# NikolasMarkou/blind_image_denoising

Measured on AMD Instinct MI355X. Metric: denoised images/sec (256x256x3) + MAE vs ref, resnet_1x18, higher is better.
Workload: dtype f16x2 split (hi+lo, fp32 accumulate)

## Files before the change

### blind_image_denoising_amd/_native.py

```python
import ctypes as C
import os
import pathlib

_HERE = pathlib.Path(__file__).resolve().parent
LIB_PATH = pathlib.Path(os.environ.get("BFCNN_HIP_LIB", _HERE / "lib" / "libbfcnn_hip.so"))

BF_OK, BF_EINVAL, BF_EUNSUPPORTED, BF_EWORKSPACE, BF_EHIP = 0, -1, -2, -3, -4
BF_ACT_LINEAR, BF_ACT_RELU, BF_ACT_LEAKY_RELU = 0, 1, 2
BF_REG_NONE, BF_REG_L1, BF_REG_L2 = 0, 1, 2
BF_MODE_INFERENCE, BF_MODE_TRAIN = 0, 1
BF_DTYPE_U8, BF_DTYPE_F32 = 0, 1
BF_LOSS_COUNT = 8
(BF_LOSS_TOTAL, BF_LOSS_DENOISER_TOTAL, BF_LOSS_MAE, BF_LOSS_MSE, BF_LOSS_SSIM,
 BF_LOSS_REGULARIZATION, BF_LOSS_MODEL_TOTAL, BF_LOSS_GRAD_NORM) = range(8)
EPI_RELU, EPI_AFFINE, EPI_RES, EPI_MASK, EPI_STATS, EPI_BNBWD = 1, 2, 4, 8, 16, 32


class ResnetDesc(C.Structure):
    _fields_ = [(n, C.c_int32) for n in (
        "struct_size", "in_channels", "filters", "kernel_size", "no_layers", "block_convs",
        "block_kernel", "activation", "base_activation", "use_bn", "head_filters",
        "head_activation", "out_channels", "denormalize", "reg_base", "reg_block", "reg_head")] + \
        [(n, C.c_float) for n in ("v_min", "v_max", "bn_eps", "bn_momentum", "leaky_alpha")]


class LossDesc(C.Structure):
    _fields_ = [("struct_size", C.c_int32)] + [(n, C.c_float) for n in (
        "hinge", "cutoff", "mae_multiplier", "mse_multiplier", "ssim_multiplier",
        "regularization", "depth_weight")]


class TensorInfo(C.Structure):
    _fields_ = [("name", C.c_char * 64), ("offset", C.c_int64), ("rank", C.c_int32),
                ("shape", C.c_int32 * 4), ("kind", C.c_int32), ("regularizer", C.c_int32)]


_P, _I, _I64, _F, _D = C.c_void_p, C.c_int, C.c_int64, C.c_float, C.c_double

SIGNATURES = {
    "bf_abi_version": (_I, []),
    "bf_create": (_I, [C.POINTER(ResnetDesc), C.POINTER(_P)]),
    "bf_destroy": (None, [_P]),
    "bf_last_error": (C.c_char_p, [_P]),
    "bf_param_count": (_I64, [_P]),
    "bf_state_count": (_I64, [_P]),
    "bf_tensor_count": (_I, [_P, _I]),
    "bf_tensor_at": (_I, [_P, _I, _I, C.POINTER(TensorInfo)]),
    "bf_packed_bytes": (_I64, [_P]),
    "bf_workspace_bytes": (_I64, [_P, _I, _I, _I, _I]),
    "bf_pack_inference": (_I, [_P, _P, _P, _P, _P]),
    "bf_forward_u8": (_I, [_P, _P, _P, _P, _I, _I, _I, _P, _I64, _P]),
    "bf_forward_f32": (_I, [_P, _P, _P, _P, _I, _I, _I, _P, _I64, _P]),
    "bf_forward_u8_f32": (_I, [_P, _P, _P, _P, _I, _I, _I, _P, _I64, _P]),
    "bf_train_step": (_I, [_P, _P, _P, _P, _P, _I, _I, _I, C.POINTER(LossDesc), _P, _P, _P, _P, _I64, _P]),
    "bf_adam_step": (_I, [_P, _P, _P, _P, _P, _I64, _F, _F, _F, _F, _F, _F, _P, _P, _P]),
    "bf_adam_step_ex": (_I, [_P, _P, _P, _P, _P, _I64, _F, _F, _F, _F, _F, _F, _F, _P, _I, _P, _F, _P, _P, _P]),
    "bf_avgpool_s2_same": (_I, [_P, _P, _I, _I, _I, _I, _I, _I, _P]),
    "bf_avgpool2_valid": (_I, [_P, _P, _I, _I, _I, _I, _I, _I, _P]),
    "bf_upsample2x": (_I, [_P, _P, _P, _I, _I, _I, _I, _I, _F, _F, _P]),
    "bf_laplacian_split": (_I, [_P, _P, _P, _I, _I, _I, _I, _I, _I, _P]),
    "bf_strided_slice2": (_I, [_P, _P, _I, _I, _I, _I, _P]),
    "bf_noise_augment": (_I, [_P, _P, _P, _I, _I, _I, _I, _I, _F, _F, C.c_uint64, _P]),
    "bf_image_metrics_scratch_bytes": (_I64, [_I, _I, _I, _I, _I]),
    "bf_image_metrics": (_I, [_P, _P, _I, _I, _I, _I, _I, _D, _I, _D, _D, _D, _P, _P, _I64, _P]),
    "bf_noise_estimate_scratch_bytes": (_I64, [_I, _I, _I, _I]),
    "bf_noise_estimate": (_I, [_P, _I, _I, _I, _I, _I, _P, _I64, _P, _P]),
    "bf_op_pack_pointwise": (_I, [_P, _P, _I, _I, _P]),
    "bf_op_pointwise": (_I, [_P, _P, _P, _P, _P, C.c_int64, _I, _I, _I, _F, _P]),
    "bf_op_pointwise_ex": (_I, [_P, _P, _P, _P, _P, _P, C.c_int64, _I, _I, _I, _F, _I, _P]),
    "bf_op_convnext_mlp": (_I, [_P, _P, _P, _P, _P, _P, C.c_int64, _I, _I, _F, _P]),
    "bf_op_mlp_h3_pack_bytes": (C.c_int64, [_I]),
    "bf_op_pack_mlp_h3": (_I, [_P, _P, _P, _I, _P]),
    "bf_op_convnext_mlp_h3": (_I, [_P, _P, _P, _P, _P, C.c_int64, _I, _I, _F, _P]),
    "bf_op_convnext_block1_h3": (_I, [_P, _P, _P, _P, _F, _P, _P, C.c_int64, _I, _I, _F, _P]),
    "bf_op_pack_mlp_h3_chain": (_I, [_P, _P, _P, _I, _P]),
    "bf_op_convnext_chain32_h3": (_I, [_P, _P, _P, _I, _P, _P, _P, _P, _F, _I, _I, _I, _I, _F, _I, _F, _P]),
    "bf_op_convnext_block1_up_h3": (_I, [_P, _P, _P, _P, _P, _F, _P, _P, _I, _I, _I, _I, _I, _F, _I, _F, _P]),
    "bf_op_convnext_block_h3": (_I, [_P, _P, _P, _I, _P, _F, _P, _P, _I, _I, _I, _I, _I, _F, _P]),
    "bf_op_set_variant": (_I, [C.c_char_p, _I]),
    "bf_op_dwconv_ln": (_I, [_P, _P, _P, _P, _I, _I, _I, _I, _I, _F, _I, _F, _P]),
    "bf_op_smooth_split": (_I, [_P, _P, _P, _P, _I, _I, _I, _I, _I, _I, _P]),
    "bf_op_conv2d": (_I, [_P, _P, _P, _P, _P, _I, _I, _I, _I, _I, _I, _I, _I, _I, _F, _P]),
    "bf_op_upcat_conv2d": (_I, [_P, _P, _P, _P, _P, _P, _I, _I, _I, _I, _I, _I, _I, _I, _F, _P]),
    "bf_op_dwconv_mult": (_I, [_P, _P, _P, _P, _I, _I, _I, _I, _I, _I, _I, _F, _P]),
    "bf_op_bneck_h3_pack_bytes": (C.c_int64, []),
    "bf_op_pack_bneck_h3": (_I, [_P, _P, _P, _P, _P]),
    "bf_op_bneck_block_h3": (_I, [_P, _P, _P, _P, _I, _F, _P, _I, _F, _P, _I, _F, _I, _I, _I, _I, _P]),
    "bf_op_dwmult_pointwise": (_I, [_P, _P, _P, _P, _I, _F, _P, _P, _I, _F, _P, _I, _I, _I, _I, _I, _I, _I, _P]),
    "bf_op_maxpool2": (_I, [_P, _P, _I, _I, _I, _I, _P]),
    "bf_op_maxpool2_bwd": (_I, [_P, _P, _P, _I, _I, _I, _I, _P]),
    "bf_op_norm_smooth_split": (_I, [_P, _P, _F, _I, _F, _P, _P, _P, _I, _I, _I, _I, _I, _P]),
    "bf_op_upsample_act_add": (_I, [_P, _P, _P, _I, _I, _I, _I, _I, _F, _P]),
    "bf_op_resize_bilinear": (_I, [_P, _P, _I, _I, _I, _I, _I, _I, _P]),
    "bf_op_attention": (_I, [_P, _P, _P, _P, _I, _I, _I, _P]),
    "bf_op_attention_ld": (_I, [_P, _P, _P, _P, _I, _I, _I, _I, _P]),
    "bf_op_first_conv": (_I, [_P, _I, _P, _P, _I, _I, _I, _I, _I, _I, _I, _I, _I, _F, _F, _I, _F, _P]),
    "bf_op_first_conv_h3": (_I, [_P, _I, _P, _P, _I, _I, _I, _I, _I, _I, _F, _F, _I, _F, _P]),
    "bf_op_first_conv_h3k": (_I, [_P, _I, _P, _P, _I, _I, _I, _I, _I, _I, _I, _F, _F, _I, _F, _P]),
    "bf_op_head_out": (_I, [_P, _P, _P, _I, _I, _I, _I, _I, _I, _I, _I, _I, _F, _F, _P, _P]),
    "bf_op_head_fused": (_I, [_P, _P, _F, _P, _I, _F, _P, _P, _I, _I, _I, _I, _I, _I, _I, _I, _I, _I, _F, _F, _P, _P]),
    "bf_op_head_fused_h3": (_I, [_P, _P, _F, _P, _I, _F, _P, _P, _I, _I, _I, _I, _I, _I, _I, _I, _I, _I, _F, _F, _P, _P]),
    "bf_op_fill32": (_I, [_P, _I, _I64, _P]),
    "bf_op_axpy": (_I, [_P, _P, _F, _I, _I64, _P]),
    "bf_op_conv2d_transpose": (_I, [_P, _P, _P, _I, _I, _I, _I, _I, _I, _I, _I, _F, _P]),
    "bf_op_adam_step": (_I, [_P, _P, _P, _P, _I64, _I64, _F, _F, _F, _F, _F, _F, _F, _P, _I, _P, _F, _P, _P, _P]),
    "bf_op_act_bwd": (_I, [_P, _P, _P, _I64, _I, _F, _I, _P]),
    "bf_op_matmul_wgrad": (_I, [_P, _P, _P, _I64, _I, _I, _P, _I64, _P]),
    "bf_op_dwconv_wgrad": (_I, [_P, _P, _P, _I, _I, _I, _I, _I, _P, _I64, _P]),
    "bf_op_layernorm_bwd": (_I, [_P, _P, _P, _P, _P, _I64, _I, _F, _P, _I64, _P]),
    "bf_op_scale_add": (_I, [_P, _P, _P, _P, _P, _I, _I64, _I, _P]),
    "bf_op_scale_add_bwd": (_I, [_P, _P, _P, _P, _P, _P, _I, _I64, _I, _P, _I64, _P]),
    "bf_op_multiplier_bwd": (_I, [_P, _P, _P, _I, _P]),
    "bf_op_smooth_split_bwd": (_I, [_P, _P, _P, _P, _I, _I, _I, _I, _I, _P]),
    "bf_op_smooth_split_bwd_ex": (_I, [_P, _P, _P, _P, _I, _I, _I, _I, _I, _I, _P]),
    "bf_op_upsample2x_bwd": (_I, [_P, _P, _I, _I, _I, _I, _I, _P]),
    "bf_op_conv2d_wgrad": (_I, [_P, _I, _P, _P, _I, _I, _I, _I, _I, _I, _I, _F, _F, _P, _I64, _P]),
    "bf_op_head_out_bwd": (_I, [_P, _P, _P, _P, _P, _I64, _I, _I, _I, _F, _F, _P, _I64, _P]),
    "bf_op_denoiser_loss_scratch_floats": (_I64, [_I, _I, _I, _I]),
    "bf_op_denoiser_loss": (_I, [_P, _P, _I, _I, _I, _I, C.POINTER(LossDesc), _P, _P, _P, _I64, _P]),
    "bf_op_attention_train": (_I, [_P, _P, _P, _P, _P, _P, _I, _I, _I, _P]),
    "bf_op_attention_bwd": (_I, [_P, _P, _P, _P, _P, _P, _P, _P, _P, _P, _I, _I, _I, _P]),
    "bf_op_resize_bilinear_bwd": (_I, [_P, _P, _I, _I, _I, _I, _I, _I, _P, _P]),
    "bf_op_reg_elementwise": (_I, [_P, _P, _I64, _I, _F, _F, _P, _P]),
    "bf_op_reg_soft_orthonormal": (_I, [_P, _P, _I, _I, _F, _F, _F, _F, _P, _P, _P]),
    "bf_op_reg_soft_orthogonal_ex": (_I, [_P, _P, _I, _I, _F, _F, _F, _F, _P, _P, _I, _P]),
    "bf_op_bn_train_scratch_floats": (_I64, [_I]),
    "bf_op_bn_train_fwd": (_I, [_P, _P, _P, _P, _P, _P, _I64, _I, _F, _F, _I, _F, _P, _I64, _P]),
    "bf_op_bn_train_bwd": (_I, [_P, _P, _P, _P, _P, _P, _I64, _I, _P, _I64, _P]),
    "bf_op_gate_save_floats": (_I64, [_I, _I, _I]),
    "bf_op_gate_scratch_floats": (_I64, [_I, _I]),
    "bf_op_gate_fwd": (_I, [_P, _P, _P, _P, _P, _P, _I, _I64, _I, _I, _P, _I64, _P]),
    "bf_op_gate_bwd": (_I, [_P, _P, _P, _P, _P, _P, _P, _P, _I, _I64, _I, _I, _P, _I64, _P]),
    "bf_op_channel_gate_save_floats": (_I64, [_I, _I, _I, _I]),
    "bf_op_channel_gate_ex": (_I, [_P, _P, _P, _P, _P, _P, _P, _P, _P, _P, _I, _I64, _I, _I, _I, _I, _F, _I, _P, _I64, _P]),
    "bf_op_dense2": (_I, [_P, _P, _P, _P, _P, _P, _I64, _I, _I, _I, _I, _F, _I, _P]),
    "bf_op_selector_mix": (_I, [_P, _P, _P, _P, _I64, _I, _P]),
    "bf_op_avgpool_same": (_I, [_P, _P, _I, _I, _I, _I, _I, _I, _I, _I, _P]),
    "bf_op_concat_channels": (_I, [_P, _P, _P, _P, _I64, _I, _I, _I, _P]),
    "bf_op_channel_mean_broadcast": (_I, [_P, _P, _I, _I64, _I, _I64, _P, _I64, _P]),
    "bf_op_sigmoid_gate": (_I, [_P, _P, _P, _P, _I64, _P]),
    "bf_op_sigmoid_gate_bwd": (_I, [_P, _P, _P, _P, _P, _I64, _P]),
    "bf_op_relu_shift": (_I, [_P, _I, _F, _P, _I, _P]),
    "bf_op_linear_shift": (_I, [_P, _I, _F, _P, _I, _P]),
    "bf_op_center_scale": (_I, [_P, _P, _P, _P, _I64, _F, _P]),
    "bf_op_pass_filter": (_I, [_P, _P, _I64, _F, _I, _I, _P]),
    "bf_op_pass_filter_bwd": (_I, [_P, _P, _P, _I64, _F, _I, _I, _P]),
    "bf_op_center_scale_bwd": (_I, [_P, _P, _P, _P, _P, _P, _I64, _F, _P]),
    "bf_op_center_sq_bwd": (_I, [_P, _P, _P, _P, _P, _I64, _P]),
    "bf_op_concat_input": (_I, [_P, _P, _I, _P, _I, _I, _I, _I, _I, _I, _I, _I, _F, _F, _P]),
    "bf_op_selector_mix_bwd": (_I, [_P, _P, _P, _P, _P, _P, _P, _I64, _I, _P]),
    "bf_op_avgpool_same_bwd": (_I, [_P, _P, _I, _I, _I, _I, _I, _I, _I, _I, _I, _P]),
    "bf_op_dense2_bwd_scratch_floats": (_I64, [_I64, _I, _I]),
    "bf_op_dense2_bwd": (_I, [_P, _P, _P, _P, _P, _P, _P, _I64, _I, _I, _I, _F, _P, _I64, _P]),
    "bf_op_slice_channels": (_I, [_P, _P, _I64, _I, _I, _I, _P]),
    "bf_op_relu_shift_bwd": (_I, [_P, _I, _F, _P, _P, _I, _P]),
    "bf_op_normalize": (_I, [_P, _P, _I64, _F, _F, _I, _P]),
    "bf_op_channel_repeat": (_I, [_P, _P, _I64, _I, _I, _P]),
    "bf_op_channel_group_sum": (_I, [_P, _P, _I64, _I, _I, _P]),
    "bf_op_group_kernel": (_I, [_P, _P, _I, _I, _I, _I, _P]),
    "bf_op_flip_hw": (_I, [_P, _P, _I, _I, _P]),
    "bf_op_transpose2d": (_I, [_P, _P, _I, _I, _P]),
    "bf_comm_unique_id": (_I, [C.c_char_p]),
    "bf_comm_init_rank": (_I, [C.POINTER(_P), _I, _I, C.c_char_p]),
    "bf_comm_destroy": (_I, [_P]),
    "bf_allreduce_grads": (_I, [_P, _P, _I64, _P, _P]),
    "bf_comm_last_error": (C.c_char_p, []),
    "bf_op_channel_multiplier": (_I, [_P, _P, _I, _P]),
    "bf_op_prune_tensors": (_I, [_P, _I64, _P, _I, _I, _F, _F, _F, C.c_uint64, _P, _P, _P]),
    "bf_op_count_below": (_I, [_P, _I64, _P, _I, _F, _P, _P]),
    "bf_op_dihedral_stack_u8": (_I, [_P, _P, _P, _I, _I, _I, _I, _I, _P]),
    "bf_op_dihedral_merge": (_I, [_P, _P, _P, _I, _I, _I, _I, _I, _I, _P]),
    "bf_op_risk_probe_u8": (_I, [_P, _P, _I, _I, _I, _I, _I, _I, C.c_uint64, _P]),
    "bf_op_risk_sums_scratch_bytes": (_I64, [_I, _I, _I, _I, _I]),
    "bf_op_risk_sums": (_I, [_P, _P, _I, _I, _I, _I, _I, _I, C.c_uint64, _P, _I64, _P, _P]),
    "bf_op_neighbor_pairs": (_I, [_P, _I, _P, _F, _P, _P, _I, _I, _I, _I, C.c_uint64, _P]),
    "bf_set_option": (_I, [_P, C.c_char_p, _I]),
    "bf_get_timing": (_I, [_P, C.POINTER(C.c_float), C.POINTER(C.c_int)]),
    "bf_get_block_kernel": (C.c_char_p, [_P, C.POINTER(C.c_int)]),
    "bf_get_train_kernels": (C.c_char_p, [_P]),
    "bf_debug_conv3x3": (_I, [_P, _P, _P, _P, _P, _P, _P, _P, _P, _I, _I, _I, _I, _I, _P]),
    "bf_debug_conv3x3_grid": (_I, [_I, _I, _I]),
    "bf_debug_h3_weight_scale": (_F, [_F]),
    "bf_debug_fused_block": (_I, [_P, _P, _P, _P, _P, _P, _P, _I, _I, _I, _I, _P]),
    "bf_debug_fused_block_h3_scratch_floats": (_I64, [_I, _I, _I]),
    "bf_debug_fused_block_h3": (_I, [_P, _P, _P, _P, _P, _P, _P, _I, _I, _I, _I, _P]),
    "bf_debug_fused_block2_h3_scratch_floats": (_I64, [_I, _I, _I]),
    "bf_debug_fused_block2_h3": (_I, [_P, _P, _P, _P, _P, _P, _I, _I, _I, _I, _I, _P]),
    "bf_debug_set_h3_variant": (_I, [_I]),
    "bf_debug_set_upsample_band": (_I, [_I]),
    "bf_debug_conv3x3_h3_scratch_floats": (_I64, []),
    "bf_debug_conv3x3_h3": (_I, [_P, _P, _P, _P, _P, _P, _P, _I, _I, _I, _I, _I, _P]),
    "bf_debug_wgrad_partial_floats": (_I64, [_I, _I, _I]),
    "bf_debug_wgrad3x3": (_I, [_P, _P, _P, _P, _I, _I, _I, _P]),
    "bf_debug_wgrad3x3_h3": (_I, [_P, _P, _P, _P, _I, _I, _I, _P]),
    "bf_debug_fwd_block_h3t_scratch_floats": (_I64, [_I, _I, _I]),
    "bf_debug_fwd_block_h3t": (_I, [_P, _P, _P, _P, _P, _P, _P, _P, _P, _P, _P, _I, _I, _I, _I, _I, _P]),
    "bf_debug_bwd_block_h3t_scratch_floats": (_I64, [_I, _I, _I]),
    "bf_debug_bwd_block_h3t": (_I, [_P, _P, _P, _P, _P, _P, _P, _P, _P, _P, _P, _P, _I, _I, _I, _I, _I, _P]),
    "bf_debug_conv3x3_h3_pre": (_I, [_P, _P, _P, _P, _P, _P, _P, _P, _I, _I, _I, _I, _I, _P]),
    "bf_debug_bwd3x3_h3_scratch_floats": (_I64, [_I, _I, _I]),
    "bf_debug_bwd3x3_h3_grid": (_I, [_I, _I, _I]),
    "bf_debug_bwd3x3_h3_grid_ex": (_I, [_I, _I, _I, _I]),
    "bf_debug_bwd3x3_h3": (_I, [_P, _P, _P, _P, _P, _P, _P, _P, _P, _P, _P, _I, _I, _I, _I, _I, _I, _P]),
    "bf_debug_forward_plan": (_I, [_P, _I, _I, _I, _I, C.c_char_p, _I]),
    "bf_debug_mfma_probe": (_I, [_P, _P, _P, _P]),
}

BF_STATUS_BYTES = 2048
BF_STATUS_F16_RANGE = 1

_lib = None


class StreamArg(C.c_void_p):
    _bf_device = None


def _device_guard(fn):
    def call(*args):
        for a in args:
            dev = getattr(a, "_bf_device", None)
            if dev is not None:
                import torch
                if torch.cuda.current_device() != dev:
                    with torch.cuda.device(dev):
                        return fn(*args)
                break
        return fn(*args)
    call.raw = fn
    call.__name__ = getattr(fn, "__name__", "bf_call")
    return call


class _Library:

    def __init__(self, handle):
        self._handle = handle

    def __getattr__(self, name):
        return getattr(self._handle, name)


def lib():
    global _lib
    if _lib is None:
        if not LIB_PATH.exists():
            raise ImportError(
                f"{LIB_PATH} is missing: the gfx950 HIP library has not been built "
                f"(run blind_image_denoising_amd/csrc/build.sh). There is no CPU fallback.")
        handle = C.CDLL(str(LIB_PATH), mode=getattr(os, "RTLD_NOW", 2))
        wrapped = _Library(handle)
        for name, (res, args) in SIGNATURES.items():
            fn = getattr(handle, name)
            fn.restype = res
            fn.argtypes = args
            setattr(wrapped, name, _device_guard(fn))
        if handle.bf_abi_version() != 1:
            raise ImportError("libbfcnn_hip.so ABI version mismatch")
        _lib = wrapped
    return _lib


def last_error(handle=None) -> str:
    msg = lib().bf_last_error(handle)
    return msg.decode("utf-8", "replace") if msg else ""


def check(rc: int, handle=None, what: str = ""):
    if rc == BF_OK:
        return
    msg = f"{what}: {last_error(handle)}" if what else last_error(handle)
    if rc == BF_EINVAL:
        raise ValueError(msg)
    if rc == BF_EUNSUPPORTED:
        raise NotImplementedError(msg)
    if rc == BF_EWORKSPACE:
        raise MemoryError(msg)
    raise RuntimeError(f"HIP error ({rc}) {msg}")


def call(fn_name: str, *args):
    check(getattr(lib(), fn_name)(*args), None, fn_name)


def ptr(t):
    if t is None:
        return None
    if not t.is_contiguous():
        raise ValueError("tensor must be contiguous")
    return C.c_void_p(t.data_ptr())


def stream_ptr(t=None):
    import torch
    if t is not None and t.is_cuda:
        dev = t.device.index if t.device.index is not None else torch.cuda.current_device()
    else:
        dev = torch.cuda.current_device()
    s = StreamArg(torch.cuda.current_stream(dev).cuda_stream)
    s._bf_device = dev
    return s
```

### blind_image_denoising_amd/csrc/base_rows.hip

```cpp
#include "bf_common.h"
#include "h3_core.h"
#include "h3_weights.h"
#include <cstdlib>

constexpr int BR_NT = 256, BR_CW = 256, BR_RING = 4, BR_ROWPX = BR_CW + 4;

__global__ __launch_bounds__(BR_NT) void base_conv_rows_kernel(BaseConvArgs a, int nchunks, int rows_per_band, int nbands, int abl)
{
    __shared__ __attribute__((aligned(16))) h4 ring[BR_RING][2][BR_ROWPX];
    __shared__ float red[BR_NT];
    const int tid = threadIdx.x, lane = tid & 63, wave = tid >> 6, n = lane & 15, q = lane >> 4;
    if (a.status && blockIdx.x == 0 && tid == 0) *a.status = 0;
    const float* __restrict__ w = a.w;

    auto wval = [&](const int tap, const int c, const int m) -> float {
        if (c < 3) return w[(tap * 3 + c) * 16 + m] / 255.0f;
        return -0.5f * (w[(tap * 3 + 0) * 16 + m] + w[(tap * 3 + 1) * 16 + m] + w[(tap * 3 + 2) * 16 + m]);
    };
    const float s = bf_h3_block_weight_scale<BR_NT>([&](const int i) { return wval(i / 64, (i >> 4) & 3, i & 15); }, 9 * 4 * 16, red);
    const float inv_s = 1.0f / s;
    h8 wa[3];
#pragma unroll
    for (int dy = 0; dy < 3; ++dy) {
#pragma unroll
        for (int j = 0; j < 8; ++j) {
            const int slot = 8 * (q & 1) + j, dx = slot >> 2, c = slot & 3;
            float v = 0.f;
            if (dx < 3) v = wval(dy * 3 + dx, c, n) * s;
            _Float16 hi, lo;
            bf_h3_split(v, hi, lo);
            wa[dy][j] = (q >> 1) ? lo : hi;
        }
    }

    int bx = blockIdx.x;
    const int ch = bx % nchunks; bx /= nchunks;
    const int band = bx % nbands;
    const int b = bx / nbands;
    const int x0 = ch * BR_CW;
    const int y0 = band * rows_per_band, y1 = min(y0 + rows_per_band, a.H);
    const uint8_t* __restrict__ src = reinterpret_cast<const uint8_t*>(a.in) + (int64_t)b * a.Hs * a.Ws * 3;

    auto fetch = [&](const int yy, const int j) -> h4 {
        const int x = x0 - 1 + j;
        h4 r = {(_Float16)0.f, (_Float16)0.f, (_Float16)0.f, (_Float16)0.f};
        if (yy >= 0 && yy < a.H && x >= 0 && x < a.W) {
            r[3] = (_Float16)1.f;
            if (!(abl & 2) && yy < a.Hs && x < a.Ws) {
                const uint8_t* p = src + ((int64_t)yy * a.Ws + x) * 3;
                r[0] = (_Float16)(float)p[0];
                r[1] = (_Float16)(float)p[1];
                r[2] = (_Float16)(float)p[2];
            }
        }
        return r;
    };
    auto store_px = [&](const int slot, const int j, const h4 v) {
        ring[slot][0][j] = v;
        if (j > 0) ring[slot][1][j - 1] = v;
    };
    auto put = [&](const int yy) {
        const int slot = ((yy % BR_RING) + BR_RING) % BR_RING;
        store_px(slot, tid, fetch(yy, tid));
        if (tid < 4) store_px(slot, BR_CW + tid, fetch(yy, BR_CW + tid));
    };
    put(y0 - 1);
    put(y0);
    put(y0 + 1);
    __syncthreads();

    const int64_t hw = (int64_t)a.H * a.W;
    char* outb = reinterpret_cast<char*>(a.out) + (int64_t)b * hw * 64 + (int64_t)((q >> 1) + 2 * (q & 1)) * hw * 16;
    int frag_off[4];
#pragma unroll
    for (int g = 0; g < 4; ++g) {
        const int p = 64 * wave + 16 * g + n + 2 * (q & 1);
        frag_off[g] = ((p & 1) * BR_ROWPX + (p & ~1)) * 8;
    }
    const char* ring_b = reinterpret_cast<const char*>(&ring[0][0][0]);
    constexpr int SLOT_BYTES = 2 * BR_ROWPX * 8;
    for (int y = y0; y < y1; ++y) {
        const h4 nx = fetch(y + 2, tid);
        h4 nx2 = {(_Float16)0.f, (_Float16)0.f, (_Float16)0.f, (_Float16)0.f};
        if (tid < 4) nx2 = fetch(y + 2, BR_CW + tid);
        int so[3];
#pragma unroll
        for (int dy = 0; dy < 3; ++dy) so[dy] = ((((y + dy - 1) % BR_RING) + BR_RING) % BR_RING) * SLOT_BYTES;
        char* orow = outb + (int64_t)y * a.W * 16;
#pragma unroll
        for (int g = 0; g < 4; ++g) {
            const int xc = 64 * wave + 16 * g + n;
            f32x4 acc = {0.f, 0.f, 0.f, 0.f};
#pragma unroll
            for (int dy = 0; dy < 3; ++dy)
                acc = MFMA_H(wa[dy], *reinterpret_cast<const h8*>(ring_b + so[dy] + frag_off[g]), acc);
            acc = bf_acc_ready(acc) * inv_s;
            if (a.act_relu) {
#pragma unroll
                for (int c = 0; c < 4; ++c) acc[c] = fmaxf(acc[c], 0.f);
            }
            const int x = x0 + xc;
            const h8 rec = h3_split_record(acc);
            if ((abl & 1) ? acc[0] == 12345.678f : x < a.W) *reinterpret_cast<h8*>(orow + (int64_t)x * 16) = rec;
        }
        const int slot = (((y + 2) % BR_RING) + BR_RING) % BR_RING;
        store_px(slot, tid, nx);
        if (tid < 4) store_px(slot, BR_CW + tid, nx2);
        __syncthreads();
    }
}

bool bf_base_conv_rows_supports(const BaseConvArgs& a)
{
    return a.in_is_u8 && a.cin == 3 && a.k == 3 && a.out_split == 1 && a.v_min == 0.f && a.v_max == 255.f && a.H >= 1 && a.W >= 1;
}

hipError_t bf_launch_base_conv_rows(const BaseConvArgs& a, hipStream_t s)
{
    if (!bf_base_conv_rows_supports(a)) return hipErrorInvalidValue;
    const int nchunks = (a.W + BR_CW - 1) / BR_CW;
    int rows = 32;
    int ablate = 0;
#ifdef BF_ABLATE
    if (const char* e = getenv("BF_BASE_ROWS_ABL")) ablate = atoi(e);
    if (const char* e = getenv("BF_BASE_ROWS_BAND")) rows = atoi(e) > 0 ? atoi(e) : rows;
    else
#endif
    while (rows > 8 && (int64_t)a.B * nchunks * ((a.H + rows - 1) / rows) < 1024) rows /= 2;
    const int nbands = (a.H + rows - 1) / rows;
    const int64_t grid = (int64_t)a.B * nchunks * nbands;
    if (grid > 0x7fffffff) return hipErrorInvalidValue;
    hipLaunchKernelGGL(base_conv_rows_kernel, dim3((unsigned)grid), dim3(BR_NT), 0, s, a, nchunks, rows, nbands, ablate);
    return hipGetLastError();
}
```

### blind_image_denoising_amd/csrc/bf_common.h

```cpp
#pragma once
#include <hip/hip_runtime.h>
#include <stdint.h>
#include <stddef.h>
#include "../../include/bfcnn_hip.h"
#include "../../include/bfcnn_hip_debug.h"

typedef float f32x4 __attribute__((ext_vector_type(4)));

__device__ __forceinline__ f32x4 bf_acc_ready(f32x4 acc)
{
    asm volatile("s_nop 7" : "+v"(acc));
    return acc;
}


#include <mutex>
#include <unordered_set>
inline hipError_t bf_set_max_lds(const void* kernel, int bytes)
{
    static std::mutex mu;
    static std::unordered_set<uint64_t> done;
    int dev = 0;
    hipError_t e = hipGetDevice(&dev);
    if (e != hipSuccess) return e;
    const uint64_t key = (uint64_t)(uintptr_t)kernel * 131u + (uint64_t)(dev + 1);
    std::lock_guard<std::mutex> lock(mu);
    if (done.count(key)) return hipSuccess;
    e = hipFuncSetAttribute(kernel, hipFuncAttributeMaxDynamicSharedMemorySize, bytes);
    if (e == hipSuccess) done.insert(key);
    return e;
}

typedef _Float16 bf_h8 __attribute__((ext_vector_type(8)));
typedef _Float16 bf_h2 __attribute__((ext_vector_type(2)));
typedef short bf_s2 __attribute__((ext_vector_type(2)));
typedef unsigned bf_u2 __attribute__((ext_vector_type(2)));
#define BF_H3C_SCALE (1.0f / 4096.0f)
__device__ __forceinline__ bf_u2 bf_h3c_encode8(const bf_h8 v)
{
    const bf_h2 lim = {(_Float16)(448.0f / 4096.0f), (_Float16)(448.0f / 4096.0f)};
    bf_h2 p[4] = {{v[0], v[1]}, {v[2], v[3]}, {v[4], v[5]}, {v[6], v[7]}};
#pragma unroll
    for (int i = 0; i < 4; ++i) p[i] = __builtin_elementwise_min(__builtin_elementwise_max(p[i], -lim), lim);
    bf_s2 r0 = {0, 0}, r1 = {0, 0};
    r0 = __builtin_amdgcn_cvt_scalef32_pk_fp8_f16(r0, p[0], BF_H3C_SCALE, false);
    r0 = __builtin_amdgcn_cvt_scalef32_pk_fp8_f16(r0, p[1], BF_H3C_SCALE, true);
    r1 = __builtin_amdgcn_cvt_scalef32_pk_fp8_f16(r1, p[2], BF_H3C_SCALE, false);
    r1 = __builtin_amdgcn_cvt_scalef32_pk_fp8_f16(r1, p[3], BF_H3C_SCALE, true);
    bf_u2 out;
    out[0] = ((unsigned)(unsigned short)r0[0]) | ((unsigned)(unsigned short)r0[1] << 16);
    out[1] = ((unsigned)(unsigned short)r1[0]) | ((unsigned)(unsigned short)r1[1] << 16);
    return out;
}
__device__ __forceinline__ bf_h8 bf_h3c_decode8(const bf_u2 b)
{
    const bf_h2 a0 = __builtin_amdgcn_cvt_scalef32_pk_f16_fp8(b[0], BF_H3C_SCALE, false);
    const bf_h2 a1 = __builtin_amdgcn_cvt_scalef32_pk_f16_fp8(b[0], BF_H3C_SCALE, true);
    const bf_h2 a2 = __builtin_amdgcn_cvt_scalef32_pk_f16_fp8(b[1], BF_H3C_SCALE, false);
    const bf_h2 a3 = __builtin_amdgcn_cvt_scalef32_pk_f16_fp8(b[1], BF_H3C_SCALE, true);
    return (bf_h8){a0[0], a0[1], a1[0], a1[1], a2[0], a2[1], a3[0], a3[1]};
}

__device__ __forceinline__ float bf_gelu(const float v)
{
    const float a = fabsf(v) * 0.70710678f;
    float q = fmaf(4.22452448e-05f, a, -4.19236813e-04f);
    q = fmaf(q, a, 1.40204388e-03f);
    q = fmaf(q, a, 9.21467334e-04f);
    q = fmaf(q, a, -2.83861113e-02f);
    q = fmaf(q, a, 1.48544322e-01f);
    q = fmaf(q, a, 9.18402423e-01f);
    q = fmaf(q, a, 1.62790967f);
    const float h = __builtin_amdgcn_exp2f(fmaf(-a, q, -1.f));
    return v * (v >= 0.f ? 1.f - h : h);
}

#define BF_C 16
#define BF_WPACK_FLOATS (36 * 64)

enum { EPI_RELU = 1, EPI_AFFINE = 2, EPI_RES = 4, EPI_MASK = 8, EPI_STATS = 16, EPI_BNBWD = 32 };

struct ConvArgs {
    const float* in;
    float* out;
    const float* wpack;
    const float* scale;
    const float* shift;
    const float* res;
    const float* mask;
    float* stats;
    const float* bnc;
    int B, H, W;
    int reverse;
    const float* pre_c; const float* pre_scale; const float* pre_shift; float* pre_out;
};

struct FusedBlockArgs {
    const float* in;
    float* out;
    const float* w1pack;
    const float* w2pack;
    const float* scale;
    const float* shift;
    int B, H, W;
    int tiles_x, tiles_y, ntiles;
    int act1_relu;
    const float* zeros;
};

#define BF_H3R_WPACK_FLOATS (13 * 64 * 4)
#define BF_H3_BLOCK_FLOATS (64 + 2 * BF_H3R_WPACK_FLOATS)
struct FusedH3Args {
    const void* in;
    void* out;
    const void* w1r;
    const void* w2r;
    const float* aux;
    int B, H, W;
    int tiles_x, tiles_y, ntiles;
    int rows_per_tile;
    int reverse_tiles;
    int variant;
    int act1_relu;
    const void* zeros;
    void* dump;
    unsigned long long* dbg;
    const float* head_wh;
    void* head_out;
    int head_u8, Ho, Wo, denormalize;
    float v_min, v_max;
    int* status;
    int compact = 0;
};
struct H3Request {
    int B, H, W;
    int variant;
    bool head;
    bool compact;
};
enum class H3Kernel { Tiles32, Tiles16, FullRow };
struct H3Choice {
    H3Kernel kernel;
    bool bottom_up;
};
H3Choice   bf_select_fused_block_h3(const H3Request& r);
hipError_t bf_launch_fused_block_h3_as(const FusedH3Args& a, H3Kernel k, hipStream_t s);
hipError_t bf_launch_fused_block_h3(const FusedH3Args& a, hipStream_t s);
bool       bf_fused_block_h3_use_pairs(const H3Request& r);
const char* bf_fused_block_h3_kernel_name(H3Kernel k);
const char* bf_fused_block_kernel_name();
void       bf_set_h3_variant(int v);
hipError_t bf_launch_fused_block_h3v(const FusedH3Args& a, hipStream_t s);
bool       bf_fused_block_h3v_supports(int H, int W);
struct FusedH3WArgs {
    const void* in;
    void* out;
    const void* w1r[2];
    const void* w2r[2];
    const float* aux[2];
    int B, H, W;
    int nstrips, tiles_y, ntiles, rows_per_tile;
    int reverse_tiles;
    int act1_relu;
    const void* zeros;
    unsigned long long* dbg;
    const float* head_wh;
    void* head_out;
    int head_u8, Ho, Wo, denormalize;
    float v_min, v_max;
    int* status;
};
hipError_t bf_launch_fused_block2_h3w(const FusedH3WArgs& a, hipStream_t s);
bool       bf_fused_block2_h3w_supports(int H, int W);
hipError_t bf_launch_pack_h3(const float* params, const float* state, int64_t p_blocks, int64_t p_stride, float* dst,
                             int64_t d_stride, int layers, int use_bn, float eps, const float* ext_scale,
                             const float* ext_shift, hipStream_t s);
#define BF_H3_TRAIN_PACK_FLOATS (BF_H3R_WPACK_FLOATS + 64)
#define BF_TRAIN_PACK_STRIDE BF_H3_TRAIN_PACK_FLOATS
hipError_t bf_launch_conv3x3_h3(const ConvArgs& a, int epi, hipStream_t s);
hipError_t bf_launch_wgrad3x3_h3(const float* x, const float* dy, float* partial, float* dw, int B, int H, int W, hipStream_t s);

struct BwdH3Args {
    const float* x;
    const float* g;
    const float* c;
    const float* coef;
    const float* wpack;
    float* out;
    const float* res;
    const float* bnc;
    float* wpartial;
    float* stats;
    int B, H, W, reverse;
    int reserved[4];
    int tiles_x, tiles_y, ntiles;
};
struct FwdBlockH3Args {
    const float* x;
    const float* pre_c;
    const float* pre_scale; const float* pre_shift;
    float* a_out;
    float* t_out;
    float* c_out;
    const float* wpack0;
    const float* wpack1;
    float* stats;
    int B, H, W, reverse, act_relu;
    int tiles_y, ntiles, rows_per_tile;
    const float* fin_partial;
    int fin_nblk;
    double fin_count;
    const float* fin_gamma;
    float *fin_mm, *fin_mv;
    float fin_eps, fin_momentum;
    float* fin_scale;
    float* fin_meaninv;
};
bool       bf_fwd_block_h3t_supports(int H, int W);
int        bf_fwd_block_h3t_grid(int B, int H, int W);
hipError_t bf_launch_fwd_block_h3t(const FwdBlockH3Args& a, hipStream_t s);
struct BwdBlockH3Args {
    const float* a;
    const float* g;
    const float* c;
    const float* coef;
    const float* wfwd0;
    const float* wdg1;
    const float* wdg0;
    const float* bnc;
    float* out;
    float* wpartial1;
    float* wpartial0;
    float* stats;
    int B, H, W, reverse, act_relu;
    int nstrips, tiles_y, ntiles, rows_per_tile;
    unsigned long long* dbg;
    const float* fin_partial;
    int fin_nblk;
    double fin_count;
    const float* fin_gamma;
    const float* fin_meaninv;
    float* fin_dgamma;
};
bool       bf_bwd_block_h3t_supports(int H, int W);
int        bf_bwd_block_h3t_grid(int B, int H, int W);
int64_t    bf_bwd_block_h3t_strip_rows(int B, int H, int W);
hipError_t bf_launch_bwd_block_h3t(const BwdBlockH3Args& a, hipStream_t s);
int        bf_bwd3x3_h3_grid(int B, int H, int W);
hipError_t bf_launch_bwd3x3_h3(const BwdH3Args& a, int epi, float* dw, hipStream_t s);
hipError_t bf_launch_reduce_wgrad_slots(const float* slots, int64_t slot_floats, int nblk, float* out, int64_t p_stride, int layers,
                                        int nconv, int unit, hipStream_t s);
hipError_t bf_launch_pack_h3_train(const float* params, int64_t p_blocks, int64_t p_stride, float* dst, int layers, int nconv,
                                   int unit, hipStream_t s);
hipError_t bf_launch_h3_from_f32(const float* x, void* y, int B, int H, int W, hipStream_t s);
hipError_t bf_launch_h3_to_f32(const void* y, float* x, int B, int H, int W, hipStream_t s);

hipError_t bf_launch_conv3x3_c16(const ConvArgs& a, int epi, hipStream_t s);
int        bf_conv3x3_c16_grid(int B, int H, int W);
hipError_t bf_launch_fused_block(const FusedBlockArgs& a, hipStream_t s);
void       bf_set_fused_tile(int variant);
hipError_t bf_launch_pack_conv(const float* w_hwio, float* wpack, int transpose_flip, hipStream_t s);
hipError_t bf_launch_wgrad3x3_c16(const float* x, const float* dy, float* partial, float* dw,
                                  int B, int H, int W, hipStream_t s);
int        bf_wgrad_grid(int B, int H, int W);

struct BaseConvArgs {
    const void* in; float* out; const float* w;
    int B, Hs, Ws, H, W, cin, k, in_is_u8, act_relu;
    float v_min, v_max;
    int out_split;
    int* status;
};
hipError_t bf_launch_base_conv(const BaseConvArgs& a, hipStream_t s);
bool       bf_base_conv_rows_supports(const BaseConvArgs& a);
hipError_t bf_launch_base_conv_rows(const BaseConvArgs& a, hipStream_t s);
void       bf_set_base_conv_rows(int on);
hipError_t bf_launch_base_wgrad(const float* in_f32, const float* dy, float* partial, float* dw,
                                int B, int H, int W, int cin, int k, float v_min, float v_max, hipStream_t s);
int        bf_base_wgrad_grid(int B, int H, int W);

struct HeadArgs {
    const float* feat;
    const float* w0;
    const float* w1;
    const float* wh;
    void* out;
    int B, H, W, Ho, Wo, hf, cout, act, out_is_u8, denormalize;
    float v_min, v_max, leaky_alpha;
    int feat_split;
    int* status;
};
#define BF_STATUS_BYTES 2048

hipError_t bf_launch_head(const HeadArgs& a, hipStream_t s);

struct HeadTrainArgs {
    const float* feat; const float* wh;
    const float* gt; float* pred;
    float* dfeat;
    float* partial;
    const float* dextra;
    int B, H, W, cout, denormalize;
    float v_min, v_max, hinge, cutoff, dscale;
    float dfeat_scale;
};
hipError_t bf_launch_head_train(const HeadTrainArgs& a, int grid, hipStream_t s);
hipError_t bf_launch_loss_extra(const float* pred, const float* gt, int B, int H, int W, int C, const float* head_partial,
                                int blocks_per_image, float hinge, float cutoff, float mse_multiplier, float ssim_multiplier,
                                float depth_weight, float max_val, float* maps, float* ssim_partial, float* coef, float* scal,
                                float* dextra, hipStream_t s);
hipError_t bf_launch_loss_extra_finalize(const float* scal, int B, int H, int W, int C, float mse_multiplier, float ssim_multiplier,
                                         float depth_weight, float* losses, hipStream_t s);
int        bf_head_train_grid(int B, int H, int W);

hipError_t bf_launch_bn_finalize(const float* partial, int nblk, double count, const float* gamma,
                                 float* moving_mean, float* moving_var, float eps, float momentum,
                                 float* scale, float* shift, float* mean_inv , double* stage1 ,
                                 hipStream_t s);
hipError_t bf_launch_affine_add(const float* x, const float* c, const float* scale, const float* shift,
                                float* y, int64_t npix, hipStream_t s);
hipError_t bf_launch_affine_act(const float* c, const float* scale, const float* shift, float* y, int relu, int64_t npix,
                                hipStream_t s);
hipError_t bf_launch_bn_bwd_reduce(const float* dy, const float* c, float* partial, int64_t npix, int grid, hipStream_t s);
hipError_t bf_launch_bn_bwd_finalize(const float* partial, int nblk, double count, const float* gamma,
                                     const float* mean_inv, float* coef , float* dgamma,
                                     double* stage1 , hipStream_t s);
hipError_t bf_launch_bn_bwd_apply(const float* dy, const float* c, const float* coef, float* dc, int64_t npix, hipStream_t s);
hipError_t bf_launch_reduce_partials(const float* partial, int nblk, int width, float* out, float scale, hipStream_t s);
hipError_t bf_launch_zero(float* p, int64_t n, hipStream_t s);
```

### blind_image_denoising_amd/csrc/edge_layers.hip

```cpp
#include "bf_common.h"
#include "block_reduce.h"

typedef _Float16 h8 __attribute__((ext_vector_type(8)));

constexpr int BC_T = 16;

template <int CIN, int K, bool U8>
__global__ __launch_bounds__(256) void base_conv_kernel(BaseConvArgs a)
{
    constexpr int R = K / 2, IT = BC_T + 2 * R;
    __shared__ float tile[IT * IT * CIN];
    const float* __restrict__ wg = a.w;
    const int tiles_x = (a.W + BC_T - 1) / BC_T, tiles_y = (a.H + BC_T - 1) / BC_T;
    int t = blockIdx.x;
    const int tx = t % tiles_x; t /= tiles_x;
    const int ty = t % tiles_y;
    const int b = t / tiles_y;
    const int y0 = ty * BC_T, x0 = tx * BC_T;
    if (a.status && blockIdx.x == 0 && threadIdx.x == 0) *a.status = 0;
    const float range = a.v_max - a.v_min;
    {
        constexpr int NE = (IT * IT * CIN + 255) / 256;
        float raw[NE];
        bool inimg[NE];
#pragma unroll
        for (int i = 0; i < NE; ++i) {
            const int n = threadIdx.x + i * 256;
            const int ci = n % CIN, px = (n / CIN) % IT, row = n / (CIN * IT);
            const int gy = y0 - R + row, gx = x0 - R + px;
            inimg[i] = n < IT * IT * CIN && gy >= 0 && gy < a.H && gx >= 0 && gx < a.W;
            raw[i] = 0.f;
            if (inimg[i] && gy < a.Hs && gx < a.Ws) {
                const int64_t si = (((int64_t)b * a.Hs + gy) * a.Ws + gx) * CIN + ci;
                raw[i] = U8 ? (float)reinterpret_cast<const uint8_t*>(a.in)[si] : reinterpret_cast<const float*>(a.in)[si];
            }
        }
#pragma unroll
        for (int i = 0; i < NE; ++i) {
            const int n = threadIdx.x + i * 256;
            const float v = inimg[i] ? (fminf(fmaxf(raw[i], a.v_min), a.v_max) - a.v_min) / range - 0.5f : 0.f;
            if (n < IT * IT * CIN) tile[n] = v;
        }
    }
    __syncthreads();
    const int ly = threadIdx.x >> 4, lx = threadIdx.x & 15;
    const int y = y0 + ly, x = x0 + lx;
    float acc[16];
#pragma unroll
    for (int c = 0; c < 16; ++c) acc[c] = 0.f;
#pragma unroll
    for (int ky = 0; ky < K; ++ky)
#pragma unroll
        for (int kx = 0; kx < K; ++kx)
#pragma unroll
            for (int ci = 0; ci < CIN; ++ci) {
                const float v = tile[((ly + ky) * IT + lx + kx) * CIN + ci];
                const float* wr = wg + ((ky * K + kx) * CIN + ci) * 16;
#pragma unroll
                for (int c = 0; c < 16; ++c) acc[c] = fmaf(v, wr[c], acc[c]);
            }
    if (y < a.H && x < a.W) {
        if (a.act_relu) {
#pragma unroll
            for (int c = 0; c < 16; ++c) acc[c] = fmaxf(acc[c], 0.f);
        }
        if (a.out_split) {
            const int64_t hw = (int64_t)a.H * a.W;
            char* base = reinterpret_cast<char*>(a.out) + (int64_t)b * hw * 64 + ((int64_t)y * a.W + x) * 16;
            h8 hi[2], lo[2];
#pragma unroll
            for (int c = 0; c < 16; ++c) {
                const _Float16 h = (_Float16)acc[c];
                hi[c >> 3][c & 7] = h;
                lo[c >> 3][c & 7] = (_Float16)(acc[c] - (float)h);
            }
            *reinterpret_cast<h8*>(base) = hi[0];
            *reinterpret_cast<h8*>(base + hw * 16) = hi[1];
            if (a.out_split == 2) {
                char* lob = reinterpret_cast<char*>(a.out) + (int64_t)b * hw * 64 + hw * 32 + ((int64_t)y * a.W + x) * 8;
                *reinterpret_cast<bf_u2*>(lob) = bf_h3c_encode8(lo[0]);
                *reinterpret_cast<bf_u2*>(lob + hw * 8) = bf_h3c_encode8(lo[1]);
                return;
            }
            *reinterpret_cast<h8*>(base + hw * 32) = lo[0];
            *reinterpret_cast<h8*>(base + hw * 48) = lo[1];
            return;
        }
        float4* o = reinterpret_cast<float4*>(a.out + (((int64_t)b * a.H + y) * a.W + x) * 16);
        o[0] = make_float4(acc[0], acc[1], acc[2], acc[3]);
        o[1] = make_float4(acc[4], acc[5], acc[6], acc[7]);
        o[2] = make_float4(acc[8], acc[9], acc[10], acc[11]);
        o[3] = make_float4(acc[12], acc[13], acc[14], acc[15]);
    }
}

template <int CIN, int K>
static hipError_t launch_base(const BaseConvArgs& a, hipStream_t s)
{
    const int grid = a.B * ((a.H + BC_T - 1) / BC_T) * ((a.W + BC_T - 1) / BC_T);
    if (a.in_is_u8) hipLaunchKernelGGL((base_conv_kernel<CIN, K, true>), dim3(grid), dim3(256), 0, s, a);
    else            hipLaunchKernelGGL((base_conv_kernel<CIN, K, false>), dim3(grid), dim3(256), 0, s, a);
    return hipGetLastError();
}

static int g_base_rows = 1;
void bf_set_base_conv_rows(int on) { g_base_rows = on == 2 ? 2 : (on ? 1 : 0); }
static bool base_rows_preferred(const BaseConvArgs& a)
{
    const int64_t nchunks = (a.W + 255) / 256;
    return (int64_t)a.B * a.H * nchunks >= 8192 && (int64_t)a.W * 5 >= nchunks * 256 * 3;
}

hipError_t bf_launch_base_conv(const BaseConvArgs& a, hipStream_t s)
{
    if (g_base_rows && bf_base_conv_rows_supports(a) && (g_base_rows == 2 || base_rows_preferred(a))) return bf_launch_base_conv_rows(a, s);
#define BF_BASE(C, KK) if (a.cin == C && a.k == KK) return launch_base<C, KK>(a, s);
    BF_BASE(3, 3) BF_BASE(3, 5) BF_BASE(3, 7) BF_BASE(3, 1)
    BF_BASE(1, 3) BF_BASE(1, 5) BF_BASE(1, 7) BF_BASE(1, 1)
#undef BF_BASE
    return hipErrorInvalidValue;
}

constexpr int BW_TH = 16, BW_TW = 32;

template <int CIN, int K>
__global__ __launch_bounds__(512) void base_wgrad_kernel(const float* __restrict__ in, const float* __restrict__ dy,
                                                         float* __restrict__ partial, int B, int H, int W,
                                                         float v_min, float v_max, int tiles_x, int tiles_y, int ntiles)
{
    constexpr int R = K / 2, IH = BW_TH + 2 * R, IW = BW_TW + 2 * R;
    constexpr int NCOMB = K * K * CIN, PERC = (NCOMB + 31) / 32, NOUT = NCOMB * 16;
    static_assert(BW_TH == 16, "one row slice per 32 threads");
    __shared__ float tx_[IH * IW * CIN];
    __shared__ __attribute__((aligned(16))) float td[BW_TH * BW_TW * 16];
    const int tid = threadIdx.x, slice = tid >> 5, j0 = tid & 31;
    const float range = v_max - v_min;
    f32x4 acc[PERC][4];
    int xoff[PERC];
#pragma unroll
    for (int i = 0; i < PERC; ++i) {
#pragma unroll
        for (int q = 0; q < 4; ++q) acc[i][q] = (f32x4){0.f, 0.f, 0.f, 0.f};
        int jj = j0 + 32 * i;
        if (jj >= NCOMB) jj = 0;
        const int ci = jj % CIN, tap = jj / CIN;
        xoff[i] = ((tap / K) * IW + (tap % K)) * CIN + ci;
    }
    for (int t = blockIdx.x; t < ntiles; t += gridDim.x) {
        int tt = t;
        const int txi = tt % tiles_x; tt /= tiles_x;
        const int tyi = tt % tiles_y;
        const int b = tt / tiles_y;
        const int y0 = tyi * BW_TH, x0 = txi * BW_TW;
        for (int n = tid; n < IH * IW * CIN; n += 512) {
            const int ci = n % CIN, px = (n / CIN) % IW, row = n / (CIN * IW);
            const int gy = y0 - R + row, gx = x0 - R + px;
            float v = 0.f;
            if (gy >= 0 && gy < H && gx >= 0 && gx < W) {
                const float raw = in[(((int64_t)b * H + gy) * W + gx) * CIN + ci];
                v = (fminf(fmaxf(raw, v_min), v_max) - v_min) / range - 0.5f;
            }
            tx_[n] = v;
        }
        for (int n = tid; n < BW_TH * BW_TW * 4; n += 512) {
            const int row = n / (BW_TW * 4), rem = n - row * (BW_TW * 4);
            const int gy = y0 + row, gx = x0 + (rem >> 2);
            float4 v = make_float4(0.f, 0.f, 0.f, 0.f);
            if (gy < H && gx < W)
                v = *reinterpret_cast<const float4*>(dy + (((int64_t)b * H + gy) * W + gx) * 16 + (rem & 3) * 4);
            *reinterpret_cast<float4*>(td + n * 4) = v;
        }
        __syncthreads();
        for (int c = 0; c < BW_TW; ++c) {
            const int pb = (slice * IW + c) * CIN, db = (slice * BW_TW + c) * 16;
            f32x4 d[4];
#pragma unroll
            for (int q = 0; q < 4; ++q) d[q] = *reinterpret_cast<const f32x4*>(td + db + 4 * q);
#pragma unroll
            for (int i = 0; i < PERC; ++i) {
                const float xv = tx_[pb + xoff[i]];
#pragma unroll
                for (int q = 0; q < 4; ++q) acc[i][q] += d[q] * xv;
            }
        }
        __syncthreads();
    }
    float* red = td;
#pragma unroll
    for (int i = 0; i < PERC; ++i) {
        __syncthreads();
#pragma unroll
        for (int q = 0; q < 4; ++q) *reinterpret_cast<f32x4*>(red + (slice * 32 + j0) * 16 + 4 * q) = acc[i][q];
        __syncthreads();
        const int jj = (tid >> 4) + 32 * i, co = tid & 15;
        if (jj < NCOMB) {
            float a = 0.f;
#pragma unroll
            for (int sl = 0; sl < 16; ++sl) a += red[(sl * 32 + (tid >> 4)) * 16 + co];
            partial[(size_t)blockIdx.x * NOUT + jj * 16 + co] = a;
        }
    }
}

int bf_base_wgrad_grid(int B, int H, int W)
{
    const int ntiles = B * ((H + BW_TH - 1) / BW_TH) * ((W + BW_TW - 1) / BW_TW);
    return ntiles < 512 ? ntiles : 512;
}

template <int CIN, int K>
static hipError_t launch_base_wgrad(const float* in, const float* dy, float* partial, float* dw, int B, int H, int W,
                                    float v_min, float v_max, hipStream_t s)
{
    const int tiles_x = (W + BW_TW - 1) / BW_TW, tiles_y = (H + BW_TH - 1) / BW_TH;
    const int ntiles = B * tiles_x * tiles_y, grid = bf_base_wgrad_grid(B, H, W);
    hipLaunchKernelGGL((base_wgrad_kernel<CIN, K>), dim3(grid), dim3(512), 0, s, in, dy, partial, B, H, W, v_min, v_max,
                       tiles_x, tiles_y, ntiles);
    hipError_t e = hipGetLastError();
    if (e != hipSuccess) return e;
    return bf_launch_reduce_partials(partial, grid, K * K * CIN * 16, dw, 1.0f, s);
}

hipError_t bf_launch_base_wgrad(const float* in, const float* dy, float* partial, float* dw, int B, int H, int W,
                                int cin, int k, float v_min, float v_max, hipStream_t s)
{
#define BF_BW(C, KK) if (cin == C && k == KK) return launch_base_wgrad<C, KK>(in, dy, partial, dw, B, H, W, v_min, v_max, s);
    BF_BW(3, 3) BF_BW(3, 5) BF_BW(3, 7) BF_BW(3, 1)
    BF_BW(1, 3) BF_BW(1, 5) BF_BW(1, 7) BF_BW(1, 1)
#undef BF_BW
    return hipErrorInvalidValue;
}

__device__ __forceinline__ float bf_act(float x, int act, float alpha)
{
    if (act == BF_ACT_RELU) return fmaxf(x, 0.f);
    if (act == BF_ACT_LEAKY_RELU) return x > 0.f ? x : alpha * x;
    return x;
}

template <bool U8>
__global__ __launch_bounds__(256) void head_kernel(HeadArgs a)
{
    __shared__ float w0s[16 * 64];
    __shared__ float w1s[64 * 4];
    __shared__ float whs[64];
    const bool fused = a.wh != nullptr;
    if (fused) {
        for (int i = threadIdx.x; i < 64; i += 256) whs[i] = a.wh[i];
    } else {
        for (int i = threadIdx.x; i < 16 * a.hf; i += 256) w0s[i] = a.w0[i];
        for (int i = threadIdx.x; i < a.hf * a.cout; i += 256) w1s[i] = a.w1[i];
    }
    __syncthreads();
    const int64_t npix = (int64_t)a.B * a.Ho * a.Wo;
    for (int64_t pix = (int64_t)blockIdx.x * 256 + threadIdx.x; pix < npix; pix += (int64_t)gridDim.x * 256) {
        const int x = (int)(pix % a.Wo);
        const int64_t t = pix / a.Wo;
        const int y = (int)(t % a.Ho);
        const int b = (int)(t / a.Ho);
        float f[16];
        if (a.feat_split) {
            const int64_t hw = (int64_t)a.H * a.W;
            const char* base = reinterpret_cast<const char*>(a.feat) + (int64_t)b * hw * 64 + ((int64_t)y * a.W + x) * 16;
            const h8 hi0 = *reinterpret_cast<const h8*>(base), hi1 = *reinterpret_cast<const h8*>(base + hw * 16);
            h8 lo0, lo1;
            if (a.feat_split == 2) {
                const char* lob = reinterpret_cast<const char*>(a.feat) + (int64_t)b * hw * 64 + hw * 32 + ((int64_t)y * a.W + x) * 8;
                lo0 = bf_h3c_decode8(*reinterpret_cast<const bf_u2*>(lob));
                lo1 = bf_h3c_decode8(*reinterpret_cast<const bf_u2*>(lob + hw * 8));
            } else {
                lo0 = *reinterpret_cast<const h8*>(base + hw * 32);
                lo1 = *reinterpret_cast<const h8*>(base + hw * 48);
            }
            bool finite = true;
#pragma unroll
            for (int c = 0; c < 8; ++c) {
                f[c] = (float)hi0[c] + (float)lo0[c];
                f[8 + c] = (float)hi1[c] + (float)lo1[c];
                finite = finite && fabsf(f[c]) <= 3.0e38f && fabsf(f[8 + c]) <= 3.0e38f;
            }
            if (!finite && a.status) atomicOr(a.status, BF_STATUS_F16_RANGE);
        } else {
            const float4* fp = reinterpret_cast<const float4*>(a.feat + (((int64_t)b * a.H + y) * a.W + x) * 16);
#pragma unroll
            for (int i = 0; i < 4; ++i) {
                const float4 v = fp[i];
                f[4 * i] = v.x; f[4 * i + 1] = v.y; f[4 * i + 2] = v.z; f[4 * i + 3] = v.w;
            }
        }
        float h1[4] = {0.f, 0.f, 0.f, 0.f};
        if (fused) {
#pragma unroll
            for (int c = 0; c < 16; ++c)
#pragma unroll
                for (int o = 0; o < 4; ++o) h1[o] = fmaf(f[c], whs[c * 4 + o], h1[o]);
        } else {
            for (int j = 0; j < a.hf; ++j) {
                float h = 0.f;
#pragma unroll
                for (int c = 0; c < 16; ++c) h = fmaf(f[c], w0s[c * a.hf + j], h);
                h = bf_act(h, a.act, a.leaky_alpha);
                for (int o = 0; o < a.cout; ++o) h1[o] = fmaf(h, w1s[j * a.cout + o], h1[o]);
            }
        }
        for (int o = 0; o < a.cout; ++o) {
            float v = tanhf(2.0f * h1[o]) * 0.51f;
            if (a.denormalize) v = (fminf(fmaxf(v, -0.5f), 0.5f) + 0.5f) * (a.v_max - a.v_min) + a.v_min;
            if (U8) {
                const float r = fminf(fmaxf(rintf(v), 0.f), 255.f);
                reinterpret_cast<uint8_t*>(a.out)[pix * a.cout + o] = (uint8_t)r;
            } else {
                reinterpret_cast<float*>(a.out)[pix * a.cout + o] = v;
            }
        }
    }
}

hipError_t bf_launch_head(const HeadArgs& a, hipStream_t s)
{
    const int64_t npix = (int64_t)a.B * a.Ho * a.Wo;
    int64_t g = (npix + 255) / 256;
    const int grid = (int)(g < 8192 ? g : 8192);
    if (a.out_is_u8) hipLaunchKernelGGL(head_kernel<true>, dim3(grid), dim3(256), 0, s, a);
    else             hipLaunchKernelGGL(head_kernel<false>, dim3(grid), dim3(256), 0, s, a);
    return hipGetLastError();
}

constexpr int HT_BLOCKS_PER_IMAGE_MAX = 64;

__global__ __launch_bounds__(256) void head_train_kernel(HeadTrainArgs a, int blocks_per_image)
{
    __shared__ float whs[64];
    __shared__ float red[4][80];
    if (threadIdx.x < 64) whs[threadIdx.x] = a.wh[threadIdx.x];
    __syncthreads();
    const int b = blockIdx.x / blocks_per_image, sub = blockIdx.x % blocks_per_image;
    const int hw = a.H * a.W;
    float M[64];
#pragma unroll
    for (int i = 0; i < 64; ++i) M[i] = 0.f;
    float s_abs = 0.f, s_hinge = 0.f, s_sq = 0.f, s_sqh = 0.f;
    for (int pi = sub * 256 + threadIdx.x; pi < hw; pi += blocks_per_image * 256) {
        const int64_t pix = (int64_t)b * hw + pi;
        const float4* fp = reinterpret_cast<const float4*>(a.feat + pix * 16);
        float f[16];
#pragma unroll
        for (int i = 0; i < 4; ++i) {
            const float4 v = fp[i];
            f[4 * i] = v.x; f[4 * i + 1] = v.y; f[4 * i + 2] = v.z; f[4 * i + 3] = v.w;
        }
        float dh1[4] = {0.f, 0.f, 0.f, 0.f};
#pragma unroll
        for (int o = 0; o < 4; ++o) {
            if (o < a.cout) {
                float h = 0.f;
#pragma unroll
                for (int c = 0; c < 16; ++c) h = fmaf(f[c], whs[c * 4 + o], h);
                const float th = tanhf(2.0f * h);
                const float pv = th * 0.51f;
                float pred = pv, dpred_dp = 1.0f;
                if (a.denormalize) {
                    pred = (fminf(fmaxf(pv, -0.5f), 0.5f) + 0.5f) * (a.v_max - a.v_min) + a.v_min;
                    dpred_dp = (pv >= -0.5f && pv <= 0.5f) ? (a.v_max - a.v_min) : 0.f;
                }
                if (a.pred) a.pred[pix * a.cout + o] = pred;
                const float e = a.gt[pix * a.cout + o] - pred;
                const float ae = fabsf(e);
                s_abs += fminf(ae, 255.0f);
                s_hinge += ae > a.hinge ? fminf(ae, a.cutoff) : 0.f;
                const float ep = e > 0.f ? fminf(e, 255.0f) : 0.f;
                s_sq += ep * ep;
                const float eh = e > a.hinge ? fminf(e, a.cutoff * a.cutoff) : 0.f;
                s_sqh += eh * eh;
                float dpred = 0.f;
                if (ae > a.hinge && ae < a.cutoff) dpred = (e > 0.f ? -1.f : (e < 0.f ? 1.f : 0.f)) * a.dscale;
                if (a.dextra) dpred += a.dextra[pix * a.cout + o];
                dh1[o] = dpred * dpred_dp * (0.51f * 2.0f) * (1.0f - th * th);
            }
        }
        float df[16];
#pragma unroll
        for (int c = 0; c < 16; ++c) {
            float d = 0.f;
#pragma unroll
            for (int o = 0; o < 4; ++o) {
                d = fmaf(dh1[o], whs[c * 4 + o], d);
                M[c * 4 + o] = fmaf(f[c], dh1[o], M[c * 4 + o]);
            }
            df[c] = d * a.dfeat_scale;
        }
        float4* dp = reinterpret_cast<float4*>(a.dfeat + pix * 16);
#pragma unroll
        for (int i = 0; i < 4; ++i) dp[i] = make_float4(df[4 * i], df[4 * i + 1], df[4 * i + 2], df[4 * i + 3]);
    }
#pragma unroll
    for (int i = 0; i < 64; ++i) bf_tile_stage(red, i, M[i]);
    const float sv[4] = {s_abs, s_hinge, s_sq, s_sqh};
#pragma unroll
    for (int i = 0; i < 4; ++i) bf_tile_stage(red, 64 + i, sv[i]);
    __syncthreads();
    if (threadIdx.x < 80) {
        const int i = threadIdx.x;
        a.partial[(size_t)blockIdx.x * 80 + i] = i < 68 ? (red[0][i] + red[1][i]) + (red[2][i] + red[3][i]) : 0.f;
    }
}

int bf_head_train_grid(int B, int H, int W)
{
    int bpi = (H * W + 1023) / 1024;
    if (bpi > HT_BLOCKS_PER_IMAGE_MAX) bpi = HT_BLOCKS_PER_IMAGE_MAX;
    if (bpi < 1) bpi = 1;
    return B * bpi;
}

hipError_t bf_launch_head_train(const HeadTrainArgs& a, int grid, hipStream_t s)
{
    hipLaunchKernelGGL(head_train_kernel, dim3(grid), dim3(256), 0, s, a, grid / a.B);
    return hipGetLastError();
}
```

### blind_image_denoising_amd/csrc/engine.h

```cpp
#pragma once
#include "bf_common.h"
#include <string>
#include <utility>
#include <vector>

constexpr int BF_TIMING_RING = 256;

struct TimingRing {
    enum Kind { None, Forward, TrainBlock };
    std::vector<hipEvent_t> ev;
    int64_t n = 0;
    int launches_in_pair = 0;
    Kind kind = None;

    void restart() { n = 0; kind = None; }
    hipError_t begin(hipStream_t s) { return hipEventRecord(ev[2 * (n % BF_TIMING_RING)], s); }
    hipError_t end(hipStream_t s, int launches, Kind k)
    {
        int64_t slot = n % BF_TIMING_RING;
        if (k != kind) {
            std::swap(ev[0], ev[2 * slot]);
            n = 0; slot = 0; kind = k;
        }
        launches_in_pair = launches;
        ++n;
        return hipEventRecord(ev[2 * slot + 1], s);
    }
};

struct bf_engine {
    bf_resnet_desc d;
    std::string err;
    std::vector<bf_tensor_info> tensors, states;
    int64_t n_params = 0, n_state = 0;
    int64_t p_base = 0, p_blocks = 0, p_block_stride = 0, p_head0 = 0, p_head1 = 0;
    int64_t n_base = 0;
    int64_t k_base = 0, k_blocks = 0, k_block_stride = 0, k_w0 = 0, k_w1 = 0, k_wh = 0, k_zero = 0, k_h3 = 0, k_total = 0;
    int fused_blocks = 1;
    int fused_head = 0;
    int h3_zigzag = 1;
    int h3_variant = -1;
    int h3_compact = 0;
    int h3_pair = 1;
    int h3_pair_head = 0;
    int block_launches = 0;
    const char* block_kernel = "";
    std::string train_kernels;
    int arith = 1;
    int train_arith = 1;
    int train_zigzag = 1;
    int train_fused_fwd = 1;
    int train_fwd_block = 1;
    int train_bwd_block = 1;
    int train_fold_finalize = 1;
    int train_fused_bwd = 1;
    int timing = 0;
    TimingRing timed;
};

int fail(bf_handle h, int code, const char* fmt, ...);
int hip_fail(bf_handle h, hipError_t e, const char* what);

#define BF_HIP(call, what) do { hipError_t e__ = (call); if (e__ != hipSuccess) return hip_fail(h, e__, what); } while (0)

static inline int64_t align_up(int64_t v, int64_t a) { return (v + a - 1) / a * a; }

static inline int pow2_target(int n)
{
    int p = 1;
    while (p < n) p <<= 1;
    return p;
}

hipError_t bf_launch_pack_all_convs(const float* params, int64_t p_blocks, int64_t p_stride, float* dst, int64_t d_stride, int layers,
                                    int with_dgrad, int nconv, int unit, hipStream_t s);
int64_t bf_train_workspace_floats(bf_handle h, int B, int H, int W);
```

### blind_image_denoising_amd/csrc/engine.hip

```cpp
#include "engine.h"
#include <cstdarg>
#include <cstdio>
#include <cstring>

static thread_local std::string g_create_error;

int fail(bf_handle h, int code, const char* fmt, ...)
{
    char buf[512];
    va_list ap;
    va_start(ap, fmt);
    vsnprintf(buf, sizeof(buf), fmt, ap);
    va_end(ap);
    if (h) h->err = buf; else g_create_error = buf;
    return code;
}

int hip_fail(bf_handle h, hipError_t e, const char* what)
{
    return fail(h, BF_EHIP, "%s: %s", what, hipGetErrorString(e));
}

extern "C" int bf_abi_version(void) { return BFCNN_ABI_VERSION; }

extern "C" const char* bf_last_error(bf_handle h) { return h ? h->err.c_str() : g_create_error.c_str(); }

static void add_tensor(std::vector<bf_tensor_info>& v, const char* name, int64_t& off, int rank, int s0, int s1, int s2,
                       int s3, int kind, int reg)
{
    bf_tensor_info t;
    memset(&t, 0, sizeof(t));
    snprintf(t.name, sizeof(t.name), "%s", name);
    t.offset = off;
    t.rank = rank;
    t.shape[0] = s0; t.shape[1] = s1; t.shape[2] = s2; t.shape[3] = s3;
    t.kind = kind;
    t.regularizer = reg;
    int64_t n = 1;
    for (int i = 0; i < rank; ++i) n *= t.shape[i];
    off += n;
    v.push_back(t);
}

extern "C" int bf_create(const bf_resnet_desc* d, bf_handle* out)
{
    if (out) *out = nullptr;
    if (!d || !out) return fail(nullptr, BF_EINVAL, "bf_create: desc/out must not be NULL");
    if (d->struct_size != (int32_t)sizeof(bf_resnet_desc))
        return fail(nullptr, BF_EINVAL, "bf_create: struct_size %d != %d (ABI mismatch)", d->struct_size, (int)sizeof(bf_resnet_desc));
    if (d->no_layers < 0) return fail(nullptr, BF_EINVAL, "no_layers must be >= 0");
    if (d->block_convs <= 0) return fail(nullptr, BF_EINVAL, "len(block_kernels) must be >= 0 ");
    if (d->block_convs > 3) return fail(nullptr, BF_EINVAL, "len(block_kernels) must be <= 3");
    if (d->in_channels != 1 && d->in_channels != 3)
        return fail(nullptr, BF_EUNSUPPORTED, "in_channels %d: only 1 and 3 are built", d->in_channels);
    if (d->filters != BF_C) return fail(nullptr, BF_EUNSUPPORTED, "filters %d: the MFMA path is built for 16", d->filters);
    if (d->kernel_size != 1 && d->kernel_size != 3 && d->kernel_size != 5 && d->kernel_size != 7)
        return fail(nullptr, BF_EUNSUPPORTED, "base kernel_size %d: only 1,3,5,7", d->kernel_size);
    if (d->block_kernel != 3)
        return fail(nullptr, BF_EUNSUPPORTED, "block_kernels must be 3x3 (got %d convs of %d)", d->block_convs, d->block_kernel);
    if (d->activation != BF_ACT_RELU && d->activation != BF_ACT_LINEAR)
        return fail(nullptr, BF_EUNSUPPORTED, "block activation must be relu or linear");
    if (d->base_activation != BF_ACT_LINEAR)
        return fail(nullptr, BF_EUNSUPPORTED, "base_activation must be linear");
    if (d->head_filters < 1 || d->head_filters > 64) return fail(nullptr, BF_EUNSUPPORTED, "head filters must be in 1..64");
    if (d->out_channels < 1 || d->out_channels > 4) return fail(nullptr, BF_EUNSUPPORTED, "output_channels must be in 1..4");
    if (!(d->v_max > d->v_min)) return fail(nullptr, BF_EINVAL, "value_range must have max > min");

    bf_engine* h = new bf_engine();
    h->d = *d;
    const int k = d->kernel_size, cin = d->in_channels, hf = d->head_filters, co = d->out_channels;
    int64_t off = 0;
    h->p_base = off;
    add_tensor(h->tensors, "base/kernel", off, 4, k, k, cin, BF_C, BF_KIND_CONV, d->reg_base);
    h->n_base = off;
    h->p_blocks = off;
    const int nb = d->block_convs;
    h->p_block_stride = nb * 2304 + (d->use_bn ? (nb - 1) * 16 : 0);
    char name[64];
    for (int i = 0; i < d->no_layers; ++i) {
        for (int j = 0; j < nb; ++j) {
            snprintf(name, sizeof(name), "block%d/conv%d/kernel", i, j);
            add_tensor(h->tensors, name, off, 4, 3, 3, BF_C, BF_C, BF_KIND_CONV, d->reg_block);
            if (j >= 1 && d->use_bn) {
                snprintf(name, sizeof(name), "block%d/bn%d/gamma", i, j);
                add_tensor(h->tensors, name, off, 1, BF_C, 0, 0, 0, BF_KIND_GAMMA, BF_REG_NONE);
            }
        }
    }
    h->p_head0 = off;
    add_tensor(h->tensors, "head/conv0/kernel", off, 4, 1, 1, BF_C, hf, BF_KIND_CONV, d->reg_head);
    h->p_head1 = off;
    add_tensor(h->tensors, "head/conv1/kernel", off, 4, 1, 1, hf, co, BF_KIND_CONV, d->reg_head);
    h->n_params = off;
    int64_t soff = 0;
    if (d->use_bn) {
        for (int i = 0; i < d->no_layers; ++i)
            for (int j = 1; j < nb; ++j) {
                snprintf(name, sizeof(name), "block%d/bn%d/moving_mean", i, j);
                add_tensor(h->states, name, soff, 1, BF_C, 0, 0, 0, BF_KIND_MOVING_MEAN, BF_REG_NONE);
                snprintf(name, sizeof(name), "block%d/bn%d/moving_variance", i, j);
                add_tensor(h->states, name, soff, 1, BF_C, 0, 0, 0, BF_KIND_MOVING_VAR, BF_REG_NONE);
            }
    }
    h->n_state = soff;
    int64_t ko = 0;
    h->k_base = ko; ko += align_up(h->n_base, 64);
    h->k_blocks = ko; h->k_block_stride = nb == 2 ? 2 * BF_WPACK_FLOATS + 32 : nb * (BF_WPACK_FLOATS + 32);
    ko += h->k_block_stride * d->no_layers;
    h->k_w0 = ko; ko += align_up(16 * hf, 64);
    h->k_w1 = ko; ko += align_up(hf * co, 64);
    h->k_wh = ko; ko += 64;
    h->k_zero = ko; ko += 64;
    h->k_h3 = ko; ko += (int64_t)BF_H3_BLOCK_FLOATS * d->no_layers;
    h->k_total = ko;
    *out = h;
    return BF_OK;
}

extern "C" void bf_destroy(bf_handle h)
{
    if (!h) return;
    for (hipEvent_t e : h->timed.ev) (void)hipEventDestroy(e);
    delete h;
}
extern "C" int64_t bf_param_count(bf_handle h) { return h ? h->n_params : -1; }
extern "C" int64_t bf_state_count(bf_handle h) { return h ? h->n_state : -1; }
extern "C" int bf_tensor_count(bf_handle h, int state) { return h ? (int)(state ? h->states.size() : h->tensors.size()) : -1; }

extern "C" int bf_tensor_at(bf_handle h, int state, int index, bf_tensor_info* out)
{
    if (!h || !out) return BF_EINVAL;
    const auto& v = state ? h->states : h->tensors;
    if (index < 0 || index >= (int)v.size()) return fail(h, BF_EINVAL, "tensor index %d out of range", index);
    *out = v[index];
    return BF_OK;
}

extern "C" int bf_set_option(bf_handle h, const char* key, int value)
{
    if (!h || !key) return BF_EINVAL;
    if (!strcmp(key, "fused_blocks")) { h->fused_blocks = value ? 1 : 0; return BF_OK; }
    if (!strcmp(key, "fused_tile")) { bf_set_fused_tile(value); return BF_OK; }
    if (!strcmp(key, "h3_variant")) { h->h3_variant = value; return BF_OK; }
    if (!strcmp(key, "h3_zigzag")) { h->h3_zigzag = value ? 1 : 0; return BF_OK; }
    if (!strcmp(key, "h3_compact")) { h->h3_compact = value ? 1 : 0; return BF_OK; }
    if (!strcmp(key, "h3_pair")) { h->h3_pair = value == 2 ? 2 : (value ? 1 : 0); return BF_OK; }
    if (!strcmp(key, "base_rows")) { bf_set_base_conv_rows(value); return BF_OK; }
    if (!strcmp(key, "h3_pair_head")) { h->h3_pair_head = value ? 1 : 0; return BF_OK; }
    if (!strcmp(key, "fused_head")) { h->fused_head = value ? 1 : 0; return BF_OK; }
    if (!strcmp(key, "train_zigzag")) { h->train_zigzag = value ? 1 : 0; return BF_OK; }
    if (!strcmp(key, "train_fused_fwd")) { h->train_fused_fwd = value ? 1 : 0; return BF_OK; }
    if (!strcmp(key, "train_fused_bwd")) { h->train_fused_bwd = value ? 1 : 0; return BF_OK; }
    if (!strcmp(key, "train_bwd_block")) { h->train_bwd_block = value < 0 ? 1 : (value > 2 ? 2 : value); return BF_OK; }
    if (!strcmp(key, "train_fwd_block")) { h->train_fwd_block = value < 0 ? 1 : (value > 2 ? 2 : value); return BF_OK; }
    if (!strcmp(key, "train_fused_bwd2") || !strcmp(key, "train_bwd_dbuf")) return BF_OK;
    if (!strcmp(key, "train_fold_finalize")) { h->train_fold_finalize = value ? 1 : 0; return BF_OK; }
    if (!strcmp(key, "train_arith")) { h->train_arith = value < 0 ? 1 : (value ? 1 : 0); return BF_OK; }
    if (!strcmp(key, "arith")) { h->arith = value < 0 ? 1 : (value ? 1 : 0); return BF_OK; }
    if (!strcmp(key, "timing")) {
        h->timing = value ? 1 : 0;
        h->timed.restart();
        if (h->timing && h->timed.ev.empty()) {
            h->timed.ev.resize(2 * BF_TIMING_RING, nullptr);
            for (hipEvent_t& e : h->timed.ev)
                if (hipEventCreate(&e) != hipSuccess) return fail(h, BF_EHIP, "hipEventCreate failed");
        }
        return BF_OK;
    }
    return fail(h, BF_EINVAL, "unknown option [%s]", key);
}

extern "C" int bf_get_timing(bf_handle h, float* ms, int* launches)
{
    if (!h || !ms || !launches) return BF_EINVAL;
    const TimingRing& t = h->timed;
    if (!h->timing || t.ev.empty()) return fail(h, BF_EINVAL, "timing option is off");
    const int64_t n = t.n < BF_TIMING_RING ? t.n : BF_TIMING_RING;
    if (n == 0) return fail(h, BF_EINVAL, "no forward has run since the timing option was set");
    double total = 0.0;
    for (int64_t i = 0; i < n; ++i) {
        float one = 0.f;
        hipError_t e = hipEventElapsedTime(&one, t.ev[2 * i], t.ev[2 * i + 1]);
        if (e != hipSuccess) return hip_fail(h, e, "hipEventElapsedTime");
        total += one;
    }
    *ms = (float)total;
    *launches = (int)(t.launches_in_pair * n);
    return BF_OK;
}

extern "C" const char* bf_get_block_kernel(bf_handle h, int* launches_per_forward)
{
    if (!h) return "";
    if (launches_per_forward) *launches_per_forward = h->block_launches;
    return h->block_kernel;
}

extern "C" const char* bf_get_train_kernels(bf_handle h) { return h ? h->train_kernels.c_str() : ""; }

extern "C" int64_t bf_packed_bytes(bf_handle h) { return h ? h->k_total * 4 : -1; }

extern "C" int64_t bf_workspace_bytes(bf_handle h, int mode, int B, int H, int W)
{
    if (!h || B <= 0 || H <= 0 || W <= 0) return -1;
    if (mode == BF_MODE_INFERENCE) {
        const int Hp = pow2_target(H), Wp = pow2_target(W);
        return (int64_t)B * Hp * Wp * 16 * 4 * 3 + BF_STATUS_BYTES;
    }
    return bf_train_workspace_floats(h, B, H, W) * 4;
}
```

### blind_image_denoising_amd/csrc/engine_infer.hip

```cpp
#include "engine.h"
#include <cstdio>
#include <cstring>

__global__ void pack_all_convs_kernel(const float* __restrict__ params, int64_t p_blocks, int64_t p_stride, float* __restrict__ dst,
                                      int64_t d_stride, int with_dgrad, int nconv, int unit)
{
    const int per = (with_dgrad ? 2 : 1) * nconv;
    const int layer = blockIdx.x / per, which = blockIdx.x % per;
    const int cj = which % nconv;
    const float* w = params + p_blocks + layer * p_stride + (cj == 0 ? 0 : 2304 + (int64_t)(cj - 1) * unit);
    float* o = dst + layer * d_stride + which * (with_dgrad ? (int64_t)BF_TRAIN_PACK_STRIDE : (int64_t)BF_WPACK_FLOATS);
    const int tf = which / nconv;
    for (int idx = threadIdx.x; idx < BF_WPACK_FLOATS; idx += blockDim.x) {
        const int i = idx >> 6, l = idx & 63;
        const int tap = i >> 2, kk = i & 3;
        const int cin = 4 * (l >> 4) + kk, cout = l & 15;
        o[idx] = tf ? w[((8 - tap) * 16 + cout) * 16 + cin] : w[(tap * 16 + cin) * 16 + cout];
    }
}

hipError_t bf_launch_pack_all_convs(const float* params, int64_t p_blocks, int64_t p_stride, float* dst, int64_t d_stride, int layers,
                                    int with_dgrad, int nconv, int unit, hipStream_t s)
{
    hipLaunchKernelGGL(pack_all_convs_kernel, dim3(layers * (with_dgrad ? 2 : 1) * nconv), dim3(256), 0, s, params, p_blocks, p_stride, dst,
                       d_stride, with_dgrad, nconv, unit);
    return hipGetLastError();
}

__global__ void fold_bn_kernel(const float* __restrict__ params, const float* __restrict__ state, int64_t p_blocks, int64_t p_stride,
                               float* __restrict__ packed, int64_t k_blocks, int64_t k_stride, int layers, int use_bn, float eps)
{
    const int i = blockIdx.x * blockDim.x + threadIdx.x;
    if (i >= layers * 16) return;
    const int layer = i / 16, c = i % 16;
    float sc = 1.f, sh = 0.f;
    if (use_bn) {
        const float g = params[p_blocks + layer * p_stride + 4608 + c];
        const float mean = state[layer * 32 + c], var = state[layer * 32 + 16 + c];
        sc = g / sqrtf(var + eps);
        sh = -sc * mean;
    }
    float* o = packed + k_blocks + layer * k_stride + 2 * BF_WPACK_FLOATS;
    o[c] = sc;
    o[16 + c] = sh;
}

__global__ void pack_edges_kernel(const float* __restrict__ params, float* __restrict__ packed, int64_t p_base, int64_t n_base,
                                  int64_t p_head0, int64_t p_head1, int hf, int co, int64_t k_base, int64_t k_w0, int64_t k_w1,
                                  int64_t k_wh)
{
    for (int i = threadIdx.x; i < n_base; i += blockDim.x) packed[k_base + i] = params[p_base + i];
    for (int i = threadIdx.x; i < 16 * hf; i += blockDim.x) packed[k_w0 + i] = params[p_head0 + i];
    for (int i = threadIdx.x; i < hf * co; i += blockDim.x) packed[k_w1 + i] = params[p_head1 + i];
    if (threadIdx.x < 64) {
        const int c = threadIdx.x >> 2, o = threadIdx.x & 3;
        float s = 0.f;
        if (o < co)
            for (int j = 0; j < hf; ++j) s = fmaf(params[p_head0 + c * hf + j], params[p_head1 + j * co + o], s);
        packed[k_wh + threadIdx.x] = s;
        packed[k_wh + 64 + threadIdx.x] = 0.f;
    }
}

__global__ void pack_generic_blocks_kernel(const float* __restrict__ params, const float* __restrict__ state, int64_t p_blocks,
                                           int64_t p_stride, float* __restrict__ dst, int64_t d_stride, int nb, int use_bn, float eps)
{
    const int layer = blockIdx.x / nb, j = blockIdx.x % nb;
    const int64_t conv_off = (int64_t)j * 2304 + (use_bn && j >= 2 ? (j - 1) * 16 : 0);
    const float* w = params + p_blocks + layer * p_stride + conv_off;
    float* o = dst + layer * d_stride + (int64_t)j * BF_WPACK_FLOATS;
    for (int idx = threadIdx.x; idx < BF_WPACK_FLOATS; idx += blockDim.x) {
        const int i = idx >> 6, l = idx & 63;
        const int tap = i >> 2, kk = i & 3;
        const int cin = 4 * (l >> 4) + kk, cout = l & 15;
        o[idx] = w[(tap * 16 + cin) * 16 + cout];
    }
    if (threadIdx.x < 16) {
        const int c = threadIdx.x;
        float sc = 1.f, sh = 0.f;
        if (use_bn && j >= 1) {
            const float g = w[2304 + c];
            const float* st = state + ((int64_t)layer * (nb - 1) + (j - 1)) * 32;
            sc = g / sqrtf(st[16 + c] + eps);
            sh = -sc * st[c];
        }
        float* aff = dst + layer * d_stride + (int64_t)nb * BF_WPACK_FLOATS + j * 32;
        aff[c] = sc;
        aff[16 + c] = sh;
    }
}

extern "C" int bf_pack_inference(bf_handle h, const float* params, const float* state, void* packed, void* stream)
{
    if (!h) return BF_EINVAL;
    if (!params || !packed || (h->n_state > 0 && !state)) return fail(h, BF_EINVAL, "bf_pack_inference: NULL buffer");
    if ((uintptr_t)packed % 16) return fail(h, BF_EWORKSPACE, "packed buffer must be 16-byte aligned");
    hipStream_t s = (hipStream_t)stream;
    float* pk = (float*)packed;
    const bf_resnet_desc& d = h->d;
    if (d.no_layers > 0 && d.block_convs != 2) {
        hipLaunchKernelGGL(pack_generic_blocks_kernel, dim3(d.no_layers * d.block_convs), dim3(256), 0, s, params, state, h->p_blocks,
                           h->p_block_stride, pk + h->k_blocks, h->k_block_stride, d.block_convs, d.use_bn, d.bn_eps);
        BF_HIP(hipGetLastError(), "pack_generic_blocks");
    } else if (d.no_layers > 0) {
        BF_HIP(bf_launch_pack_all_convs(params, h->p_blocks, h->p_block_stride, pk + h->k_blocks, h->k_block_stride, d.no_layers, 0, 2,
                                        2320, s), "pack_all_convs");
        hipLaunchKernelGGL(fold_bn_kernel, dim3((d.no_layers * 16 + 255) / 256), dim3(256), 0, s, params, state, h->p_blocks,
                           h->p_block_stride, pk, h->k_blocks, h->k_block_stride, d.no_layers, d.use_bn, d.bn_eps);
        BF_HIP(hipGetLastError(), "fold_bn");
        BF_HIP(bf_launch_pack_h3(params, state, h->p_blocks, h->p_block_stride, pk + h->k_h3, BF_H3_BLOCK_FLOATS, d.no_layers,
                                 d.use_bn, d.bn_eps, nullptr, nullptr, s), "pack_h3");
    }
    hipLaunchKernelGGL(pack_edges_kernel, dim3(1), dim3(256), 0, s, params, pk, h->p_base, h->n_base, h->p_head0, h->p_head1,
                       d.head_filters, d.out_channels, h->k_base, h->k_w0, h->k_w1, h->k_wh);
    BF_HIP(hipGetLastError(), "pack_edges");
    return BF_OK;
}

enum class StepKind {
    Pair,
    H3Single,
    Fp32Fused,
    GeneralConvs,
    Unfused,
};
constexpr int STEP_KINDS = 5;

struct ForwardStep {
    int first, blocks;
    int launches;
    StepKind kind;
    H3Kernel h3;
    bool reverse;
    bool head;
    const char* kernel_name() const
    {
        switch (kind) {
        case StepKind::Pair: return "fused_block2_h3w_kernel";
        case StepKind::H3Single: return bf_fused_block_h3_kernel_name(h3);
        case StepKind::Fp32Fused: return bf_fused_block_kernel_name();
        default: return "conv3x3_c16_kernel";
        }
    }
};

struct ForwardPlan {
    int N = 0, block_convs = 2;
    bool h3 = false;
    bool compact = false;
    bool pair_ok = false;
    bool head_in_block = false;
    bool head_in_pair = false;
    int split = 0;
    bool zigzag = false;
    StepKind single_kind = StepKind::H3Single;
    H3Choice single = {H3Kernel::Tiles32, false}, last_single = {H3Kernel::Tiles32, false};
    int launches = 0;
    const char* dominant = "";

    bool head_kernel() const { return !head_in_block && !head_in_pair; }
    ForwardStep next(int i, int launch) const
    {
        ForwardStep st;
        st.first = i; st.blocks = 1; st.launches = 1; st.kind = single_kind; st.h3 = single.kernel; st.reverse = false; st.head = false;
        const bool zz = zigzag && (launch & 1);
        if (pair_ok && i + 1 < N && !(head_in_block && i + 1 == N - 1) && !(i == 0 && (N & 1))) {
            st.blocks = 2; st.kind = StepKind::Pair; st.reverse = zz; st.head = head_in_pair && i + 2 == N;
        } else if (single_kind == StepKind::H3Single) {
            st.head = head_in_block && i == N - 1;
            const H3Choice& c = st.head ? last_single : single;
            st.h3 = c.kernel; st.reverse = zz || c.bottom_up;
        } else if (single_kind == StepKind::GeneralConvs) {
            st.launches = block_convs;
        } else if (single_kind == StepKind::Unfused) {
            st.launches = 2;
        }
        return st;
    }
};

static ForwardPlan make_forward_plan(bf_handle h, int B, int H, int W)
{
    const bf_resnet_desc& d = h->d;
    ForwardPlan p;
    p.N = d.no_layers; p.block_convs = d.block_convs; p.zigzag = h->h3_zigzag != 0;
    p.h3 = h->fused_blocks && h->arith == 1 && d.no_layers > 0 && d.block_convs == 2;
    p.single_kind = d.block_convs != 2 ? StepKind::GeneralConvs
                    : p.h3             ? StepKind::H3Single
                    : h->fused_blocks  ? StepKind::Fp32Fused : StepKind::Unfused;
    if (p.h3) {
        const bool head_fits = d.head_activation == BF_ACT_LINEAR && d.out_channels == 3;
        p.head_in_block = h->fused_head && head_fits;
        const H3Request plain = {B, H, W, h->h3_variant, false, false};
        p.single = bf_select_fused_block_h3(plain);
        p.compact = h->h3_compact && !p.head_in_block && p.single.kernel == H3Kernel::FullRow;
        if (p.compact) p.single = bf_select_fused_block_h3({B, H, W, h->h3_variant, false, true});
        if (p.head_in_block) p.last_single = bf_select_fused_block_h3({B, H, W, 1, true, false});
        p.pair_ok = h->h3_pair && !p.compact && (h->h3_pair == 2 || bf_fused_block_h3_use_pairs(plain)) &&
                    bf_fused_block2_h3w_supports(H, W);
        p.head_in_pair = p.pair_ok && !p.head_in_block && h->h3_pair_head && d.no_layers >= 2 && head_fits;
        p.split = p.compact ? 2 : 1;
    }
    const char* name[STEP_KINDS + 1] = {nullptr, nullptr, nullptr, nullptr, nullptr, nullptr};
    int count[STEP_KINDS + 1] = {0, 0, 0, 0, 0, 0};
    for (int i = 0; i < p.N;) {
        const ForwardStep st = p.next(i, p.launches);
        const char* nm = st.kernel_name();
        for (int k = 0; k < STEP_KINDS + 1; ++k) {
            if (name[k] == nullptr) name[k] = nm;
            if (!strcmp(name[k], nm)) { count[k] += st.blocks > 1 ? st.blocks : st.launches; break; }
        }
        p.launches += st.launches;
        i += st.blocks;
    }
    for (int k = 0, best = 0; k < STEP_KINDS + 1 && name[k]; ++k)
        if (count[k] > best) { best = count[k]; p.dominant = name[k]; }
    return p;
}

static int print_forward_plan(const ForwardPlan& p, char* out, int out_bytes)
{
    int n = snprintf(out, out_bytes, "%s", p.split == 2 ? "compact" : (p.split == 1 ? "split" : "f32"));
    for (int i = 0, launch = 0; i < p.N && n < out_bytes;) {
        const ForwardStep st = p.next(i, launch);
        for (int j = 0; j < st.launches && n < out_bytes; ++j) {
            n += snprintf(out + n, out_bytes - n, " %s:%d", st.kernel_name(), st.first);
            if (n < out_bytes && st.blocks == 2) n += snprintf(out + n, out_bytes - n, "+%d", st.first + 1);
            if (n < out_bytes && st.launches > 1) n += snprintf(out + n, out_bytes - n, ".%d", j);
            if (n < out_bytes && st.kind == StepKind::H3Single && st.h3 == H3Kernel::Tiles16) n += snprintf(out + n, out_bytes - n, ",t16");
            if (n < out_bytes && st.reverse) n += snprintf(out + n, out_bytes - n, ",rev");
            if (n < out_bytes && st.head) n += snprintf(out + n, out_bytes - n, ",head");
        }
        launch += st.launches;
        i += st.blocks;
    }
    if (n < out_bytes && p.head_kernel()) n += snprintf(out + n, out_bytes - n, " head");
    return n < out_bytes ? n : -1;
}

extern "C" int bf_debug_forward_plan(bf_handle h, int B, int H, int W, int pad_pow2, char* out, int out_bytes)
{
    if (!h || !out || out_bytes <= 0) return BF_EINVAL;
    if (B <= 0 || H <= 0 || W <= 0) return fail(h, BF_EINVAL, "batch/height/width must be positive (got %d,%d,%d)", B, H, W);
    const ForwardPlan p = pad_pow2 ? make_forward_plan(h, B, pow2_target(H), pow2_target(W)) : make_forward_plan(h, B, H, W);
    if (print_forward_plan(p, out, out_bytes) < 0) {
        out[0] = 0;
        return fail(h, BF_EINVAL, "bf_debug_forward_plan: the plan does not fit %d bytes", out_bytes);
    }
    return p.launches;
}

struct ForwardRun {
    bf_handle h;
    hipStream_t s;
    const float* pk;
    int B, H, W, Hs, Ws;
    float* buf[3];
    int cur;
    int* status;
    void* out;
    int out_is_u8;
};

static int run_pair(ForwardRun& r, const ForwardStep& st)
{
    bf_handle h = r.h;
    const bf_resnet_desc& d = h->d;
    FusedH3WArgs fa;
    memset(&fa, 0, sizeof(fa));
    fa.in = r.buf[r.cur]; fa.out = r.buf[r.cur ^ 1];
    for (int b = 0; b < 2; ++b) {
        const float* aux = r.pk + h->k_h3 + (int64_t)(st.first + b) * BF_H3_BLOCK_FLOATS;
        fa.aux[b] = aux; fa.w1r[b] = aux + 64; fa.w2r[b] = aux + 64 + BF_H3R_WPACK_FLOATS;
    }
    fa.B = r.B; fa.H = r.H; fa.W = r.W;
    fa.reverse_tiles = st.reverse;
    fa.act1_relu = d.activation == BF_ACT_RELU; fa.zeros = r.pk + h->k_zero; fa.dbg = nullptr;
    if (st.head) {
        fa.head_wh = r.pk + h->k_wh; fa.head_out = r.out; fa.head_u8 = r.out_is_u8; fa.Ho = r.Hs; fa.Wo = r.Ws;
        fa.denormalize = d.denormalize; fa.v_min = d.v_min; fa.v_max = d.v_max; fa.status = r.status;
    }
    BF_HIP(bf_launch_fused_block2_h3w(fa, r.s), "fused_block2_h3w");
    r.cur ^= 1;
    return BF_OK;
}

static int run_h3_single(ForwardRun& r, const ForwardStep& st, bool compact)
{
    bf_handle h = r.h;
    const bf_resnet_desc& d = h->d;
    FusedH3Args fa;
    fa.in = r.buf[r.cur]; fa.out = r.buf[r.cur ^ 1];
    fa.aux = r.pk + h->k_h3 + (int64_t)st.first * BF_H3_BLOCK_FLOATS;
    fa.w1r = fa.aux + 64; fa.w2r = fa.aux + 64 + BF_H3R_WPACK_FLOATS;
    fa.B = r.B; fa.H = r.H; fa.W = r.W; fa.tiles_x = fa.tiles_y = fa.ntiles = 0; fa.rows_per_tile = 0; fa.variant = h->h3_variant;
    fa.reverse_tiles = st.reverse;
    fa.act1_relu = d.activation == BF_ACT_RELU; fa.zeros = r.pk + h->k_zero; fa.dump = (char*)r.status + 1024; fa.dbg = nullptr;
    fa.head_wh = nullptr; fa.head_out = nullptr; fa.head_u8 = 0; fa.Ho = fa.Wo = 0; fa.denormalize = 0;
    fa.v_min = fa.v_max = 0.f; fa.status = nullptr; fa.compact = compact;
    if (st.head) {
        fa.variant = 1;
        fa.head_wh = r.pk + h->k_wh; fa.head_out = r.out; fa.head_u8 = r.out_is_u8; fa.Ho = r.Hs; fa.Wo = r.Ws;
        fa.denormalize = d.denormalize; fa.v_min = d.v_min; fa.v_max = d.v_max; fa.status = r.status;
    }
    BF_HIP(bf_launch_fused_block_h3_as(fa, st.h3, r.s), "fused_block_h3");
    r.cur ^= 1;
    return BF_OK;
}

static int run_fp32_fused(ForwardRun& r, const ForwardStep& st)
{
    bf_handle h = r.h;
    const bf_resnet_desc& d = h->d;
    const float* blk = r.pk + h->k_blocks + st.first * h->k_block_stride;
    FusedBlockArgs fa;
    fa.in = r.buf[r.cur]; fa.out = r.buf[r.cur ^ 1];
    fa.w1pack = blk; fa.w2pack = blk + BF_WPACK_FLOATS;
    fa.scale = blk + 2 * BF_WPACK_FLOATS; fa.shift = fa.scale + 16;
    fa.B = r.B; fa.H = r.H; fa.W = r.W; fa.tiles_x = fa.tiles_y = fa.ntiles = 0;
    fa.act1_relu = d.activation == BF_ACT_RELU; fa.zeros = r.pk + h->k_zero;
    BF_HIP(bf_launch_fused_block(fa, r.s), "fused_block");
    r.cur ^= 1;
    return BF_OK;
}

static int run_general_convs(ForwardRun& r, const ForwardStep& st)
{
    bf_handle h = r.h;
    const bf_resnet_desc& d = h->d;
    const float* blk = r.pk + h->k_blocks + st.first * h->k_block_stride;
    const int cur = r.cur;
    const int nbk = d.block_convs;
    const float* aff = blk + (int64_t)nbk * BF_WPACK_FLOATS;
    int src = cur;
    for (int j = 0; j < nbk; ++j) {
        const bool last = j == nbk - 1;
        int dst = (src + 1) % 3;
        if (dst == cur) dst = (dst + 1) % 3;
        ConvArgs ca;
        memset(&ca, 0, sizeof(ca));
        ca.in = r.buf[src]; ca.out = r.buf[dst]; ca.wpack = blk + (int64_t)j * BF_WPACK_FLOATS; ca.B = r.B; ca.H = r.H; ca.W = r.W;
        ca.scale = aff + j * 32; ca.shift = ca.scale + 16; ca.res = r.buf[cur];
        const bool relu = !last && d.activation == BF_ACT_RELU;
        int epi = (j >= 1 ? EPI_AFFINE : 0) | (relu ? EPI_RELU : 0) | (last ? EPI_RES : 0);
        BF_HIP(bf_launch_conv3x3_c16(ca, epi, r.s), "block conv");
        src = dst;
    }
    r.cur = src;
    return BF_OK;
}

static int run_unfused(ForwardRun& r, const ForwardStep& st)
{
    bf_handle h = r.h;
    const bf_resnet_desc& d = h->d;
    const float* blk = r.pk + h->k_blocks + st.first * h->k_block_stride;
    const int cur = r.cur;
    const int t = (cur + 1) % 3, y = (cur + 2) % 3;
    ConvArgs ca;
    memset(&ca, 0, sizeof(ca));
    ca.in = r.buf[cur]; ca.out = r.buf[t]; ca.wpack = blk; ca.B = r.B; ca.H = r.H; ca.W = r.W;
    BF_HIP(bf_launch_conv3x3_c16(ca, d.activation == BF_ACT_RELU ? EPI_RELU : 0, r.s), "conv1");
    ca.in = r.buf[t]; ca.out = r.buf[y]; ca.wpack = blk + BF_WPACK_FLOATS;
    ca.scale = blk + 2 * BF_WPACK_FLOATS; ca.shift = ca.scale + 16; ca.res = r.buf[cur];
    BF_HIP(bf_launch_conv3x3_c16(ca, EPI_AFFINE | EPI_RES, r.s), "conv2");
    r.cur = y;
    return BF_OK;
}

static int run_step(ForwardRun& r, const ForwardStep& st, const ForwardPlan& p)
{
    switch (st.kind) {
    case StepKind::Pair: return run_pair(r, st);
    case StepKind::H3Single: return run_h3_single(r, st, p.compact);
    case StepKind::Fp32Fused: return run_fp32_fused(r, st);
    case StepKind::GeneralConvs: return run_general_convs(r, st);
    default: return run_unfused(r, st);
    }
}

static int run_forward(bf_handle h, const float* pk, const void* in, int in_is_u8, void* out, int out_is_u8, int B, int Hs,
                          int Ws, int H, int W, void* ws, int64_t ws_bytes, hipStream_t s)
{
    const bf_resnet_desc& d = h->d;
    const int64_t act_bytes = (int64_t)B * H * W * 16 * 4;
    if (!ws || (uintptr_t)ws % 16) return fail(h, BF_EWORKSPACE, "workspace must be a 16-byte aligned device buffer");
    if (ws_bytes < act_bytes * 3 + BF_STATUS_BYTES)
        return fail(h, BF_EWORKSPACE, "workspace too small: %lld < %lld bytes", (long long)ws_bytes,
                    (long long)(act_bytes * 3 + BF_STATUS_BYTES));
    const ForwardPlan p = make_forward_plan(h, B, H, W);
    ForwardRun r;
    r.h = h; r.s = s; r.pk = pk; r.B = B; r.H = H; r.W = W; r.Hs = Hs; r.Ws = Ws;
    r.buf[0] = (float*)ws; r.buf[1] = (float*)((char*)ws + act_bytes); r.buf[2] = (float*)((char*)ws + 2 * act_bytes);
    r.cur = 0;
    r.status = (int*)((char*)ws + (ws_bytes - BF_STATUS_BYTES) / 4 * 4);
    r.out = out; r.out_is_u8 = out_is_u8;

    BaseConvArgs ba;
    ba.in = in; ba.out = r.buf[0]; ba.w = pk + h->k_base;
    ba.B = B; ba.Hs = Hs; ba.Ws = Ws; ba.H = H; ba.W = W; ba.cin = d.in_channels; ba.k = d.kernel_size;
    ba.in_is_u8 = in_is_u8; ba.act_relu = d.base_activation == BF_ACT_RELU;
    ba.v_min = d.v_min; ba.v_max = d.v_max;
    ba.out_split = p.split;
    ba.status = r.status;
    BF_HIP(bf_launch_base_conv(ba, s), "base_conv");

    if (h->timing) BF_HIP(h->timed.begin(s), "hipEventRecord");
    for (int i = 0, launch = 0; i < p.N;) {
        const ForwardStep st = p.next(i, launch);
        const int rc = run_step(r, st, p);
        if (rc != BF_OK) return rc;
        launch += st.launches;
        i += st.blocks;
    }
    if (h->timing) BF_HIP(h->timed.end(s, p.launches, TimingRing::Forward), "hipEventRecord");
    h->block_launches = p.launches;
    h->block_kernel = p.dominant;
    if (!p.head_kernel()) return BF_OK;
    HeadArgs ha;
    ha.feat = r.buf[r.cur];
    ha.w0 = pk + h->k_w0; ha.w1 = pk + h->k_w1;
    ha.wh = d.head_activation == BF_ACT_LINEAR ? pk + h->k_wh : nullptr;
    ha.out = out;
    ha.B = B; ha.H = H; ha.W = W; ha.Ho = Hs; ha.Wo = Ws; ha.hf = d.head_filters; ha.cout = d.out_channels;
    ha.act = d.head_activation; ha.out_is_u8 = out_is_u8; ha.denormalize = d.denormalize;
    ha.v_min = d.v_min; ha.v_max = d.v_max; ha.leaky_alpha = d.leaky_alpha;
    ha.feat_split = p.split;
    ha.status = r.status;
    BF_HIP(bf_launch_head(ha, s), "head");
    return BF_OK;
}

static int check_dims(bf_handle h, const void* packed, const void* in, const void* out, int B, int H, int W)
{
    if (!packed || !in || !out) return fail(h, BF_EINVAL, "NULL tensor pointer");
    if (B <= 0 || H <= 0 || W <= 0) return fail(h, BF_EINVAL, "batch/height/width must be positive (got %d,%d,%d)", B, H, W);
    if ((int64_t)B * H * W * 16 >= ((int64_t)1 << 40)) return fail(h, BF_EINVAL, "tensor too large");
    return BF_OK;
}

extern "C" int bf_forward_u8(bf_handle h, const void* packed, const uint8_t* in, uint8_t* out, int B, int H, int W, void* ws,
                             int64_t ws_bytes, void* stream)
{
    if (!h) return BF_EINVAL;
    int rc = check_dims(h, packed, in, out, B, H, W);
    if (rc) return rc;
    return run_forward(h, (const float*)packed, in, 1, out, 1, B, H, W, pow2_target(H), pow2_target(W), ws, ws_bytes,
                          (hipStream_t)stream);
}

extern "C" int bf_forward_u8_f32(bf_handle h, const void* packed, const uint8_t* in, float* out, int B, int H, int W, void* ws,
                                 int64_t ws_bytes, void* stream)
{
    if (!h) return BF_EINVAL;
    int rc = check_dims(h, packed, in, out, B, H, W);
    if (rc) return rc;
    return run_forward(h, (const float*)packed, in, 1, out, 0, B, H, W, pow2_target(H), pow2_target(W), ws, ws_bytes,
                          (hipStream_t)stream);
}

extern "C" int bf_forward_f32(bf_handle h, const void* packed, const float* in, float* out, int B, int H, int W, void* ws,
                              int64_t ws_bytes, void* stream)
{
    if (!h) return BF_EINVAL;
    int rc = check_dims(h, packed, in, out, B, H, W);
    if (rc) return rc;
    return run_forward(h, (const float*)packed, in, 0, out, 0, B, H, W, H, W, ws, ws_bytes, (hipStream_t)stream);
}
```

### blind_image_denoising_amd/csrc/fused_h3w.hip

```cpp
#include "h3v_core.h"
#include "h3_bands.h"

#ifndef H3W_PRIO_SET
#define H3W_PRIO_SET 0
#endif
#if H3W_PRIO_SET == 1
#define H3W_PRIO_A1 0
#define H3W_PRIO_B1 1
#define H3W_PRIO_A2 2
#define H3W_PRIO_B2 3
#elif H3W_PRIO_SET == 2
#define H3W_PRIO_A1 3
#define H3W_PRIO_B1 2
#define H3W_PRIO_A2 1
#define H3W_PRIO_B2 0
#elif H3W_PRIO_SET == 3
#define H3W_PRIO_A1 0
#define H3W_PRIO_B1 2
#define H3W_PRIO_A2 0
#define H3W_PRIO_B2 2
#elif H3W_PRIO_SET == 4
#define H3W_PRIO_A1 2
#define H3W_PRIO_B1 0
#define H3W_PRIO_A2 2
#define H3W_PRIO_B2 0
#endif
#ifndef H3W_PRIO_A1
#define H3W_PRIO_A1 1
#endif
#ifndef H3W_PRIO_B1
#define H3W_PRIO_B1 1
#endif
#ifndef H3W_PRIO_A2
#define H3W_PRIO_A2 1
#endif
#ifndef H3W_PRIO_B2
#define H3W_PRIO_B2 1
#endif

struct H3WGeom {
    static constexpr int NG = 9, GW = 16 * NG;
    static constexpr int G = 3;
    static constexpr int NR = 3, NW = 12, NT = 768;
    static constexpr int SW = 128;
    static constexpr int PITCH = (GW + 2) * 16;
    static constexpr int NRX0 = 5, NRM = 2, NRX1 = 3, NRO = 2;
    static constexpr int PD = 3;
    static constexpr int UNROLL = 6;
    static constexpr int X0_PLANE = (NRX0 * PITCH + 255) / 256 * 256, M_PLANE = (NRM * PITCH + 255) / 256 * 256;
    static constexpr int X1_PLANE = (NRX1 * PITCH + 255) / 256 * 256;
    static constexpr int OUT_PLANE = GW * 16, OUT_SLOT = 4 * OUT_PLANE;
    static constexpr int X0_OFF = 0, M1_OFF = X0_OFF + 4 * X0_PLANE, X1_OFF = M1_OFF + 4 * M_PLANE, M2_OFF = X1_OFF + 4 * X1_PLANE;
    static constexpr int OUT_OFF = M2_OFF + 4 * M_PLANE, LDS_BYTES = OUT_OFF + NRO * OUT_SLOT;
    static constexpr int LEAD = 12;
    static constexpr int NSTAMP = 4;
    static_assert(UNROLL % NRM == 0 && UNROLL % NRO == 0 && UNROLL % NRX1 == 0 && UNROLL % 3 == 0, "static slots");
    static_assert(NRX0 == PD + 2, "x0 ring: rows s-1 (residual), s (conv1a), s+1 (landed), s+2, s+3 (in flight)");
    static_assert(LDS_BYTES <= 160 * 1024, "LDS");
    static_assert(3 * X0_PLANE + NRX0 * PITCH < 65536, "fragment offsets fit the 16-bit ds offset");
};

struct H3WTile : BandUnit {
    int X0, X1;
    int G0;
    int D0, D1;
};

__device__ __forceinline__ H3WTile h3w_tile(const FusedH3WArgs& a, const int t)
{
    H3WTile r{bf_band_unit<false>(a, t)};
    r.X0 = r.sx * H3WGeom::SW;
    r.X1 = min(a.W, r.X0 + H3WGeom::SW);
    r.G0 = min(max(r.X0 - 8, 0), max(a.W - H3WGeom::GW, 0));
    r.D0 = max(0, (r.X0 - 4) & ~7);
    r.D1 = min(a.W, (r.X1 + 4 + 7) & ~7);
    return r;
}

template <int INP>
struct H3WRoleA {
    using Gm = H3WGeom;
    const char* tin;
    char* tmid;
    h8 w[13];
    f32x4 acc[Gm::G][3];
    int rp, rs;
    int wr;
    float inv_s, relu_floor;
    float lane_scale[Gm::G];
    bool skip_last = false;

    __device__ __forceinline__ void init(const void* wimg, const FusedH3WArgs& a, const float* aux, const int lane, const int gc0)
    {
        const int q = lane >> 4;
#pragma unroll
        for (int i = 0; i < 13; ++i) w[i] = reinterpret_cast<const h8*>(wimg)[bf_band_wimage(a, i) * 64 + lane];
        inv_s = aux[0];
        relu_floor = a.act1_relu ? 0.f : -__builtin_inff();
        rp = (q & 1) * INP + (gc0 + (q >> 1)) * 16;
        rs = ((q & 1) + 2 * (q >> 1)) * INP + (gc0 + 2) * 16;
        wr = (q >> 1) * Gm::M_PLANE + (gc0 + 1) * 16 + (q & 1) * 8;
#pragma unroll
        for (int g = 0; g < Gm::G; ++g)
#pragma unroll
            for (int k = 0; k < 3; ++k) acc[g][k] = (f32x4){0.f, 0.f, 0.f, 0.f};
    }
    __device__ __forceinline__ void set_tile(const H3WTile& t, const int W, const int gc0)
    {
#pragma unroll
        for (int g = 0; g < Gm::G; ++g) lane_scale[g] = (t.G0 + gc0 + 16 * g < W) ? inv_s : 0.f;
    }

    __device__ __forceinline__ H3VFrag load(const int islot_bytes, const int g) const
    {
        H3VFrag f;
        const char* p = tin + rp + islot_bytes;
        f.ph = *reinterpret_cast<const h8*>(p + g * 256);
        f.pl = *reinterpret_cast<const h8*>(p + g * 256 + 2 * INP);
        f.s = *reinterpret_cast<const h8*>(tin + rs + islot_bytes + g * 256);
        return f;
    }

    __device__ __forceinline__ H3VEpi<true> epilogue(const int g, const int mslot, const f32x4 v, const bool rowok) const
    {
        H3VEpi<true> e;
        e.v = v;
        e.sc = rowok ? lane_scale[g] : 0.f;
        e.floor_ = relu_floor;
        e.p = tmid + wr + mslot * Gm::PITCH + g * 256;
        e.lo_off = 2 * Gm::M_PLANE;
        return e;
    }

    template <int J, class Epi>
    __device__ __forceinline__ void mfmas(const int g, const int a1, const int a2, const H3VFrag& cur, f32x4& c0, Epi* epi)
    {
        if constexpr (J < 15) {
            constexpr int k = J / 3, which = J % 3;
            if (!(H3V_ABLATE & 8) && !(skip_last && g == Gm::G - 1)) {
                if constexpr (which == 0) acc[g][a2] = h3v_mfma(cur, w, 2, k, acc[g][a2]);
                else if constexpr (which == 1) acc[g][a1] = h3v_mfma(cur, w, 1, k, acc[g][a1]);
                else c0 = h3v_mfma(cur, w, 0, k, c0);
            } else if (J == 0) {
                acc[g][a2][0] += (float)cur.ph[0] + (float)cur.pl[1] + (float)cur.s[2];
            }
            __builtin_amdgcn_sched_barrier(0);
            if constexpr (J >= 2) {
                if (epi) epi->template pair<J - 2>();
            }
            mfmas<J + 1>(g, a1, a2, cur, c0, epi);
        }
    }

    template <int PH, class Hook>
    __device__ __forceinline__ void step(const int islot_bytes, const bool rowok, Hook& hook)
    {
        constexpr int a0 = PH % 3, a1 = (PH + 2) % 3, a2 = (PH + 1) % 3;
        constexpr int mslot = PH % Gm::NRM;
        H3VFrag cur = load(islot_bytes, 0);
#pragma unroll
        for (int g = 0; g < Gm::G; ++g) {
            H3VFrag nx;
            if (g + 1 < Gm::G) nx = load(islot_bytes, g + 1);
            __builtin_amdgcn_sched_barrier(0);
            f32x4 c0 = {0.f, 0.f, 0.f, 0.f};
            if (g > 0) {
                H3VEpi<true> e = epilogue(g - 1, mslot, acc[g - 1][a2], rowok);
                mfmas<0>(g, a1, a2, cur, c0, &e);
            } else {
                mfmas<0>(g, a1, a2, cur, c0, (H3VEpi<true>*)nullptr);
                hook.after_first_group();
                __builtin_amdgcn_sched_barrier(0);
            }
            acc[g][a0] = c0;
            if (g + 1 < Gm::G) cur = nx;
        }
        H3VEpi<true> e = epilogue(Gm::G - 1, mslot, bf_acc_ready(acc[Gm::G - 1][a2]), rowok);
        e.all();
    }
};

template <int RESP, int OUTP>
struct H3WRoleB {
    using Gm = H3WGeom;
    const char* tmid;
    const char* tres;
    char* tout;
    h8 w[13];
    f32x4 acc[Gm::G][3];
    int rp, rs;
    int rr;
    int wo;
    float inv_s2;
    f32x4 shs;
    float lane_scale[Gm::G];
    bool skip_last = false;

    __device__ __forceinline__ void init(const void* wimg, const FusedH3WArgs& a, const float* aux, const int lane, const int gc0,
                                         const bool out_is_ring)
    {
        const int q = lane >> 4;
#pragma unroll
        for (int i = 0; i < 13; ++i) w[i] = reinterpret_cast<const h8*>(wimg)[bf_band_wimage(a, i) * 64 + lane];
        inv_s2 = aux[48];
        shs = *reinterpret_cast<const f32x4*>(aux + 32 + q * 4) * (1.0f / inv_s2);
        rp = (q & 1) * Gm::M_PLANE + (gc0 + (q >> 1)) * 16;
        rs = ((q & 1) + 2 * (q >> 1)) * Gm::M_PLANE + (gc0 + 2) * 16;
        rr = ((q & 1) + 2 * (q >> 1)) * RESP + (gc0 + 1) * 16;
        wo = (q >> 1) * OUTP + (gc0 + (out_is_ring ? 1 : 0)) * 16 + (q & 1) * 8;
#pragma unroll
        for (int g = 0; g < Gm::G; ++g)
#pragma unroll
            for (int k = 0; k < 3; ++k) acc[g][k] = (f32x4){0.f, 0.f, 0.f, 0.f};
    }
    __device__ __forceinline__ void set_tile(const H3WTile& t, const int W, const int gc0)
    {
#pragma unroll
        for (int g = 0; g < Gm::G; ++g) lane_scale[g] = (t.G0 + gc0 + 16 * g < W) ? inv_s2 : 0.f;
    }

    __device__ __forceinline__ H3VFrag load(const int mslot, const int g) const
    {
        H3VFrag f;
        const int o = mslot * Gm::PITCH + g * 256;
        f.ph = *reinterpret_cast<const h8*>(tmid + rp + o);
        f.pl = *reinterpret_cast<const h8*>(tmid + rp + o + 2 * Gm::M_PLANE);
        f.s = *reinterpret_cast<const h8*>(tmid + rs + o);
        return f;
    }
    __device__ __forceinline__ h8 load_res(const int xslot_bytes, const int g) const
    {
        return *reinterpret_cast<const h8*>(tres + rr + xslot_bytes + g * 256);
    }

    __device__ __forceinline__ H3VEpi<false> epilogue(const int g, const int oslot_bytes, const f32x4 accv, const bool rowok) const
    {
        H3VEpi<false> e;
        e.v = accv;
        e.sc = rowok ? lane_scale[g] : 0.f;
        e.floor_ = 0.f;
        e.p = tout + wo + oslot_bytes + g * 256;
        e.lo_off = 2 * OUTP;
        return e;
    }

    template <int J, class Epi>
    __device__ __forceinline__ void mfmas(const int g, const int a1, const int a2, const H3VFrag& cur, const h8 xr, f32x4& c0, Epi* epi)
    {
        if constexpr (J < 16) {
            if (!(H3V_ABLATE & 4) && !(skip_last && g == Gm::G - 1)) {
                if constexpr (J == 0) {
                    c0 = MFMA_H(w[12], xr, shs);
                } else {
                    constexpr int k = (J - 1) / 3, which = (J - 1) % 3;
                    if constexpr (which == 0) acc[g][a2] = h3v_mfma(cur, w, 2, k, acc[g][a2]);
                    else if constexpr (which == 1) acc[g][a1] = h3v_mfma(cur, w, 1, k, acc[g][a1]);
                    else c0 = h3v_mfma(cur, w, 0, k, c0);
                }
            } else if (J == 0) {
                acc[g][a2][0] += (float)cur.ph[0] + (float)cur.pl[1] + (float)cur.s[2] + (float)xr[3];
            }
            __builtin_amdgcn_sched_barrier(0);
            if constexpr (J >= 2) {
                if (epi) epi->template pair<J - 2>();
            }
            mfmas<J + 1>(g, a1, a2, cur, xr, c0, epi);
        }
    }

    template <int PH, class Hook>
    __device__ __forceinline__ void step(const int xslot_bytes, const int oslot_bytes, const bool rowok, Hook& hook)
    {
        constexpr int mslot = (PH + 1) % Gm::NRM;
        constexpr int a0 = PH % 3, a1 = (PH + 2) % 3, a2 = (PH + 1) % 3;
        H3VFrag cur = load(mslot, 0);
        h8 xr = load_res(xslot_bytes, 0);
#pragma unroll
        for (int g = 0; g < Gm::G; ++g) {
            H3VFrag nx;
            h8 xn;
            if (g + 1 < Gm::G) {
                nx = load(mslot, g + 1);
                xn = load_res(xslot_bytes, g + 1);
            }
            __builtin_amdgcn_sched_barrier(0);
            f32x4 c0;
            if (g > 0) {
                H3VEpi<false> e = epilogue(g - 1, oslot_bytes, acc[g - 1][a2], rowok);
                mfmas<0>(g, a1, a2, cur, xr, c0, &e);
            } else {
                mfmas<0>(g, a1, a2, cur, xr, c0, (H3VEpi<false>*)nullptr);
                hook.after_first_group();
                __builtin_amdgcn_sched_barrier(0);
            }
            acc[g][a0] = c0;
            if (g + 1 < Gm::G) {
                cur = nx;
                xr = xn;
            }
        }
        H3VEpi<false> e = epilogue(Gm::G - 1, oslot_bytes, bf_acc_ready(acc[Gm::G - 1][a2]), rowok);
        e.all();
    }
};

#ifndef H3W_MEM_ROLES
#define H3W_MEM_ROLES 0
#endif
constexpr int h3w_mem_kind(const int role)
{
    constexpr int loader[4] = {2, 0, 1, 3}, storer[4] = {0, 1, 0, 0};
    return role == loader[H3W_MEM_ROLES] ? 1 : (role == storer[H3W_MEM_ROLES] ? 2 : 0);
}

template <int KIND>
struct H3WMem {
    __device__ __forceinline__ H3WMem(const FusedH3WArgs&, char*, const char*, int, unsigned) {}
    __device__ __forceinline__ void set_tile(const H3WTile&, int) {}
    __device__ __forceinline__ void prologue(const H3WTile&) {}
    __device__ __forceinline__ void begin(const H3WTile&, int, int) {}
    __device__ __forceinline__ void after_first_group() {}
    __device__ __forceinline__ void end() {}
    __device__ __forceinline__ void finish() {}
};

template <>
struct H3WMem<1> {
    using Gm = H3WGeom;
    const FusedH3WArgs& a;
    char* tin;
    int piece;
    unsigned plane_g;
    unsigned col_off;
    bool active;
    int dslot;

    __device__ __forceinline__ H3WMem(const FusedH3WArgs& a_, char* tx0, const char*, const int rw, const unsigned pg)
        : a(a_), tin(tx0), piece(rw), plane_g(pg), col_off(0), active(false), dslot(0) {}
    __device__ __forceinline__ void set_tile(const H3WTile& t, const int lane)
    {
        const int c = t.G0 + 64 * piece + lane;
        active = (c >= t.D0) & (c < t.D1) & (64 * piece + lane < Gm::GW);
        col_off = (unsigned)c * 16u;
    }
    __device__ __forceinline__ void dma_row(const H3WTile& t, const int r, const int slot) const
    {
        if (H3V_ABLATE & 1) return;
        const int y = t.y(r - 4);
        const bool ok = (y >= 0) & (y < a.H) & (r < t.nrows + 8);
#pragma unroll
        for (int plane = 0; plane < 4; ++plane) {
            const char* src = ok ? reinterpret_cast<const char*>(a.in) + t.img + (size_t)plane * plane_g + (size_t)y * a.W * 16 + col_off
                                 : reinterpret_cast<const char*>(a.zeros);
            char* dst = tin + plane * Gm::X0_PLANE + slot * Gm::PITCH + (1 + 64 * piece) * 16;
            if (active)
                __builtin_amdgcn_global_load_lds((const __attribute__((address_space(1))) void*)src,
                                                 (__attribute__((address_space(3))) void*)dst, 16, 0, 0);
        }
    }
    static constexpr int INFLIGHT = 2 * 4;
    __device__ __forceinline__ void wait_landed() const { __builtin_amdgcn_s_waitcnt(h3_vmcnt((H3V_ABLATE & 1) ? 0 : INFLIGHT)); }
    __device__ __forceinline__ void prologue(const H3WTile& t)
    {
#pragma unroll
        for (int r = 0; r < Gm::PD; ++r) dma_row(t, r, r);
        wait_landed();
        dslot = Gm::PD;
    }
    __device__ __forceinline__ void begin(const H3WTile& t, const int s, int)
    {
        dma_row(t, s + Gm::PD, dslot);
        dslot = h3v_wrap(dslot + 1, Gm::NRX0);
    }
    __device__ __forceinline__ void after_first_group() {}
    __device__ __forceinline__ void end() { wait_landed(); }
    __device__ __forceinline__ void finish() { __builtin_amdgcn_s_waitcnt(h3_vmcnt(0)); }
};

template <>
struct H3WMem<2> {
    using Gm = H3WGeom;
    const FusedH3WArgs& a;
    const char* tout;
    int first, np;
    unsigned plane_g;
    int st_off[3];
    unsigned g_off[3];
    bool okc[3];
    h8 rec[3];
    bool have;
    char* grow;

    __device__ __forceinline__ H3WMem(const FusedH3WArgs& a_, char*, const char* tout_, const int rw, const unsigned pg)
        : a(a_), tout(tout_), first(3 * rw), np(rw < 2 ? 3 : 2), plane_g(pg), have(false), grow(nullptr) {}
    __device__ __forceinline__ void set_tile(const H3WTile& t, const int lane)
    {
#pragma unroll
        for (int i = 0; i < 3; ++i) {
            const int p = first + i, plane = p >> 1, c = t.X0 + 64 * (p & 1) + lane;
            okc[i] = (i < np) & (c < t.X1);
            st_off[i] = plane * Gm::OUT_PLANE + (c - t.G0) * 16;
            g_off[i] = (unsigned)plane * plane_g + (unsigned)c * 16u;
        }
    }
    __device__ __forceinline__ void prologue(const H3WTile&) {}
    __device__ __forceinline__ void begin(const H3WTile& t, const int s, const int PH)
    {
        const int k = s - Gm::LEAD, oslot = (PH + 1) % Gm::NRO;
        have = (k >= 0) & (k < t.nrows) & !(H3V_ABLATE & 2);
        if (!have) return;
        grow = reinterpret_cast<char*>(a.out) + t.img + (size_t)t.y(k) * a.W * 16;
#pragma unroll
        for (int i = 0; i < 3; ++i)
            if (i < np) rec[i] = *reinterpret_cast<const h8*>(tout + oslot * Gm::OUT_SLOT + st_off[i]);
    }
    __device__ __forceinline__ void after_first_group()
    {
        if (!have) return;
#pragma unroll
        for (int i = 0; i < 3; ++i)
            if (okc[i]) *reinterpret_cast<h8*>(grow + g_off[i]) = rec[i];
    }
    __device__ __forceinline__ void end() {}
    __device__ __forceinline__ void finish() {}
};

template <>
struct H3WMem<3> {
    using Gm = H3WGeom;
    const FusedH3WArgs& a;
    const char* tout;
    int half;
    int st_off;
    int col;
    bool okc;

    __device__ __forceinline__ H3WMem(const FusedH3WArgs& a_, char*, const char* tout_, const int rw, const unsigned)
        : a(a_), tout(tout_), half(rw), st_off(0), col(0), okc(false) {}
    __device__ __forceinline__ void set_tile(const H3WTile& t, const int lane)
    {
        col = t.X0 + 64 * half + lane;
        okc = (half < 2) & (col < t.X1) & (col < a.Wo);
        st_off = (col - t.G0) * 16;
    }
    __device__ __forceinline__ void prologue(const H3WTile&) {}
    __device__ __forceinline__ void begin(const H3WTile& t, const int s, const int PH)
    {
        const int k = s - Gm::LEAD, oslot = (PH + 1) % Gm::NRO;
        bool have = (half < 2) & (k >= 0) & (k < t.nrows) & !(H3V_ABLATE & 2);
        if (have) have = t.y(k) < a.Ho;
        if (!have) return;
        char* orow = reinterpret_cast<char*>(a.head_out) + ((size_t)t.b * a.Ho + (size_t)t.y(k)) * a.Wo * 3 * (a.head_u8 ? 1 : 4);
        const char* src = tout + oslot * Gm::OUT_SLOT + st_off;
        float h0 = 0.f, h1 = 0.f, h2 = 0.f;
#pragma unroll
        for (int hf = 0; hf < 2; ++hf) {
            const h8 hi = *reinterpret_cast<const h8*>(src + hf * Gm::OUT_PLANE), lo = *reinterpret_cast<const h8*>(src + (2 + hf) * Gm::OUT_PLANE);
#pragma unroll
            for (int c = 0; c < 8; ++c) {
                const float v = (float)hi[c] + (float)lo[c];
                const f32x4 w = *reinterpret_cast<const f32x4*>(a.head_wh + (hf * 8 + c) * 4);
                h0 = fmaf(v, w.x, h0);
                h1 = fmaf(v, w.y, h1);
                h2 = fmaf(v, w.z, h2);
            }
        }
        const bool finite = fabsf(h0) <= 3.0e38f && fabsf(h1) <= 3.0e38f && fabsf(h2) <= 3.0e38f;
        if (!finite && a.status) atomicOr(a.status, BF_STATUS_F16_RANGE);
        float r[3] = {h0, h1, h2};
#pragma unroll
        for (int o = 0; o < 3; ++o) {
            float v = (1.0f - 2.0f / (__expf(4.0f * r[o]) + 1.0f)) * 0.51f;
            if (a.denormalize) v = (fminf(fmaxf(v, -0.5f), 0.5f) + 0.5f) * (a.v_max - a.v_min) + a.v_min;
            r[o] = v;
        }
        if (!okc) return;
        if (a.head_u8) {
            unsigned char* p = reinterpret_cast<unsigned char*>(orow) + (size_t)col * 3;
#pragma unroll
            for (int o = 0; o < 3; ++o) p[o] = (unsigned char)fminf(fmaxf(rintf(r[o]), 0.f), 255.f);
        } else {
            float* p = reinterpret_cast<float*>(orow) + (size_t)col * 3;
#pragma unroll
            for (int o = 0; o < 3; ++o) p[o] = r[o];
        }
        __builtin_amdgcn_sched_barrier(0);
    }
    __device__ __forceinline__ void after_first_group() {}
    __device__ __forceinline__ void end() {}
    __device__ __forceinline__ void finish() {}
};

template <bool HEAD>
__global__ __launch_bounds__(H3WGeom::NT, 3) void fused_block2_h3w_kernel(FusedH3WArgs a)
{
    using Gm = H3WGeom;
    extern __shared__ __attribute__((aligned(16))) char h3w_lds[];
    char* tx0 = h3w_lds + Gm::X0_OFF;
    char* tm1 = h3w_lds + Gm::M1_OFF;
    char* tx1 = h3w_lds + Gm::X1_OFF;
    char* tm2 = h3w_lds + Gm::M2_OFF;
    char* tout = h3w_lds + Gm::OUT_OFF;
    const int tid = threadIdx.x, lane = tid & 63;
    const int wave = __builtin_amdgcn_readfirstlane(tid >> 6);
    const int n = lane & 15;
    const int role = wave / Gm::NR, rw = wave - role * Gm::NR;
    const unsigned plane_g = (unsigned)a.H * (unsigned)a.W * 16u;
    const int gc0 = 16 * Gm::G * rw + n;

    for (int i = tid * 16; i < Gm::LDS_BYTES; i += Gm::NT * 16) *reinterpret_cast<f32x4*>(h3w_lds + i) = (f32x4){0.f, 0.f, 0.f, 0.f};
    __syncthreads();

#if H3V_ABLATE & 32
    unsigned long long stamp_sum[Gm::NSTAMP] = {0, 0, 0, 0}, stamp_prev, real0;
    asm volatile("s_memrealtime %0\n\ts_memtime %1\n\ts_waitcnt lgkmcnt(0)" : "=s"(real0), "=s"(stamp_prev)::"memory");
#endif

#define H3W_ROW_IN_IMAGE(k) ((t.y(k) >= 0) & (t.y(k) < a.H))
#define H3W_BAND(R, M, ACTIVE, STEP)                                                                          \
    for (int ti = blockIdx.x; ti < a.ntiles; ti += gridDim.x) {                                               \
        const H3WTile t = h3w_tile(a, ti);                                                                    \
        R.set_tile(t, a.W, gc0);                                                                              \
        M.set_tile(t, lane);                                                                                  \
        M.prologue(t);                                                                                        \
        h3v_barrier();                                                               \
        const int nsteps = t.nrows + Gm::LEAD;                                                                \
        int slot5 = 0;                                                                           \
        for (int s0 = 0; s0 < nsteps; s0 += Gm::UNROLL) {                                                     \
            H3W_ONE(0, M, ACTIVE, STEP); H3W_ONE(1, M, ACTIVE, STEP); H3W_ONE(2, M, ACTIVE, STEP);            \
            H3W_ONE(3, M, ACTIVE, STEP); H3W_ONE(4, M, ACTIVE, STEP); H3W_ONE(5, M, ACTIVE, STEP);            \
        }                                                                                                     \
        M.finish();                                                                                           \
        h3v_barrier();                                                                                        \
    }
#define H3W_ONE(PH, M, ACTIVE, STEP)                                                                          \
    do {                                                                                                      \
        const int s = s0 + PH;                                                                                \
        M.begin(t, s, PH);                                                                                    \
        if (ACTIVE(s)) { STEP(PH); }                                                                          \
        else M.after_first_group();                                                                           \
        slot5 = h3v_wrap(slot5 + 1, Gm::NRX0);                                                                \
        H3V_STAMP(0);                                                                                         \
        M.end();                                                                                              \
        H3V_STAMP(1);                                                                                         \
        h3v_barrier();                                                                                        \
        H3V_STAMP(2);                                                                                         \
    } while (0)

    if (role == 0) {
        __builtin_amdgcn_s_setprio(H3W_PRIO_A1);
        H3WRoleA<Gm::X0_PLANE> R;
        R.tin = tx0; R.tmid = tm1;
        R.init(a.w1r[0], a, a.aux[0], lane, gc0);
        R.skip_last = (H3V_ABLATE & 256) && rw == Gm::NR - 1;
        H3WMem<(HEAD && h3w_mem_kind(0) == 2) ? 3 : h3w_mem_kind(0)> M(a, tx0, tout, rw, plane_g);
        __builtin_amdgcn_s_waitcnt(h3_vmcnt(0));
#define H3W_ACTIVE(s) ((s) < t.nrows + 8)
#define H3W_STEP(PH) R.template step<PH>(slot5 * Gm::PITCH, (s >= 2) & H3W_ROW_IN_IMAGE(s - 5), M)
        H3W_BAND(R, M, H3W_ACTIVE, H3W_STEP)
#undef H3W_ACTIVE
#undef H3W_STEP
    } else if (role == 1) {
        __builtin_amdgcn_s_setprio(H3W_PRIO_B1);
        H3WRoleB<Gm::X0_PLANE, Gm::X1_PLANE> R;
        R.tmid = tm1; R.tres = tx0; R.tout = tx1;
        R.init(a.w2r[0], a, a.aux[0], lane, gc0, true);
        R.skip_last = (H3V_ABLATE & 256) && rw == Gm::NR - 1;
        H3WMem<(HEAD && h3w_mem_kind(1) == 2) ? 3 : h3w_mem_kind(1)> M(a, tx0, tout, rw, plane_g);
        __builtin_amdgcn_s_waitcnt(h3_vmcnt(0));
#define H3W_ACTIVE(s) (((s) >= 3) & ((s) < t.nrows + 9))
#define H3W_STEP(PH) R.template step<PH>(h3v_wrap(slot5 + Gm::NRX0 - 1, Gm::NRX0) * Gm::PITCH, (PH % Gm::NRX1) * Gm::PITCH, H3W_ROW_IN_IMAGE(s - 7), M)
        H3W_BAND(R, M, H3W_ACTIVE, H3W_STEP)
#undef H3W_ACTIVE
#undef H3W_STEP
    } else if (role == 2) {
        __builtin_amdgcn_s_setprio(H3W_PRIO_A2);
        H3WRoleA<Gm::X1_PLANE> R;
        R.tin = tx1; R.tmid = tm2;
        R.init(a.w1r[1], a, a.aux[1], lane, gc0);
        R.skip_last = (H3V_ABLATE & 256) && rw == Gm::NR - 1;
        H3WMem<(HEAD && h3w_mem_kind(2) == 2) ? 3 : h3w_mem_kind(2)> M(a, tx0, tout, rw, plane_g);
        __builtin_amdgcn_s_waitcnt(h3_vmcnt(0));
#define H3W_ACTIVE(s) (((s) >= 6) & ((s) < t.nrows + 10))
#define H3W_STEP(PH) R.template step<PH>(((PH + 2) % Gm::NRX1) * Gm::PITCH, H3W_ROW_IN_IMAGE(s - 9), M)
        H3W_BAND(R, M, H3W_ACTIVE, H3W_STEP)
#undef H3W_ACTIVE
#undef H3W_STEP
    } else {
        __builtin_amdgcn_s_setprio(H3W_PRIO_B2);
        H3WRoleB<Gm::X1_PLANE, Gm::OUT_PLANE> R;
        R.tmid = tm2; R.tres = tx1; R.tout = tout;
        R.init(a.w2r[1], a, a.aux[1], lane, gc0, false);
        R.skip_last = (H3V_ABLATE & 256) && rw == Gm::NR - 1;
        H3WMem<(HEAD && h3w_mem_kind(3) == 2) ? 3 : h3w_mem_kind(3)> M(a, tx0, tout, rw, plane_g);
        __builtin_amdgcn_s_waitcnt(h3_vmcnt(0));
#define H3W_ACTIVE(s) (((s) >= 9) & ((s) < t.nrows + 11))
#define H3W_STEP(PH) R.template step<PH>(((PH + 1) % Gm::NRX1) * Gm::PITCH, (PH % Gm::NRO) * Gm::OUT_SLOT, true, M)
        H3W_BAND(R, M, H3W_ACTIVE, H3W_STEP)
#undef H3W_ACTIVE
#undef H3W_STEP
    }
#undef H3W_BAND
#undef H3W_ONE
#undef H3W_ROW_IN_IMAGE
#if H3V_ABLATE & 32
    {
        unsigned long long real1;
        asm volatile("s_memrealtime %0\n\ts_waitcnt lgkmcnt(0)" : "=s"(real1)::"memory");
        stamp_sum[3] = real1 - real0;
    }
    if (a.dbg && lane == 0) {
        for (int k = 0; k < Gm::NSTAMP; ++k) a.dbg[((size_t)blockIdx.x * Gm::NW + wave) * 8 + k] = stamp_sum[k];
    }
#endif
}

bool bf_fused_block2_h3w_supports(int H, int W) { return W >= 1 && H >= 1; }

hipError_t bf_launch_fused_block2_h3w(const FusedH3WArgs& args, hipStream_t s)
{
    using Gm = H3WGeom;
    FusedH3WArgs a = args;
    if (!a.zeros || !a.in || (!a.out && !a.head_wh) || !bf_fused_block2_h3w_supports(a.H, a.W)) return hipErrorInvalidValue;
    if ((int64_t)a.H * a.W * 64 >= ((int64_t)1 << 32)) return hipErrorInvalidValue;
    const BandPlan p = bf_band_plan(a.B, a.H, (a.W + Gm::SW - 1) / Gm::SW, Gm::LEAD + 2);
    a.nstrips = p.nstrips;
    a.rows_per_tile = p.rows_per_tile;
    a.tiles_y = p.tiles_y;
    a.ntiles = p.ntiles;
    if (a.head_wh && (!a.head_out || a.Ho < 1 || a.Wo < 1 || a.Ho > a.H || a.Wo > a.W)) return hipErrorInvalidValue;
    void (*kernel)(FusedH3WArgs) = a.head_wh ? fused_block2_h3w_kernel<true> : fused_block2_h3w_kernel<false>;
    const hipError_t e = bf_set_max_lds(reinterpret_cast<const void*>(kernel), Gm::LDS_BYTES);
    if (e != hipSuccess) return e;
    hipLaunchKernelGGL(kernel, dim3(p.grid), dim3(Gm::NT), Gm::LDS_BYTES, s, a);
    return hipGetLastError();
}
```

### blind_image_denoising_amd/model.py

```python
import copy
import ctypes as C
import json
import math
import os
from collections import namedtuple
from typing import Dict, List, Optional, Sequence, Union

import numpy as np
import torch

from . import _native as N
from .constants import *
from .custom_logger import logger
from .utilities import input_shape_fixer, load_config

BuilderResults = namedtuple(
    "BuilderResults", ["backbone", "normalizer", "denormalizer", "denoiser", "hydra", "options"])

_ACT = {"linear": N.BF_ACT_LINEAR, "relu": N.BF_ACT_RELU}
_LEAKY = {"leakyrelu": 0.3, "leaky_relu": 0.3, "leakyrelu_01": 0.1, "leaky_relu_01": 0.1,
          "leaky_relu_001": 0.01, "leakyrelu_001": 0.01}
_REG = {None: N.BF_REG_NONE, "l1": N.BF_REG_L1, "l2": N.BF_REG_L2}


def _act_code(name: Optional[str]):
    name = (name or "linear").lower().strip()
    if name in _ACT:
        return _ACT[name], 0.0
    if name in _LEAKY:
        return N.BF_ACT_LEAKY_RELU, _LEAKY[name]
    raise NotImplementedError(f"activation [{name}] is outside the hot path")


def _reg_code(reg):
    if isinstance(reg, str):
        reg = reg.lower().strip()
    if reg not in _REG:
        raise NotImplementedError(
            f"regularizer [{reg}]: only the keras strings 'l1' / 'l2' are on the hot path")
    return _REG[reg]


def describe_resnet(config: Dict, strict_snapshot: bool = False) -> N.ResnetDesc:
    config_backbone = copy.deepcopy(config[BACKBONE_STR])
    config_denoiser = copy.deepcopy(config[DENOISER_STR])
    model_type = config_backbone[TYPE_STR].strip().lower()
    if model_type == "convnext":
        raise NotImplementedError(
            f"backbone [{model_type}] is outside the MI355X hot path (resnet, unet and unet_laplacian only)")
    if model_type in ("unet", "unet_laplacian"):
        raise ValueError(f"{model_type} models are described by blind_image_denoising_amd."
                         f"{'unet_backbone' if model_type == 'unet' else 'unet_laplacian'}")
    if model_type == "efficientnet":
        raise NotImplementedError("efficientnet not implemented yet")
    if model_type != "resnet":
        raise ValueError("don't know how to build model [{0}]".format(model_type))

    value_range = config_backbone.get("value_range", (0, 255))
    input_shape = input_shape_fixer(config_backbone.get(INPUT_SHAPE_STR, (None, None, 1)))
    block_kernels = list(config_backbone.get("block_kernels", [3, 3]))
    block_filters = list(config_backbone.get("block_filters", [32, 32]))
    kernel_regularizer = config_backbone.get("kernel_regularizer", "l1")
    block_regularizer = config_backbone.get("block_regularizer") or [kernel_regularizer] * len(block_kernels)
    activation = config_backbone.get("activation", "relu")
    block_activation = config_backbone.get("block_activation") or [activation] * len(block_kernels)
    block_depthwise = config_backbone.get("block_depthwise") or [-1] * len(block_kernels)
    block_groups = config_backbone.get("block_groups") or [1] * len(block_kernels)

    if len(block_kernels) <= 0:
        raise ValueError("len(block_kernels) must be >= 0 ")
    if len(block_kernels) > 3:
        raise ValueError("len(block_kernels) must be <= 3")
    if len(block_filters) <= 0:
        raise ValueError("len(block_filters) must be >= 0 ")
    if len(block_kernels) != len(block_filters):
        raise ValueError("len(block_filters) must == len(block_kernels)")
    if len(block_kernels) != len(block_groups):
        raise ValueError("len(block_filters) must == len(block_groups)")
    if len(block_regularizer) != len(block_groups):
        raise ValueError("len(block_regularizer) must == len(block_groups)")
    if len(block_activation) != len(block_groups):
        raise ValueError("len(block_activation) must == len(block_groups)")
    if len(block_depthwise) != len(block_kernels):
        raise ValueError("len(block_depthwise) must == len(block_kernels)")

    unsupported = [k for k in ("add_gelu", "add_gates", "add_final_bn", "add_initial_bn",
                               "add_concat_input", "add_gradient_dropout", "add_channelwise_scaling",
                               "add_learnable_multiplier", "add_mean_sigma_normalization")
                   if config_backbone.get(k, False)]
    if config_backbone.get("selector_params") is not None:
        unsupported.append("selector_params")
    if config_backbone.get("dropout_rate", -1) != -1:
        unsupported.append("dropout_rate")
    if any(d != -1 for d in block_depthwise):
        unsupported.append("block_depthwise")
    if any(g != 1 for g in block_groups):
        unsupported.append("block_groups")
    if config_backbone.get(USE_BIAS, False) or config_denoiser.get(USE_BIAS, False):
        unsupported.append("use_bias")
    if config_denoiser.get("use_bn", False) or config_denoiser.get("use_ln", False):
        unsupported.append("denoiser use_bn/use_ln")
    if unsupported:
        raise NotImplementedError(f"resnet options outside the hot path: {unsupported}")
    if len(set(block_kernels)) != 1 or len(set(block_filters)) != 1 or \
            block_filters[0] != config_backbone["filters"]:
        raise NotImplementedError("block_kernels / block_filters must be uniform and equal to `filters`")
    if len(set(block_regularizer)) != 1:
        raise NotImplementedError("block_regularizer must be uniform")

    d = N.ResnetDesc()
    d.struct_size = C.sizeof(N.ResnetDesc)
    d.in_channels = int(input_shape[-1])
    d.filters = int(config_backbone["filters"])
    d.kernel_size = int(config_backbone["kernel_size"])
    d.no_layers = int(config_backbone["no_layers"])
    d.block_convs = len(block_kernels)
    d.block_kernel = int(block_kernels[0])
    d.activation, alpha0 = _act_code(block_activation[0])
    d.base_activation, _ = _act_code(config_backbone.get("base_activation", "linear"))
    d.use_bn = 1 if config_backbone.get("use_bn", True) else 0
    d.head_filters = int(config_denoiser.get("filters", 32))
    d.head_activation, alpha1 = _act_code(config_denoiser.get("activation", "linear"))
    d.out_channels = int(config_denoiser.get("output_channels", 3))
    d.denormalize = 0 if strict_snapshot else 1
    d.reg_base = _reg_code(kernel_regularizer)
    d.reg_block = _reg_code(block_regularizer[0])
    d.reg_head = _reg_code(config_denoiser.get(KERNEL_REGULARIZER, "l2"))
    d.v_min, d.v_max = float(value_range[0]), float(value_range[1])
    d.bn_eps, d.bn_momentum = DEFAULT_BN_EPSILON, DEFAULT_BN_MOMENTUM
    d.leaky_alpha = alpha1 or alpha0
    return d


def glorot_normal(shape: Sequence[int], rng: np.random.Generator) -> np.ndarray:
    kh, kw, ci, co = shape
    std = math.sqrt(2.0 / (kh * kw * ci + kh * kw * co)) / 0.87962566103423978
    w = rng.standard_normal(shape)
    bad = np.abs(w) > 2.0
    while bad.any():
        w[bad] = rng.standard_normal(int(bad.sum()))
        bad = np.abs(w) > 2.0
    return (w * std).astype(np.float32)


class Variable:

    def __init__(self, name, tensor, kind, regularizer, offset):
        self.name, self.tensor, self.kind, self.regularizer, self.offset = name, tensor, kind, regularizer, offset

    @property
    def shape(self):
        return tuple(self.tensor.shape)

    def numpy(self):
        return self.tensor.detach().cpu().numpy()

    def __repr__(self):
        return f"<Variable {self.name} {self.shape}>"


class HydraModel:

    name = "hydra"

    def __init__(self, config: Dict, device: Optional[Union[str, torch.device]] = None,
                 strict_snapshot: bool = False, seed: Optional[int] = None):
        self.config = copy.deepcopy(config)
        self.desc = describe_resnet(config, strict_snapshot)
        self._lib = N.lib()
        handle = C.c_void_p()
        N.check(self._lib.bf_create(C.byref(self.desc), C.byref(handle)), None, "model_builder")
        self._h = handle
        if device is None:
            device = torch.device("cuda", torch.cuda.current_device()) if torch.cuda.is_available() \
                else torch.device("cpu")
        self.device = torch.device(device)
        self.n_params = int(self._lib.bf_param_count(self._h))
        self.n_state = int(self._lib.bf_state_count(self._h))
        self._infos, self._state_infos = self._tensor_infos(0), self._tensor_infos(1)
        params, state = self._initial_values(seed)
        self.params = torch.from_numpy(params).to(self.device)
        self.state = torch.from_numpy(state).to(self.device)
        self._packed = None
        self._packed_dirty = True
        self.version = 0
        self._workspace = None
        self.outputs = [None]
        self.inputs = [None]

    def __del__(self):
        try:
            if getattr(self, "_h", None):
                self._lib.bf_destroy(self._h)
                self._h = None
        except Exception:
            pass

    def _tensor_infos(self, state: int):
        out = []
        ti = N.TensorInfo()
        for i in range(self._lib.bf_tensor_count(self._h, state)):
            N.check(self._lib.bf_tensor_at(self._h, state, i, C.byref(ti)), self._h)
            out.append((ti.name.decode(), int(ti.offset), tuple(ti.shape[:ti.rank]), int(ti.kind),
                        int(ti.regularizer)))
        return out

    def _initial_values(self, seed):
        rng = np.random.default_rng(seed)
        params = np.empty(self.n_params, np.float32)
        for name, off, shape, kind, _ in self._infos:
            n = int(np.prod(shape))
            params[off:off + n] = glorot_normal(shape, rng).ravel() if kind == 0 else 1.0
        state = np.empty(self.n_state, np.float32)
        for name, off, shape, kind, _ in self._state_infos:
            state[off:off + int(np.prod(shape))] = 0.0 if kind == 2 else 1.0
        return params, state

    @property
    def trainable_variables(self) -> List[Variable]:
        return [Variable(n, self.params[o:o + int(np.prod(s))].view(*s), k, r, o)
                for n, o, s, k, r in self._infos]

    @property
    def non_trainable_variables(self) -> List[Variable]:
        return [Variable(n, self.state[o:o + int(np.prod(s))].view(*s), k, r, o)
                for n, o, s, k, r in self._state_infos]

    def count_params(self) -> int:
        return self.n_params + self.n_state

    def get_weights(self):
        return self.params.detach().cpu().numpy().copy(), self.state.detach().cpu().numpy().copy()

    def set_weights(self, params: np.ndarray, state: Optional[np.ndarray] = None):
        params = np.ascontiguousarray(params, np.float32).ravel()
        if params.size != self.n_params:
            raise ValueError(f"expected {self.n_params} parameters, got {params.size}")
        self.params.copy_(torch.from_numpy(params))
        if state is not None:
            state = np.ascontiguousarray(state, np.float32).ravel()
            if state.size != self.n_state:
                raise ValueError(f"expected {self.n_state} state values, got {state.size}")
            self.state.copy_(torch.from_numpy(state))
        self.mark_dirty()

    def mark_dirty(self):
        self._packed_dirty = True
        self.version = getattr(self, "version", 0) + 1

    def _require_gpu(self):
        if self.device.type != "cuda":
            raise RuntimeError("this model lives on the CPU: the engine has no CPU execution path "
                               "(construct it with a cuda device on an MI355X)")

    def workspace(self, mode: int, batch: int, height: int, width: int) -> torch.Tensor:
        need = int(self._lib.bf_workspace_bytes(self._h, mode, batch, height, width))
        if need < 0:
            raise ValueError("invalid workspace query")
        if self._workspace is None or self._workspace.numel() < need:
            self._workspace = None
            self._workspace = torch.empty(need, dtype=torch.uint8, device=self.device)
        return self._workspace

    def packed(self) -> torch.Tensor:
        if self._packed is None:
            self._packed = torch.empty(int(self._lib.bf_packed_bytes(self._h)), dtype=torch.uint8, device=self.device)
        if self._packed_dirty:
            N.check(self._lib.bf_pack_inference(self._h, N.ptr(self.params), N.ptr(self.state), N.ptr(self._packed),
                                                N.stream_ptr(self.params)), self._h, "bf_pack_inference")
            self._packed_dirty = False
        return self._packed

    def set_option(self, key: str, value: int):
        self.version = getattr(self, "version", 0) + 1
        if self.device.type == "cuda":
            with torch.cuda.device(self.device):
                N.check(self._lib.bf_set_option(self._h, key.encode(), int(value)), self._h)
        else:
            N.check(self._lib.bf_set_option(self._h, key.encode(), int(value)), self._h)

    def block_kernel(self):
        import ctypes as C
        n = C.c_int()
        name = self._lib.bf_get_block_kernel(self._h, C.byref(n))
        return (name.decode() if name else ""), int(n.value)

    def forward_plan(self, batch: int, height: int, width: int, pad_pow2: bool = True):
        import ctypes as C
        buf = C.create_string_buffer(1 << 14)
        n = self._lib.bf_debug_forward_plan(self._h, int(batch), int(height), int(width), int(bool(pad_pow2)), buf, len(buf))
        N.check(n if n < 0 else 0, self._h, "bf_debug_forward_plan")
        return buf.value.decode(), int(n)

    def _as_device(self, x, dtype):
        was_numpy = isinstance(x, np.ndarray)
        if was_numpy:
            x = torch.from_numpy(np.ascontiguousarray(x))
        if not isinstance(x, torch.Tensor):
            raise ValueError("input must be a torch.Tensor or numpy array")
        if x.dim() != 4:
            raise ValueError(f"input must be rank 4 [B,H,W,C], got shape {tuple(x.shape)}")
        if x.shape[-1] != self.desc.in_channels:
            raise ValueError(f"expected {self.desc.in_channels} channels, got {x.shape[-1]}")
        x = x.to(device=self.device, dtype=dtype).contiguous()
        return x, was_numpy

    def __call__(self, x, training: bool = False):
        if isinstance(x, (list, tuple)):
            if len(x) != 1:
                raise ValueError("hydra takes one input tensor")
            x = x[0]
        self._require_gpu()
        x, was_numpy = self._as_device(x, torch.float32)
        B, H, W, _ = x.shape
        if training:
            out = self.training_forward(x)
        else:
            out = torch.empty((B, H, W, self.desc.out_channels), dtype=torch.float32, device=self.device)
            ws = self.workspace(N.BF_MODE_INFERENCE, B, H, W)
            N.check(self._lib.bf_forward_f32(self._h, N.ptr(self.packed()), N.ptr(x), N.ptr(out), B, H, W,
                                             N.ptr(ws), ws.numel(), N.stream_ptr(x)), self._h, "bf_forward_f32")
            if was_numpy and not self.check_status(raise_on_overflow=not self.auto_exact_fallback):
                logger.warning("activations exceed the f16 range: switching this model to the exact-fp32 kernels (arith = 0)")
                self.set_option("arith", 0)
                return self(x, training=False).cpu().numpy()
        return out.cpu().numpy() if was_numpy else out

    auto_exact_fallback = True

    def status_tensor(self) -> Optional[torch.Tensor]:
        ws = self._workspace
        if ws is None:
            return None
        off = (ws.numel() - N.BF_STATUS_BYTES) // 4 * 4
        return ws[off:off + 4].view(torch.int32)

    def check_status(self, raise_on_overflow: bool = True) -> bool:
        ws = self._workspace
        if ws is None:
            return True
        n = ws.numel()
        off = (n - N.BF_STATUS_BYTES) // 4 * 4
        status = int(ws[off:off + 4].view(torch.int32).item())
        if status & N.BF_STATUS_F16_RANGE:
            if raise_on_overflow:
                raise FloatingPointError("an activation left the f16 range (|x| >= 65504) inside the split-f16 residual "
                                         "blocks; call set_option('arith', 0) to run the exact-fp32 kernels")
            return False
        return True

    def predict(self, x):
        return self(x, training=False)

    def infer_u8(self, image: torch.Tensor, cast_to_uint8: bool = True) -> torch.Tensor:
        self._require_gpu()
        B, H, W, _ = image.shape
        out = torch.empty((B, H, W, self.desc.out_channels), dtype=torch.uint8 if cast_to_uint8 else torch.float32, device=self.device)
        ws = self.workspace(N.BF_MODE_INFERENCE, B, H, W)
        fn = self._lib.bf_forward_u8 if cast_to_uint8 else self._lib.bf_forward_u8_f32
        N.check(fn(self._h, N.ptr(self.packed()), N.ptr(image), N.ptr(out), B, H, W,
                                        N.ptr(ws), ws.numel(), N.stream_ptr(image)), self._h, "bf_forward_u8")
        return out

    def train_forward_backward(self, gt: torch.Tensor, noisy: torch.Tensor, loss_desc: N.LossDesc,
                               grads: torch.Tensor, losses: torch.Tensor, want_predictions: bool = True):
        self._require_gpu()
        B, H, W, _ = noisy.shape
        pred = torch.empty((B, H, W, self.desc.out_channels), dtype=torch.float32, device=self.device) \
            if want_predictions else None
        ws = self.workspace(N.BF_MODE_TRAIN, B, H, W)
        N.check(self._lib.bf_train_step(self._h, N.ptr(self.params), N.ptr(self.state), N.ptr(gt), N.ptr(noisy),
                                        B, H, W, C.byref(loss_desc), N.ptr(pred), N.ptr(grads), N.ptr(losses),
                                        N.ptr(ws), ws.numel(), N.stream_ptr(noisy)), self._h, "bf_train_step")
        self.mark_dirty()
        return pred

    def training_forward(self, x: torch.Tensor) -> torch.Tensor:
        ld = N.LossDesc()
        ld.struct_size = C.sizeof(N.LossDesc)
        ld.hinge, ld.cutoff, ld.mae_multiplier, ld.regularization, ld.depth_weight = 0.0, 255.0, 1.0, 0.0, 1.0
        grads = torch.empty(self.n_params, dtype=torch.float32, device=self.device)
        losses = torch.empty(N.BF_LOSS_COUNT, dtype=torch.float32, device=self.device)
        if self.desc.in_channels != self.desc.out_channels:
            raise NotImplementedError("training needs in_channels == output_channels")
        return self.train_forward_backward(x, x, ld, grads, losses, True)

    @property
    def losses(self):
        self._require_gpu()
        regs = [v for v in self.trainable_variables if v.regularizer in (N.BF_REG_L1, N.BF_REG_L2)]
        vals = torch.zeros(max(len(regs), 1), dtype=torch.float32, device=self.device)
        for k, v in enumerate(regs):
            N.check(self._lib.bf_op_reg_elementwise(N.ptr(v.tensor.reshape(-1)), None, v.tensor.numel(), v.regularizer, 0.01, 0.0,
                                                    N.ptr(vals[k:k + 1]), N.stream_ptr(vals)), None, "bf_op_reg_elementwise")
        return [vals[k] for k in range(len(regs))]


def _normalize_op(x, lo: float, hi: float, inverse: int):
    if not isinstance(x, torch.Tensor) or x.device.type != "cuda":
        raise RuntimeError("normalize / denormalize need a GPU tensor: there is no CPU execution path")
    x = x.to(torch.float32).contiguous()
    out = torch.empty_like(x)
    N.check(N.lib().bf_op_normalize(N.ptr(x), N.ptr(out), x.numel(), lo, hi, inverse, N.stream_ptr(x)), None, "bf_op_normalize")
    return out


def build_normalize_model(input_dims=None, min_value: float = 0.0, max_value: float = 255.0, name: str = "normalize"):
    lo, hi = float(min_value), float(max_value)

    def normalize(x, training=False):
        return _normalize_op(x, lo, hi, 0)
    normalize.name = name
    return normalize


def build_denormalize_model(input_dims=None, min_value: float = 0.0, max_value: float = 255.0, name: str = "denormalize"):
    lo, hi = float(min_value), float(max_value)

    def denormalize(y, training=False):
        return _normalize_op(y, lo, hi, 1)
    denormalize.name = name
    return denormalize


class _SubModelView:

    def __init__(self, name: str, hydra: HydraModel, prefixes):
        self.name, self._hydra, self._prefixes = name, hydra, prefixes
        self.outputs = [None]

    @property
    def trainable_variables(self):
        return [v for v in self._hydra.trainable_variables if v.name.startswith(self._prefixes)]


def _build_hydra(config: Dict, device=None, strict_snapshot: bool = False, seed: Optional[int] = None):
    btype = str(config[BACKBONE_STR].get(TYPE_STR, "")).strip().lower()
    if btype == "unet_laplacian":
        from .unet_laplacian import UnetLaplacianHydra
        return UnetLaplacianHydra(config, device=device, seed=seed)
    if btype == "unet":
        from .unet_backbone import UnetHydra
        return UnetHydra(config, device=device, seed=seed)
    try:
        return HydraModel(config, device=device, strict_snapshot=strict_snapshot, seed=seed)
    except NotImplementedError as first:
        if btype != "resnet":
            raise
        from .resnet_generic import GenericResnetHydra
        try:
            return GenericResnetHydra(config, device=device, seed=seed)
        except NotImplementedError as second:
            raise NotImplementedError(f"{first}; generic resnet path: {second}") from None


def model_builder(config: Dict, device=None, strict_snapshot: bool = False, seed: Optional[int] = None) -> BuilderResults:
    hydra = _build_hydra(config, device, strict_snapshot, seed)
    if not isinstance(hydra, HydraModel):
        outs = getattr(hydra, "depth", 1) if getattr(hydra, "multi_output", False) else 1
        logger.warning(f"Backbone model has [{outs}] outputs, probably of different scale or depth")
        return BuilderResults(
            backbone=None, denoiser=None, hydra=hydra, options={},
            normalizer=build_normalize_model(min_value=hydra.v_min, max_value=hydra.v_max),
            denormalizer=build_denormalize_model(min_value=hydra.v_min, max_value=hydra.v_max))
    vr = config[BACKBONE_STR].get("value_range", (0, 255))
    logger.warning(f"Backbone model has [1] outputs, probably of different scale or depth")
    return BuilderResults(
        backbone=_SubModelView(f"resnet_backbone", hydra, ("base/", "block")),
        normalizer=build_normalize_model(min_value=vr[0], max_value=vr[1]),
        denormalizer=build_denormalize_model(min_value=vr[0], max_value=vr[1]),
        denoiser=_SubModelView("denoiser_head", hydra, ("head/",)),
        hydra=hydra,
        options={})



def save_model(hydra: HydraModel, directory: str, pipeline_config: Optional[Dict] = None) -> None:
    os.makedirs(directory, exist_ok=True)
    cfg = copy.deepcopy(pipeline_config) if pipeline_config else {MODEL_STR: hydra.config}
    cfg.setdefault(MODEL_STR, hydra.config)
    if not isinstance(hydra, HydraModel):
        with open(os.path.join(directory, PIPELINE_FILE_STR), "w") as f:
            json.dump(cfg, f, indent=4)
        tv = hydra.trainable_variables
        w = hydra.get_weights()
        params, state = w if isinstance(w, tuple) else (w, np.zeros(0, np.float32))
        np.savez(os.path.join(directory, WEIGHTS_FILE_STR), params=params, state=state,
                 names=np.array([v[0] for v in tv]), offsets=np.array([v[3] for v in tv]))
        return
    cfg["strict_snapshot"] = not bool(hydra.desc.denormalize)
    with open(os.path.join(directory, PIPELINE_FILE_STR), "w") as f:
        json.dump(cfg, f, indent=4)
    params, state = hydra.get_weights()
    np.savez(os.path.join(directory, WEIGHTS_FILE_STR), params=params, state=state,
             names=np.array([i[0] for i in hydra._infos]), offsets=np.array([i[1] for i in hydra._infos]))


def load_hydra(directory: str, device=None) -> HydraModel:
    cfg_path = os.path.join(directory, PIPELINE_FILE_STR)
    w_path = os.path.join(directory, WEIGHTS_FILE_STR)
    if not os.path.isfile(cfg_path) or not os.path.isfile(w_path):
        raise ValueError(f"model_path [{directory}] does not hold {PIPELINE_FILE_STR} + {WEIGHTS_FILE_STR}")
    cfg = load_config(cfg_path)
    hydra = _build_hydra(cfg[MODEL_STR], device, bool(cfg.get("strict_snapshot", False)))
    if not isinstance(hydra, HydraModel):
        with np.load(w_path) as z:
            if getattr(hydra, "n_state", 0):
                hydra.set_weights(z["params"], z["state"])
            else:
                hydra.set_weights(z["params"])
        return hydra
    with np.load(w_path) as z:
        hydra.set_weights(z["params"], z["state"])
    return hydra
```

### include/bfcnn_hip_debug.h

```cpp
#ifndef BFCNN_HIP_DEBUG_H
#define BFCNN_HIP_DEBUG_H
#include "bfcnn_hip.h"
#ifdef __cplusplus
extern "C" {
#endif

int bf_debug_conv3x3(const float* in, const float* w_hwio, float* out, const float* scale, const float* shift,
                     const float* res, const float* mask, float* stats, float* wpack_scratch,
                     int batch, int height, int width, int epi, int transpose_flip, void* stream);
int bf_debug_conv3x3_grid(int batch, int height, int width);
int bf_debug_fused_block(const float* in, const float* w1_hwio, const float* w2_hwio, const float* scale,
                         const float* shift, float* out, float* wpack_scratch,
                         int batch, int height, int width, int act1_relu, void* stream);
int64_t bf_debug_fused_block_h3_scratch_floats(int batch, int height, int width);
int bf_debug_fused_block_h3(const float* in, const float* w1_hwio, const float* w2_hwio, const float* scale,
                            const float* shift, float* out, float* scratch,
                            int batch, int height, int width, int act1_relu, void* stream);
int64_t bf_debug_fused_block2_h3_scratch_floats(int batch, int height, int width);
int bf_debug_fused_block2_h3(const float* in, const float* w_hwio, const float* scale, const float* shift, float* out,
                             float* scratch, int batch, int height, int width, int act1_relu, int reverse, void* stream);
int bf_debug_set_h3_variant(int variant);
int64_t bf_debug_conv3x3_h3_scratch_floats(void);
int bf_debug_conv3x3_h3(const float* in, const float* w_hwio, float* out, const float* res, const float* mask, float* stats,
                        float* scratch, int batch, int height, int width, int epi, int transpose_flip, void* stream);
int64_t bf_debug_wgrad_partial_floats(int batch, int height, int width);
int bf_debug_wgrad3x3(const float* x, const float* dy, float* partial, float* dw,
                      int batch, int height, int width, void* stream);
int bf_debug_wgrad3x3_h3(const float* x, const float* dy, float* partial, float* dw,
                         int batch, int height, int width, void* stream);
int bf_debug_conv3x3_h3_pre(const float* in, const float* pre_c, const float* pre_scale, const float* pre_shift, float* pre_out,
                            const float* w_hwio, float* out, float* scratch, int batch, int height, int width, int relu,
                            int reverse, void* stream);
int64_t bf_debug_fwd_block_h3t_scratch_floats(int batch, int height, int width);
int bf_debug_fwd_block_h3t(const float* x, const float* pre_c, const float* pre_scale, const float* pre_shift, const float* w0_hwio,
                           const float* w1_hwio, float* a_out, float* t_out, float* c_out, float* stats, float* scratch, int batch,
                           int height, int width, int relu, int reverse, void* stream);
int64_t bf_debug_bwd_block_h3t_scratch_floats(int batch, int height, int width);
int bf_debug_bwd_block_h3t(const float* a, const float* g, const float* c, const float* coef, const float* w0_hwio, const float* w1_hwio,
                           const float* bnc, float* out, float* dw1, float* dw0, float* stats, float* scratch, int batch, int height,
                           int width, int relu, int reverse, void* stream);
int64_t bf_debug_bwd3x3_h3_scratch_floats(int batch, int height, int width);
int bf_debug_bwd3x3_h3_grid(int batch, int height, int width);
int bf_debug_bwd3x3_h3_grid_ex(int batch, int height, int width, int dbuf);
int bf_debug_bwd3x3_h3(const float* x, const float* g, const float* c, const float* coef, const float* w_hwio, float* out,
                       const float* res, const float* bnc, float* dw, float* stats, float* scratch, int batch, int height,
                       int width, int epi, int reverse, int repack, void* stream);
int bf_debug_forward_plan(bf_handle h, int batch, int height, int width, int pad_pow2, char* out, int out_bytes);
float bf_debug_h3_weight_scale(float max_abs);
int bf_debug_mfma_probe(const float* a, const float* b, float* d, void* stream);
int bf_debug_set_upsample_band(int on);

#ifdef __cplusplus
}
#endif
#endif
```

Measured before the change: 29670.

## Fuse base conv into first fused resblock pair kernel as in-band producer

When the first forward step is a non-reversed, non-head block pair and the row-based base conv would otherwise run, the base 3x3 conv on u8 input is now computed inside the fused block2 kernel. Producer waves fetch raw pixels into an LDS ring and run MFMA to fill the layer-0 input tile directly. This removes a separate launch and the full-resolution round trip of the base output through global memory. In exchange it uses more LDS and adds producer work to consumer waves, which may lower occupancy or unbalance roles. XCD-aware tile ordering is also switched on by default.

```diff
diff --git a/blind_image_denoising_amd/_native.py b/blind_image_denoising_amd/_native.py
--- a/blind_image_denoising_amd/_native.py
+++ b/blind_image_denoising_amd/_native.py
@@ -203,6 +203,7 @@
     "bf_debug_bwd3x3_h3_grid_ex": (_I, [_I, _I, _I, _I]),
     "bf_debug_bwd3x3_h3": (_I, [_P, _P, _P, _P, _P, _P, _P, _P, _P, _P, _P, _I, _I, _I, _I, _I, _I, _P]),
     "bf_debug_forward_plan": (_I, [_P, _I, _I, _I, _I, C.c_char_p, _I]),
+    "bf_debug_base_path": (_I, [_P, _I, _I, _I, _I, _I]),
     "bf_debug_mfma_probe": (_I, [_P, _P, _P, _P]),
 }
 
diff --git a/blind_image_denoising_amd/csrc/base_rows.h b/blind_image_denoising_amd/csrc/base_rows.h
--- /dev/null
+++ b/blind_image_denoising_amd/csrc/base_rows.h
@@ -0,0 +1,53 @@
+#pragma once
+#include "bf_common.h"
+#include "h3_core.h"
+#include "h3_weights.h"
+
+__device__ __forceinline__ float br_wval(const float* __restrict__ w, const int tap, const int c, const int m)
+{
+    if (c < 3) return w[(tap * 3 + c) * 16 + m] / 255.0f;
+    return -0.5f * (w[(tap * 3 + 0) * 16 + m] + w[(tap * 3 + 1) * 16 + m] + w[(tap * 3 + 2) * 16 + m]);
+}
+
+__device__ __forceinline__ float br_weight_scale(const float* __restrict__ w, float* red)
+{
+    return bf_h3_block_weight_scale<256>([&](const int i) { return br_wval(w, i / 64, (i >> 4) & 3, i & 15); }, 9 * 4 * 16, red);
+}
+
+__device__ __forceinline__ h8 br_operand(const float* __restrict__ w, const float s, const int dy, const int lane)
+{
+    const int n = lane & 15, q = lane >> 4;
+    h8 r;
+#pragma unroll
+    for (int j = 0; j < 8; ++j) {
+        const int slot = 8 * (q & 1) + j, dx = slot >> 2, c = slot & 3;
+        float v = 0.f;
+        if (dx < 3) v = br_wval(w, dy * 3 + dx, c, n) * s;
+        _Float16 hi, lo;
+        bf_h3_split(v, hi, lo);
+        r[j] = (q >> 1) ? lo : hi;
+    }
+    return r;
+}
+
+struct BrPixel {
+    bool inside, colour;
+};
+__device__ __forceinline__ BrPixel br_pixel(const int yy, const int x, const int H, const int W, const int Hs, const int Ws)
+{
+    BrPixel p;
+    p.inside = yy >= 0 && yy < H && x >= 0 && x < W;
+    p.colour = p.inside && yy < Hs && x < Ws;
+    return p;
+}
+__device__ __forceinline__ h4 br_record(const BrPixel p, const unsigned r, const unsigned g, const unsigned b)
+{
+    h4 v = {(_Float16)0.f, (_Float16)0.f, (_Float16)0.f, (_Float16)0.f};
+    if (p.inside) v[3] = (_Float16)1.f;
+    if (p.colour) {
+        v[0] = (_Float16)(float)r;
+        v[1] = (_Float16)(float)g;
+        v[2] = (_Float16)(float)b;
+    }
+    return v;
+}
diff --git a/blind_image_denoising_amd/csrc/base_rows.hip b/blind_image_denoising_amd/csrc/base_rows.hip
--- a/blind_image_denoising_amd/csrc/base_rows.hip
+++ b/blind_image_denoising_amd/csrc/base_rows.hip
@@ -1,6 +1,4 @@
-#include "bf_common.h"
-#include "h3_core.h"
-#include "h3_weights.h"
+#include "base_rows.h"
 #include <cstdlib>
 
 constexpr int BR_NT = 256, BR_CW = 256, BR_RING = 4, BR_ROWPX = BR_CW + 4;
@@ -13,25 +11,11 @@
     if (a.status && blockIdx.x == 0 && tid == 0) *a.status = 0;
     const float* __restrict__ w = a.w;
 
-    auto wval = [&](const int tap, const int c, const int m) -> float {
-        if (c < 3) return w[(tap * 3 + c) * 16 + m] / 255.0f;
-        return -0.5f * (w[(tap * 3 + 0) * 16 + m] + w[(tap * 3 + 1) * 16 + m] + w[(tap * 3 + 2) * 16 + m]);
-    };
-    const float s = bf_h3_block_weight_scale<BR_NT>([&](const int i) { return wval(i / 64, (i >> 4) & 3, i & 15); }, 9 * 4 * 16, red);
+    const float s = br_weight_scale(w, red);
     const float inv_s = 1.0f / s;
     h8 wa[3];
 #pragma unroll
-    for (int dy = 0; dy < 3; ++dy) {
-#pragma unroll
-        for (int j = 0; j < 8; ++j) {
-            const int slot = 8 * (q & 1) + j, dx = slot >> 2, c = slot & 3;
-            float v = 0.f;
-            if (dx < 3) v = wval(dy * 3 + dx, c, n) * s;
-            _Float16 hi, lo;
-            bf_h3_split(v, hi, lo);
-            wa[dy][j] = (q >> 1) ? lo : hi;
-        }
-    }
+    for (int dy = 0; dy < 3; ++dy) wa[dy] = br_operand(w, s, dy, lane);
 
     int bx = blockIdx.x;
     const int ch = bx % nchunks; bx /= nchunks;
diff --git a/blind_image_denoising_amd/csrc/bf_common.h b/blind_image_denoising_amd/csrc/bf_common.h
--- a/blind_image_denoising_amd/csrc/bf_common.h
+++ b/blind_image_denoising_amd/csrc/bf_common.h
@@ -169,6 +169,9 @@
     int head_u8, Ho, Wo, denormalize;
     float v_min, v_max;
     int* status;
+    const void* base_u8;
+    const float* base_w;
+    int Hs, Ws, base_relu;
 };
 hipError_t bf_launch_fused_block2_h3w(const FusedH3WArgs& a, hipStream_t s);
 bool       bf_fused_block2_h3w_supports(int H, int W);
@@ -272,6 +275,7 @@
     int* status;
 };
 hipError_t bf_launch_base_conv(const BaseConvArgs& a, hipStream_t s);
+bool       bf_base_conv_runs_rows(const BaseConvArgs& a);
 bool       bf_base_conv_rows_supports(const BaseConvArgs& a);
 hipError_t bf_launch_base_conv_rows(const BaseConvArgs& a, hipStream_t s);
 void       bf_set_base_conv_rows(int on);
diff --git a/blind_image_denoising_amd/csrc/edge_layers.hip b/blind_image_denoising_amd/csrc/edge_layers.hip
--- a/blind_image_denoising_amd/csrc/edge_layers.hip
+++ b/blind_image_denoising_amd/csrc/edge_layers.hip
@@ -111,9 +111,14 @@
     return (int64_t)a.B * a.H * nchunks >= 8192 && (int64_t)a.W * 5 >= nchunks * 256 * 3;
 }
 
+bool bf_base_conv_runs_rows(const BaseConvArgs& a)
+{
+    return g_base_rows && bf_base_conv_rows_supports(a) && (g_base_rows == 2 || base_rows_preferred(a));
+}
+
 hipError_t bf_launch_base_conv(const BaseConvArgs& a, hipStream_t s)
 {
-    if (g_base_rows && bf_base_conv_rows_supports(a) && (g_base_rows == 2 || base_rows_preferred(a))) return bf_launch_base_conv_rows(a, s);
+    if (bf_base_conv_runs_rows(a)) return bf_launch_base_conv_rows(a, s);
 #define BF_BASE(C, KK) if (a.cin == C && a.k == KK) return launch_base<C, KK>(a, s);
     BF_BASE(3, 3) BF_BASE(3, 5) BF_BASE(3, 7) BF_BASE(3, 1)
     BF_BASE(1, 3) BF_BASE(1, 5) BF_BASE(1, 7) BF_BASE(1, 1)
diff --git a/blind_image_denoising_amd/csrc/engine.h b/blind_image_denoising_amd/csrc/engine.h
--- a/blind_image_denoising_amd/csrc/engine.h
+++ b/blind_image_denoising_amd/csrc/engine.h
@@ -43,6 +43,7 @@
     int h3_compact = 0;
     int h3_pair = 1;
     int h3_pair_head = 0;
+    int h3_pair_base = 1;
     int block_launches = 0;
     const char* block_kernel = "";
     std::string train_kernels;
diff --git a/blind_image_denoising_amd/csrc/engine.hip b/blind_image_denoising_amd/csrc/engine.hip
--- a/blind_image_denoising_amd/csrc/engine.hip
+++ b/blind_image_denoising_amd/csrc/engine.hip
@@ -147,6 +147,7 @@
     if (!strcmp(key, "h3_pair")) { h->h3_pair = value == 2 ? 2 : (value ? 1 : 0); return BF_OK; }
     if (!strcmp(key, "base_rows")) { bf_set_base_conv_rows(value); return BF_OK; }
     if (!strcmp(key, "h3_pair_head")) { h->h3_pair_head = value ? 1 : 0; return BF_OK; }
+    if (!strcmp(key, "h3_pair_base")) { h->h3_pair_base = value ? 1 : 0; return BF_OK; }
     if (!strcmp(key, "fused_head")) { h->fused_head = value ? 1 : 0; return BF_OK; }
     if (!strcmp(key, "train_zigzag")) { h->train_zigzag = value ? 1 : 0; return BF_OK; }
     if (!strcmp(key, "train_fused_fwd")) { h->train_fused_fwd = value ? 1 : 0; return BF_OK; }
diff --git a/blind_image_denoising_amd/csrc/engine_infer.hip b/blind_image_denoising_amd/csrc/engine_infer.hip
--- a/blind_image_denoising_amd/csrc/engine_infer.hip
+++ b/blind_image_denoising_amd/csrc/engine_infer.hip
@@ -260,7 +260,42 @@
     int* status;
     void* out;
     int out_is_u8;
+    const BaseConvArgs* base;
 };
+
+enum BasePath { BaseVector = 0, BaseRows = 1, BaseInPair = 2 };
+
+static BasePath base_path(bf_handle h, const ForwardPlan& p, const BaseConvArgs& ba)
+{
+    if (!bf_base_conv_runs_rows(ba)) return BaseVector;
+    if (h->h3_pair_base && p.N > 0) {
+        const ForwardStep st = p.next(0, 0);
+        if (st.kind == StepKind::Pair && !st.head && !st.reverse) return BaseInPair;
+    }
+    return BaseRows;
+}
+
+static BaseConvArgs base_conv_args(bf_handle h, const ForwardPlan& p, int B, int Hs, int Ws, int H, int W, int in_is_u8)
+{
+    const bf_resnet_desc& d = h->d;
+    BaseConvArgs ba;
+    ba.in = nullptr; ba.out = nullptr; ba.w = nullptr;
+    ba.B = B; ba.Hs = Hs; ba.Ws = Ws; ba.H = H; ba.W = W; ba.cin = d.in_channels; ba.k = d.kernel_size;
+    ba.in_is_u8 = in_is_u8; ba.act_relu = d.base_activation == BF_ACT_RELU;
+    ba.v_min = d.v_min; ba.v_max = d.v_max;
+    ba.out_split = p.split;
+    ba.status = nullptr;
+    return ba;
+}
+
+extern "C" int bf_debug_base_path(bf_handle h, int B, int H, int W, int pad_pow2, int in_is_u8)
+{
+    if (!h) return BF_EINVAL;
+    if (B <= 0 || H <= 0 || W <= 0) return fail(h, BF_EINVAL, "batch/height/width must be positive (got %d,%d,%d)", B, H, W);
+    const int Hp = pad_pow2 ? pow2_target(H) : H, Wp = pad_pow2 ? pow2_target(W) : W;
+    const ForwardPlan p = make_forward_plan(h, B, Hp, Wp);
+    return base_path(h, p, base_conv_args(h, p, B, H, W, Hp, Wp, in_is_u8 != 0));
+}
 
 static int run_pair(ForwardRun& r, const ForwardStep& st)
 {
@@ -279,6 +314,10 @@
     if (st.head) {
         fa.head_wh = r.pk + h->k_wh; fa.head_out = r.out; fa.head_u8 = r.out_is_u8; fa.Ho = r.Hs; fa.Wo = r.Ws;
         fa.denormalize = d.denormalize; fa.v_min = d.v_min; fa.v_max = d.v_max; fa.status = r.status;
+    }
+    if (r.base && st.first == 0) {
+        fa.in = nullptr; fa.base_u8 = r.base->in; fa.base_w = r.base->w; fa.Hs = r.base->Hs; fa.Ws = r.base->Ws;
+        fa.base_relu = r.base->act_relu; fa.status = r.status;
     }
     BF_HIP(bf_launch_fused_block2_h3w(fa, r.s), "fused_block2_h3w");
     r.cur ^= 1;
@@ -396,14 +435,11 @@
     r.status = (int*)((char*)ws + (ws_bytes - BF_STATUS_BYTES) / 4 * 4);
     r.out = out; r.out_is_u8 = out_is_u8;
 
-    BaseConvArgs ba;
+    BaseConvArgs ba = base_conv_args(h, p, B, Hs, Ws, H, W, in_is_u8);
     ba.in = in; ba.out = r.buf[0]; ba.w = pk + h->k_base;
-    ba.B = B; ba.Hs = Hs; ba.Ws = Ws; ba.H = H; ba.W = W; ba.cin = d.in_channels; ba.k = d.kernel_size;
-    ba.in_is_u8 = in_is_u8; ba.act_relu = d.base_activation == BF_ACT_RELU;
-    ba.v_min = d.v_min; ba.v_max = d.v_max;
-    ba.out_split = p.split;
     ba.status = r.status;
-    BF_HIP(bf_launch_base_conv(ba, s), "base_conv");
+    r.base = base_path(h, p, ba) == BaseInPair ? &ba : nullptr;
+    if (!r.base) BF_HIP(bf_launch_base_conv(ba, s), "base_conv");
 
     if (h->timing) BF_HIP(h->timed.begin(s), "hipEventRecord");
     for (int i = 0, launch = 0; i < p.N;) {
diff --git a/blind_image_denoising_amd/csrc/fused_h3w.hip b/blind_image_denoising_amd/csrc/fused_h3w.hip
--- a/blind_image_denoising_amd/csrc/fused_h3w.hip
+++ b/blind_image_denoising_amd/csrc/fused_h3w.hip
@@ -1,5 +1,6 @@
 #include "h3v_core.h"
 #include "h3_bands.h"
+#include "base_rows.h"
 
 #ifndef H3W_PRIO_SET
 #define H3W_PRIO_SET 0
@@ -38,6 +39,10 @@
 #define H3W_PRIO_B2 1
 #endif
 
+#ifndef H3W_XCD_ORDER
+#define H3W_XCD_ORDER 1
+#endif
+
 struct H3WGeom {
     static constexpr int NG = 9, GW = 16 * NG;
     static constexpr int G = 3;
@@ -52,6 +57,11 @@
     static constexpr int OUT_PLANE = GW * 16, OUT_SLOT = 4 * OUT_PLANE;
     static constexpr int X0_OFF = 0, M1_OFF = X0_OFF + 4 * X0_PLANE, X1_OFF = M1_OFF + 4 * M_PLANE, M2_OFF = X1_OFF + 4 * X1_PLANE;
     static constexpr int OUT_OFF = M2_OFF + 4 * M_PLANE, LDS_BYTES = OUT_OFF + NRO * OUT_SLOT;
+    static constexpr int BIN_RING = 4, BIN_ROWPX = GW + 4;
+    static constexpr int BIN_SLOT = 2 * BIN_ROWPX * 8;
+    static constexpr int BIN_OFF = LDS_BYTES, BWA_OFF = BIN_OFF + BIN_RING * BIN_SLOT, BINVS_OFF = BWA_OFF + 3 * 64 * 16;
+    static constexpr int BRED_OFF = BINVS_OFF + 16, LDS_BYTES_BASE = BRED_OFF + NT * 4;
+    static_assert(LDS_BYTES_BASE <= 160 * 1024 && BIN_OFF % 16 == 0 && BIN_SLOT % 16 == 0 && LDS_BYTES_BASE % 16 == 0, "LDS (producer)");
     static constexpr int LEAD = 12;
     static constexpr int NSTAMP = 4;
     static_assert(UNROLL % NRM == 0 && UNROLL % NRO == 0 && UNROLL % NRX1 == 0 && UNROLL % 3 == 0, "static slots");
@@ -68,7 +78,7 @@
 
 __device__ __forceinline__ H3WTile h3w_tile(const FusedH3WArgs& a, const int t)
 {
-    H3WTile r{bf_band_unit<false>(a, t)};
+    H3WTile r{bf_band_unit<H3W_XCD_ORDER != 0>(a, t)};
     r.X0 = r.sx * H3WGeom::SW;
     r.X1 = min(a.W, r.X0 + H3WGeom::SW);
     r.G0 = min(max(r.X0 - 8, 0), max(a.W - H3WGeom::GW, 0));
@@ -491,7 +501,149 @@
     __device__ __forceinline__ void finish() {}
 };
 
-template <bool HEAD>
+#ifndef H3W_BASE_SPREAD
+#define H3W_BASE_SPREAD 1
+#endif
+constexpr int h3w_base_groups(const int role)
+{
+    return H3W_BASE_SPREAD == 0 ? (role == 2 ? 3 : 0) : (H3W_BASE_SPREAD == 1 ? (role >= 1 ? 1 : 0) : (role <= 2 ? 1 : 0));
+}
+constexpr int h3w_base_first_group(const int role, const int rw)
+{
+    return H3W_BASE_SPREAD == 0 ? 3 * rw : (H3W_BASE_SPREAD == 1 ? 3 * (role - 1) + rw : 3 * role + rw);
+}
+constexpr bool h3w_base_fetches(const int role) { return role == 2; }
+
+template <int NGW, bool FETCH>
+struct H3WProducer {
+    using Gm = H3WGeom;
+    const FusedH3WArgs& a;
+    char* tx0;
+    char* tring;
+    const char* twa;
+    int g0, fw;
+    float inv_s, floor_;
+    int wr;
+    int fo;
+    int col0;
+    int px, xcol;
+    const uint8_t* img;
+    unsigned raw[3];
+    BrPixel rawp;
+    int dslot;
+
+    __device__ __forceinline__ H3WProducer(const FusedH3WArgs& a_, char* lds, const int g0_, const int fw_)
+        : a(a_), tx0(lds + Gm::X0_OFF), tring(lds + Gm::BIN_OFF), twa(lds + Gm::BWA_OFF), g0(g0_), fw(fw_), wr(0), fo(0), col0(0),
+          px(0), xcol(0), img(nullptr), raw{0u, 0u, 0u}, rawp{false, false}, dslot(0)
+    {
+        inv_s = *reinterpret_cast<const float*>(lds + Gm::BINVS_OFF);
+        floor_ = a.base_relu ? 0.f : -__builtin_inff();
+    }
+    __device__ __forceinline__ void set_tile(const H3WTile& t, const int lane)
+    {
+        const int n = lane & 15, q = lane >> 4, gc0 = 16 * g0 + n;
+        wr = (q >> 1) * Gm::X0_PLANE + (gc0 + 1) * 16 + (q & 1) * 8;
+        const int p = gc0 + 2 * (q & 1);
+        fo = ((p & 1) * Gm::BIN_ROWPX + (p & ~1)) * 8;
+        twa = tx0 - Gm::X0_OFF + Gm::BWA_OFF + lane * 16;
+        col0 = t.G0 + gc0;
+        px = 64 * fw + lane;
+        xcol = t.G0 - 1 + px;
+        img = reinterpret_cast<const uint8_t*>(a.base_u8) + (size_t)t.b * a.Hs * a.Ws * 3;
+    }
+    __device__ __forceinline__ void request(const H3WTile& t, const int u)
+    {
+        const int yy = t.ybase + u - 5;
+        const bool need = (px < Gm::GW + 2) & (u <= t.nrows + 9);
+        rawp = br_pixel(yy, xcol, a.H, a.W, a.Hs, a.Ws);
+        rawp.inside &= need;
+        rawp.colour &= need;
+        if (rawp.colour) {
+            const uint8_t* p = img + ((size_t)yy * a.Ws + xcol) * 3;
+            raw[0] = p[0];
+            raw[1] = p[1];
+            raw[2] = p[2];
+        }
+    }
+    __device__ __forceinline__ void commit(const int u)
+    {
+        if (px >= Gm::GW + 2) return;
+        const h4 v = br_record(rawp, raw[0], raw[1], raw[2]);
+        h4* row = reinterpret_cast<h4*>(tring + (u & (Gm::BIN_RING - 1)) * Gm::BIN_SLOT);
+        row[px] = v;
+        if (px > 0) row[Gm::BIN_ROWPX + px - 1] = v;
+    }
+    __device__ __forceinline__ void produce(const H3WTile& t, const int r, const int slot)
+    {
+        if (r >= t.nrows + 8) return;
+        const int y = t.y(r - 4);
+        const bool rowok = (y >= 0) & (y < a.H);
+        f32x4 acc[NGW];
+#pragma unroll
+        for (int g = 0; g < NGW; ++g) acc[g] = (f32x4){0.f, 0.f, 0.f, 0.f};
+#pragma unroll
+        for (int dy = 0; dy < 3; ++dy) {
+            const h8 wa = *reinterpret_cast<const h8*>(twa + dy * 64 * 16);
+            const char* row = tring + ((r + dy) & (Gm::BIN_RING - 1)) * Gm::BIN_SLOT + fo;
+#pragma unroll
+            for (int g = 0; g < NGW; ++g) acc[g] = MFMA_H(wa, *reinterpret_cast<const h8*>(row + g * 128), acc[g]);
+        }
+#pragma unroll
+        for (int g = 0; g < NGW; ++g) {
+            H3VEpi<true> e;
+            e.v = bf_acc_ready(acc[g]);
+            e.sc = (rowok & (col0 + 16 * g < a.W)) ? inv_s : 0.f;
+            e.floor_ = floor_;
+            e.p = tx0 + wr + slot * Gm::PITCH + g * 256;
+            e.lo_off = 2 * Gm::X0_PLANE;
+            e.all();
+        }
+    }
+    __device__ __forceinline__ void fill(const H3WTile& t)
+    {
+        if constexpr (FETCH) {
+#pragma unroll
+            for (int u = 0; u < Gm::BIN_RING; ++u) {
+                request(t, u);
+                commit(u);
+            }
+            request(t, Gm::BIN_RING);
+        }
+    }
+    __device__ __forceinline__ void prologue(const H3WTile& t)
+    {
+        produce(t, 0, 0);
+        dslot = 1;
+    }
+    __device__ __forceinline__ void begin(const H3WTile& t, const int s)
+    {
+        if constexpr (FETCH) {
+            commit(s + 4);
+            request(t, s + 5);
+        }
+        produce(t, s + 1, dslot);
+        dslot = h3v_wrap(dslot + 1, Gm::NRX0);
+        __builtin_amdgcn_sched_barrier(0);
+    }
+};
+
+template <>
+struct H3WProducer<0, false> {
+    __device__ __forceinline__ H3WProducer(const FusedH3WArgs&, char*, int, int) {}
+    __device__ __forceinline__ void set_tile(const H3WTile&, int) {}
+    __device__ __forceinline__ void fill(const H3WTile&) {}
+    __device__ __forceinline__ void prologue(const H3WTile&) {}
+    __device__ __forceinline__ void begin(const H3WTile&, int) {}
+};
+
+template <bool HEAD, bool BASE>
+constexpr int h3w_hook_kind(const int role)
+{
+    const int k = h3w_mem_kind(role);
+    return (HEAD && k == 2) ? 3 : ((BASE && k == 1) ? 0 : k);
+}
+
+template <bool HEAD, bool BASE>
 __global__ __launch_bounds__(H3WGeom::NT, 3) void fused_block2_h3w_kernel(FusedH3WArgs a)
 {
     using Gm = H3WGeom;
@@ -508,8 +660,20 @@
     const unsigned plane_g = (unsigned)a.H * (unsigned)a.W * 16u;
     const int gc0 = 16 * Gm::G * rw + n;
 
-    for (int i = tid * 16; i < Gm::LDS_BYTES; i += Gm::NT * 16) *reinterpret_cast<f32x4*>(h3w_lds + i) = (f32x4){0.f, 0.f, 0.f, 0.f};
+    if (BASE && a.status && blockIdx.x == 0 && tid == 0) *a.status = 0;
+    for (int i = tid * 16; i < (BASE ? Gm::LDS_BYTES_BASE : Gm::LDS_BYTES); i += Gm::NT * 16)
+        *reinterpret_cast<f32x4*>(h3w_lds + i) = (f32x4){0.f, 0.f, 0.f, 0.f};
     __syncthreads();
+    if constexpr (BASE) {
+        const float bs = br_weight_scale(a.base_w, reinterpret_cast<float*>(h3w_lds + Gm::BRED_OFF));
+        if (wave == 0) {
+#pragma unroll
+            for (int dy = 0; dy < 3; ++dy)
+                *reinterpret_cast<h8*>(h3w_lds + Gm::BWA_OFF + (dy * 64 + lane) * 16) = br_operand(a.base_w, bs, dy, lane);
+            if (lane == 0) *reinterpret_cast<float*>(h3w_lds + Gm::BINVS_OFF) = 1.0f / bs;
+        }
+        __syncthreads();
+    }
 
 #if H3V_ABLATE & 32
     unsigned long long stamp_sum[Gm::NSTAMP] = {0, 0, 0, 0}, stamp_prev, real0;
@@ -517,25 +681,32 @@
 #endif
 
 #define H3W_ROW_IN_IMAGE(k) ((t.y(k) >= 0) & (t.y(k) < a.H))
-#define H3W_BAND(R, M, ACTIVE, STEP)                                                                          \
+#define H3W_BAND(R, M, P, ACTIVE, STEP)                                                                         \
     for (int ti = blockIdx.x; ti < a.ntiles; ti += gridDim.x) {                                               \
         const H3WTile t = h3w_tile(a, ti);                                                                    \
         R.set_tile(t, a.W, gc0);                                                                              \
         M.set_tile(t, lane);                                                                                  \
+        P.set_tile(t, lane);                                                                                  \
+        if constexpr (BASE) {                                      \
+            P.fill(t);                                                                                        \
+            h3v_barrier();                                                                                    \
+        }                                                                                                     \
+        P.prologue(t);                                                                                        \
         M.prologue(t);                                                                                        \
-        h3v_barrier();                                                               \
+        h3v_barrier();                                                 \
         const int nsteps = t.nrows + Gm::LEAD;                                                                \
         int slot5 = 0;                                                                           \
         for (int s0 = 0; s0 < nsteps; s0 += Gm::UNROLL) {                                                     \
-            H3W_ONE(0, M, ACTIVE, STEP); H3W_ONE(1, M, ACTIVE, STEP); H3W_ONE(2, M, ACTIVE, STEP);            \
-            H3W_ONE(3, M, ACTIVE, STEP); H3W_ONE(4, M, ACTIVE, STEP); H3W_ONE(5, M, ACTIVE, STEP);            \
+            H3W_ONE(0, M, P, ACTIVE, STEP); H3W_ONE(1, M, P, ACTIVE, STEP); H3W_ONE(2, M, P, ACTIVE, STEP);   \
+            H3W_ONE(3, M, P, ACTIVE, STEP); H3W_ONE(4, M, P, ACTIVE, STEP); H3W_ONE(5, M, P, ACTIVE, STEP);   \
         }                                                                                                     \
         M.finish();                                                                                           \
         h3v_barrier();                                                                                        \
     }
-#define H3W_ONE(PH, M, ACTIVE, STEP)                                                                          \
+#define H3W_ONE(PH, M, P, ACTIVE, STEP)                                                                         \
     do {                                                                                                      \
         const int s = s0 + PH;                                                                                \
+        P.begin(t, s);                                                                                        \
         M.begin(t, s, PH);                                                                                    \
         if (ACTIVE(s)) { STEP(PH); }                                                                          \
         else M.after_first_group();                                                                           \
@@ -553,11 +724,12 @@
         R.tin = tx0; R.tmid = tm1;
         R.init(a.w1r[0], a, a.aux[0], lane, gc0);
         R.skip_last = (H3V_ABLATE & 256) && rw == Gm::NR - 1;
-        H3WMem<(HEAD && h3w_mem_kind(0) == 2) ? 3 : h3w_mem_kind(0)> M(a, tx0, tout, rw, plane_g);
+        H3WMem<h3w_hook_kind<HEAD, BASE>(0)> M(a, tx0, tout, rw, plane_g);
+        H3WProducer<BASE ? h3w_base_groups(0) : 0, BASE && h3w_base_groups(0) && h3w_base_fetches(0)> P(a, h3w_lds, h3w_base_first_group(0, rw), rw);
         __builtin_amdgcn_s_waitcnt(h3_vmcnt(0));
 #define H3W_ACTIVE(s) ((s) < t.nrows + 8)
 #define H3W_STEP(PH) R.template step<PH>(slot5 * Gm::PITCH, (s >= 2) & H3W_ROW_IN_IMAGE(s - 5), M)
-        H3W_BAND(R, M, H3W_ACTIVE, H3W_STEP)
+        H3W_BAND(R, M, P, H3W_ACTIVE, H3W_STEP)
 #undef H3W_ACTIVE
 #undef H3W_STEP
     } else if (role == 1) {
@@ -566,11 +738,12 @@
         R.tmid = tm1; R.tres = tx0; R.tout = tx1;
         R.init(a.w2r[0], a, a.aux[0], lane, gc0, true);
         R.skip_last = (H3V_ABLATE & 256) && rw == Gm::NR - 1;
-        H3WMem<(HEAD && h3w_mem_kind(1) == 2) ? 3 : h3w_mem_kind(1)> M(a, tx0, tout, rw, plane_g);
+        H3WMem<h3w_hook_kind<HEAD, BASE>(1)> M(a, tx0, tout, rw, plane_g);
+        H3WProducer<BASE ? h3w_base_groups(1) : 0, BASE && h3w_base_groups(1) && h3w_base_fetches(1)> P(a, h3w_lds, h3w_base_first_group(1, rw), rw);
         __builtin_amdgcn_s_waitcnt(h3_vmcnt(0));
 #define H3W_ACTIVE(s) (((s) >= 3) & ((s) < t.nrows + 9))
 #define H3W_STEP(PH) R.template step<PH>(h3v_wrap(slot5 + Gm::NRX0 - 1, Gm::NRX0) * Gm::PITCH, (PH % Gm::NRX1) * Gm::PITCH, H3W_ROW_IN_IMAGE(s - 7), M)
-        H3W_BAND(R, M, H3W_ACTIVE, H3W_STEP)
+        H3W_BAND(R, M, P, H3W_ACTIVE, H3W_STEP)
 #undef H3W_ACTIVE
 #undef H3W_STEP
     } else if (role == 2) {
@@ -579,11 +752,12 @@
         R.tin = tx1; R.tmid = tm2;
         R.init(a.w1r[1], a, a.aux[1], lane, gc0);
         R.skip_last = (H3V_ABLATE & 256) && rw == Gm::NR - 1;
-        H3WMem<(HEAD && h3w_mem_kind(2) == 2) ? 3 : h3w_mem_kind(2)> M(a, tx0, tout, rw, plane_g);
+        H3WMem<h3w_hook_kind<HEAD, BASE>(2)> M(a, tx0, tout, rw, plane_g);
+        H3WProducer<BASE ? h3w_base_groups(2) : 0, BASE && h3w_base_groups(2) && h3w_base_fetches(2)> P(a, h3w_lds, h3w_base_first_group(2, rw), rw);
         __builtin_amdgcn_s_waitcnt(h3_vmcnt(0));
 #define H3W_ACTIVE(s) (((s) >= 6) & ((s) < t.nrows + 10))
 #define H3W_STEP(PH) R.template step<PH>(((PH + 2) % Gm::NRX1) * Gm::PITCH, H3W_ROW_IN_IMAGE(s - 9), M)
-        H3W_BAND(R, M, H3W_ACTIVE, H3W_STEP)
+        H3W_BAND(R, M, P, H3W_ACTIVE, H3W_STEP)
 #undef H3W_ACTIVE
 #undef H3W_STEP
     } else {
@@ -592,11 +766,12 @@
         R.tmid = tm2; R.tres = tx1; R.tout = tout;
         R.init(a.w2r[1], a, a.aux[1], lane, gc0, false);
         R.skip_last = (H3V_ABLATE & 256) && rw == Gm::NR - 1;
-        H3WMem<(HEAD && h3w_mem_kind(3) == 2) ? 3 : h3w_mem_kind(3)> M(a, tx0, tout, rw, plane_g);
+        H3WMem<h3w_hook_kind<HEAD, BASE>(3)> M(a, tx0, tout, rw, plane_g);
+        H3WProducer<BASE ? h3w_base_groups(3) : 0, BASE && h3w_base_groups(3) && h3w_base_fetches(3)> P(a, h3w_lds, h3w_base_first_group(3, rw), rw);
         __builtin_amdgcn_s_waitcnt(h3_vmcnt(0));
 #define H3W_ACTIVE(s) (((s) >= 9) & ((s) < t.nrows + 11))
 #define H3W_STEP(PH) R.template step<PH>(((PH + 1) % Gm::NRX1) * Gm::PITCH, (PH % Gm::NRO) * Gm::OUT_SLOT, true, M)
-        H3W_BAND(R, M, H3W_ACTIVE, H3W_STEP)
+        H3W_BAND(R, M, P, H3W_ACTIVE, H3W_STEP)
 #undef H3W_ACTIVE
 #undef H3W_STEP
     }
@@ -621,7 +796,8 @@
 {
     using Gm = H3WGeom;
     FusedH3WArgs a = args;
-    if (!a.zeros || !a.in || (!a.out && !a.head_wh) || !bf_fused_block2_h3w_supports(a.H, a.W)) return hipErrorInvalidValue;
+    if (!a.zeros || (!a.in && !a.base_u8) || (!a.out && !a.head_wh) || !bf_fused_block2_h3w_supports(a.H, a.W)) return hipErrorInvalidValue;
+    if (a.base_u8 && (!a.base_w || a.head_wh || a.reverse_tiles || a.Hs < 1 || a.Ws < 1 || a.Hs > a.H || a.Ws > a.W)) return hipErrorInvalidValue;
     if ((int64_t)a.H * a.W * 64 >= ((int64_t)1 << 32)) return hipErrorInvalidValue;
     const BandPlan p = bf_band_plan(a.B, a.H, (a.W + Gm::SW - 1) / Gm::SW, Gm::LEAD + 2);
     a.nstrips = p.nstrips;
@@ -629,9 +805,11 @@
     a.tiles_y = p.tiles_y;
     a.ntiles = p.ntiles;
     if (a.head_wh && (!a.head_out || a.Ho < 1 || a.Wo < 1 || a.Ho > a.H || a.Wo > a.W)) return hipErrorInvalidValue;
-    void (*kernel)(FusedH3WArgs) = a.head_wh ? fused_block2_h3w_kernel<true> : fused_block2_h3w_kernel<false>;
-    const hipError_t e = bf_set_max_lds(reinterpret_cast<const void*>(kernel), Gm::LDS_BYTES);
+    void (*kernel)(FusedH3WArgs) = a.base_u8 ? fused_block2_h3w_kernel<false, true>
+                                   : a.head_wh ? fused_block2_h3w_kernel<true, false> : fused_block2_h3w_kernel<false, false>;
+    const int lds = a.base_u8 ? Gm::LDS_BYTES_BASE : Gm::LDS_BYTES;
+    const hipError_t e = bf_set_max_lds(reinterpret_cast<const void*>(kernel), lds);
     if (e != hipSuccess) return e;
-    hipLaunchKernelGGL(kernel, dim3(p.grid), dim3(Gm::NT), Gm::LDS_BYTES, s, a);
+    hipLaunchKernelGGL(kernel, dim3(p.grid), dim3(Gm::NT), lds, s, a);
     return hipGetLastError();
 }
diff --git a/blind_image_denoising_amd/model.py b/blind_image_denoising_amd/model.py
--- a/blind_image_denoising_amd/model.py
+++ b/blind_image_denoising_amd/model.py
@@ -292,6 +292,13 @@
         N.check(n if n < 0 else 0, self._h, "bf_debug_forward_plan")
         return buf.value.decode(), int(n)
 
+    BASE_PATHS = ("base_conv_kernel", "base_conv_rows_kernel", "fused_block2_h3w_kernel")
+
+    def base_path(self, batch: int, height: int, width: int, pad_pow2: bool = True, in_is_u8: bool = True) -> str:
+        n = self._lib.bf_debug_base_path(self._h, int(batch), int(height), int(width), int(bool(pad_pow2)), int(bool(in_is_u8)))
+        N.check(n if n < 0 else 0, self._h, "bf_debug_base_path")
+        return self.BASE_PATHS[n]
+
     def _as_device(self, x, dtype):
         was_numpy = isinstance(x, np.ndarray)
         if was_numpy:
diff --git a/include/bfcnn_hip_debug.h b/include/bfcnn_hip_debug.h
--- a/include/bfcnn_hip_debug.h
+++ b/include/bfcnn_hip_debug.h
@@ -46,6 +46,7 @@
                        const float* res, const float* bnc, float* dw, float* stats, float* scratch, int batch, int height,
                        int width, int epi, int reverse, int repack, void* stream);
 int bf_debug_forward_plan(bf_handle h, int batch, int height, int width, int pad_pow2, char* out, int out_bytes);
+int bf_debug_base_path(bf_handle h, int batch, int height, int width, int pad_pow2, int in_is_u8);
 float bf_debug_h3_weight_scale(float max_abs);
 int bf_debug_mfma_probe(const float* a, const float* b, float* d, void* stream);
 int bf_debug_set_upsample_band(int on);
```

Result: faster. 30080 (median of 6 runs) (+1.4%).
